# Huiweizhou/GCGCN

Measured on AMD Instinct MI355X. Metric: docs/sec fwd+bwd through CAGGC+MAGGC, higher is better.
Workload: dtype f32; 1 GPU; c2: GraphHops fwd+bwd, B=32/GPU N=64 D=256 L=2 H=8, train mode, E1/E2/X/params require grad, rotating inputs: 3 resident batches (805 MB of E per GPU), step i runs on batch i mod 3; global_batch=32, mode=graph, input_sets=3, parallelism=dp1, grad_allreduce=one coalesced collective after backward

## Files before the change

### gcgcn_amd/_lib.py

```python
from __future__ import annotations

import ctypes
import os
import re
from ctypes import c_char_p, c_double, c_float, c_int, c_int64, c_uint64, c_void_p

_HERE = os.path.dirname(os.path.abspath(__file__))
LIB_PATH = os.environ.get("GCGCN_LIB") or os.path.join(_HERE, "lib", "libgcgcn_hip.so")
HEADER_PATH = os.path.join(os.path.dirname(_HERE), "include", "gcgcn.h")
OPTIM_HEADER_PATH = os.path.join(os.path.dirname(_HERE), "include", "gcgcn_optim.h")
BERT_EMBED_HEADER_PATH = os.path.join(os.path.dirname(_HERE), "include", "gcgcn_bert_embed.h")

ABI_VERSION = 7

SALT_GAT = 0x47415431
SALT_MHA = 0x4D484131
SALT_GCN = 0x47434E31
SALT_GLUE = 0x474C5531
SALT_BERT_ATTN = 0x42415431
SALT_BERT_AO = 0x42414F31
SALT_BERT_OUT = 0x424F5531
SALT_BERT_EMB = 0x42454D31

P, I, F, L = c_void_p, c_int, c_float, c_int64


class MhaHook(ctypes.Structure):
    _fields_ = [("flat_q", c_void_p), ("Q", c_void_p), ("P", c_void_p), ("A", c_void_p), ("dQ", c_void_p), ("rng_snap", c_void_p),
                ("p", ctypes.c_float)]


class EdgeRide(ctypes.Structure):
    _fields_ = [("B", ctypes.c_int32), ("N", ctypes.c_int32), ("D", ctypes.c_int32),
                ("inp", c_void_p), ("n_valid", c_void_p), ("out", c_void_p)]


_SCALARS = {"int": c_int, "int32_t": c_int, "int64_t": c_int64, "uint64_t": c_uint64, "float": c_float, "double": c_double}
_DECL = re.compile(r"([\w\s*]+?)\b(gcgcn_\w+)\s*\(([^()]*)\)")
_DECL_OPTIM = re.compile(r"([\w\s*]+?)\b(gcopt_\w+)\s*\(([^()]*)\)")
_DECL_BERT_EMBED = re.compile(r"([\w\s*]+?)\b(gcbe_\w+)\s*\(([^()]*)\)")
_STRUCT = re.compile(r"typedef\s+struct\s+(\w+)\s*\{([^{}]*)\}\s*\1\s*;")


def _ctype(text: str, symbol: str, named: bool = True, header: str = "include/gcgcn.h"):
    toks = text.replace("*", " * ").split()
    if "*" in toks:
        return c_char_p if toks[:3] == ["const", "char", "*"] and toks.count("*") == 1 else c_void_p
    toks = [t for t in toks if t != "const"]
    if toks == ["void"] and not named:
        return None
    if toks and toks[0] in _SCALARS and len(toks) <= 1 + named:
        return _SCALARS[toks[0]]
    bad = toks[0] if toks and toks[0] not in _SCALARS else " ".join(toks[1:]) or "an empty declaration"
    raise RuntimeError(f"gcgcn_amd: cannot bind {symbol}: no ctypes type for {bad!r} in {text.strip()!r} ({header})")


def _parse_header(text: str, pattern=_DECL, header: str = "include/gcgcn.h"):
    text = re.sub(r"/\*.*?\*/|//[^\n]*", " ", text, flags=re.S)
    text = re.sub(r"^[ \t]*#.*$", " ", text, flags=re.M)
    structs = {}
    for name, body in _STRUCT.findall(text):
        structs[name] = []
        for decl in filter(str.strip, body.split(";")):
            first, *more = decl.split(",")
            ctype = _ctype(first, name, header=header)
            if more and "*" in first:
                raise RuntimeError(f"gcgcn_amd: cannot bind {name}: several names behind a pointer in {decl.strip()!r} ({header})")
            structs[name] += [(n.replace("*", " ").split()[-1], ctype) for n in (first, *more)]
    sigs = {}
    for stmt in filter(str.strip, re.sub(r'extern\s+"C"\s*\{|\}', " ", _STRUCT.sub(" ", text)).split(";")):
        m = pattern.fullmatch(stmt.strip())
        if not m or m.group(2) in sigs:
            raise RuntimeError(f"gcgcn_amd: cannot bind {m.group(2) if m else header}: "
                               f"{'declared twice' if m else 'not a declaration'}: {' '.join(stmt.split())[:100]!r}")
        ret, name, args = m.groups()
        sigs[name] = (_ctype(ret, name, named=False, header=header),
                      [] if args.strip() == "void" else [_ctype(a, name, header=header) for a in args.split(",")])
    return sigs, structs


def _load_header():
    if not os.path.exists(HEADER_PATH):
        raise RuntimeError(f"gcgcn_amd: {HEADER_PATH} not found. The binding is derived from the C header of the source tree; "
                           "there is no recorded copy to fall back to.")
    with open(HEADER_PATH) as f:
        sigs, structs = _parse_header(f.read())
    for cls, name in ((MhaHook, "gcgcn_mha_hook"), (EdgeRide, "gcgcn_edge_ride")):
        declared = [("inp" if n == "in" else n, t) for n, t in structs.get(name, [])]
        if cls._fields_ != declared:
            raise RuntimeError(f"gcgcn_amd: {cls.__name__}._fields_ {cls._fields_} differ from {name} in include/gcgcn.h: {declared}")
    return sigs


def _load_optim_header():
    if not os.path.exists(OPTIM_HEADER_PATH):
        raise RuntimeError(f"gcgcn_amd: {OPTIM_HEADER_PATH} not found. The binding is derived from the C headers of the source tree.")
    with open(OPTIM_HEADER_PATH) as f:
        sigs, structs = _parse_header(f.read(), _DECL_OPTIM, "include/gcgcn_optim.h")
    if structs:
        raise RuntimeError(f"gcgcn_amd: include/gcgcn_optim.h declares structs {list(structs)}; its tables travel as const void*")
    return sigs


def _load_bert_embed_header():
    if not os.path.exists(BERT_EMBED_HEADER_PATH):
        raise RuntimeError(f"gcgcn_amd: {BERT_EMBED_HEADER_PATH} not found. The binding is derived from the C headers of the source tree.")
    with open(BERT_EMBED_HEADER_PATH) as f:
        sigs, structs = _parse_header(f.read(), _DECL_BERT_EMBED, "include/gcgcn_bert_embed.h")
    if structs:
        raise RuntimeError(f"gcgcn_amd: include/gcgcn_bert_embed.h declares structs {list(structs)}; it takes plain arguments only")
    return sigs


SIGNATURES = _load_header()
OPTIM_SIGNATURES = _load_optim_header()
BERT_EMBED_SIGNATURES = _load_bert_embed_header()

_lib = None


def lib() -> ctypes.CDLL:
    global _lib
    if _lib is None:
        if not os.path.exists(LIB_PATH):
            raise RuntimeError(
                f"gcgcn_amd: {LIB_PATH} not found. Build it with `make -C gcgcn_amd/csrc` "
                "(or `python -c 'import __graft_entry__ as g; g.build()'`). There is no CPU fallback.")
        handle = ctypes.CDLL(LIB_PATH)
        for name, (res, args) in list(SIGNATURES.items()) + list(OPTIM_SIGNATURES.items()) + list(BERT_EMBED_SIGNATURES.items()):
            fn = getattr(handle, name)
            fn.restype = res
            fn.argtypes = args
        if handle.gcgcn_version() != ABI_VERSION:
            raise RuntimeError(f"gcgcn_amd: ABI version {handle.gcgcn_version()} != {ABI_VERSION}")
        _lib = handle
    return _lib


def call(name: str, *args):
    h = lib()
    rc = getattr(h, name)(*args)
    if rc != 0:
        raise RuntimeError(f"{name} failed ({rc}): {h.gcgcn_last_error().decode()}")


def layout(kind: str, *dims) -> list:
    n = {"gat": 9, "mha": 3, "gcn": 7, "producer": 17, "head": 7}[kind]
    out = (c_int64 * n)()
    call(f"gcgcn_{kind}_layout", *dims, ctypes.cast(out, c_void_p))
    return list(out)
```

### gcgcn_amd/csrc/api.hip

```cpp
#include "../../include/gcgcn.h"

#include <stdarg.h>
#include <string.h>

#include <new>
#include <vector>

#include <stdlib.h>

#include "attn_plan.hpp"
#include "compact.hpp"
#include "gat_body.hpp"
#include "gemm.hpp"
#include "lstm.hpp"
#include "frontend.hpp"
#include "bert.hpp"
#include "gemm_bf16.hpp"
#include "rowops.hpp"

namespace gc {

static thread_local char g_err[512] = "";

void set_error(const char* fmt, ...) {
  va_list ap;
  va_start(ap, fmt);
  vsnprintf(g_err, sizeof(g_err), fmt, ap);
  va_end(ap);
}

int check_launch(const char* what) {
  hipError_t e = hipGetLastError();
  if (e != hipSuccess) {
    set_error("%s: launch failed: %s", what, hipGetErrorString(e));
    return 2;
  }
  return 0;
}

static struct {
  bool on = false;
  char filter[48] = "";
  std::vector<hipEvent_t> ev;
  int used = 0;
  double work = 0;
} g_prof;

ProfScope::ProfScope(const char* tag, hipStream_t s, double work) : slot(-1), st(s) {
  if (!g_prof.on || strncmp(tag, g_prof.filter, strlen(g_prof.filter)) != 0) return;
  if (2 * (g_prof.used + 1) > (int)g_prof.ev.size()) return;
  slot = g_prof.used++;
  g_prof.work += work;
  (void)hipEventRecord(g_prof.ev[2 * slot], st);
}
ProfScope::~ProfScope() {
  if (slot >= 0) (void)hipEventRecord(g_prof.ev[2 * slot + 1], st);
}
bool prof_events(const char* tag, double work, hipEvent_t* start, hipEvent_t* stop) {
  if (!g_prof.on || strncmp(tag, g_prof.filter, strlen(g_prof.filter)) != 0) return false;
  if (2 * (g_prof.used + 1) > (int)g_prof.ev.size()) return false;
  const int slot = g_prof.used++;
  g_prof.work += work;
  *start = g_prof.ev[2 * slot], *stop = g_prof.ev[2 * slot + 1];
  return true;
}

struct GcnLayout {
  long oWnX, oWe, oWd, oWlin, oblin, total, wd_head;
  int gh;
  long wd_off(int h, int l) const { return oWd + h * wd_head + (long)gh * gh * l * (l - 1) / 2; }
};
static GcnLayout gcn_layout(int D, int L, int H) {
  GcnLayout y;
  y.gh = D / L;
  const long DHD = (long)D * H * D;
  y.wd_head = (long)y.gh * y.gh * L * (L - 1) / 2;
  y.oWnX = 0;
  y.oWe = DHD;
  y.oWd = 2 * DHD;
  y.oWlin = y.oWd + H * y.wd_head;
  y.oblin = y.oWlin + DHD;
  y.total = y.oblin + D;
  return y;
}

static int check_dims(const char* who, int B, int N, int D, int L, int H) {
  GC_REQUIRE(B > 0 && N > 0 && D > 0, "%s: bad shape B=%d N=%d D=%d", who, B, N, D);
  GC_REQUIRE(L > 0 && D % L == 0, "%s: D=%d not divisible by layer_num=%d", who, D, L);
  GC_REQUIRE(H > 0 && D % H == 0, "%s: D=%d not divisible by head_num=%d", who, D, H);
  return 0;
}

static long col_ride_elems(int D) { return (long)COL_RIDE_SLICES * D; }
static long gemm_scratch_elems(int B, int N, int D, int H) {
  const long a = colsum_scratch_elems((long)B * N, D, 1);
  const long rows = (long)B * N > D ? (long)B * N : D;
  const long b = gemm_ws_elems(rows, (long)H * D);
  return a > b ? a : b;
}
static long scratch_elems(int B, int N, int D, int H) { return gemm_scratch_elems(B, N, D, H) + col_ride_elems(D); }

struct Opt {
  const char* name;
  int value;
  bool resolved;
};
static Opt g_opts[] = {{"head_v1", 0, false},      {"head_bil3", 0, false}, {"head_bil3_bwd", 0, false}, {"head_dw3", 0, false},
                       {"head_compact", 0, false}, {"chain_t", 0, false},   {"chain_big", 0, false},     {"split_widen", 0, false},
                       {"chain", 0, false},        {"mha_core", 0, false},  {"group_dump", 0, false},
                       {"bf16_rows", 0, false}};
int option(const char* name, int dflt) {
  for (Opt& o : g_opts) {
    if (strcmp(o.name, name) != 0) continue;
    if (!o.resolved) {
      char env[64] = "GCGCN_";
      size_t n = strlen(env);
      for (const char* c = name; *c && n + 1 < sizeof(env); ++c) env[n++] = (char)((*c >= 'a' && *c <= 'z') ? *c - 32 : *c);
      env[n] = 0;
      const char* e = getenv(env);
      o.value = e ? atoi(e) : dflt;
      o.resolved = true;
    }
    return o.value;
  }
  return dflt;
}
static thread_local int g_head_matmul_next = 0;
int head_matmul_take() {
  const int v = g_head_matmul_next;
  g_head_matmul_next = 0;
  return v;
}
static thread_local int g_lstm_recurrent_next = 0;
int lstm_recurrent_take() {
  const int v = g_lstm_recurrent_next;
  g_lstm_recurrent_next = 0;
  return v;
}
static bool set_opt(const char* name, int value) {
  if (strcmp(name, "head_matmul") == 0) {
    g_head_matmul_next = value;
    return true;
  }
  if (strcmp(name, "lstm_recurrent") == 0) {
    g_lstm_recurrent_next = value;
    return true;
  }
  for (Opt& o : g_opts)
    if (strcmp(o.name, name) == 0) {
      o.value = value, o.resolved = true;
      return true;
    }
  return false;
}

static AttnQuery make_attn_query(int N, int D, int H, const void* Q, const void* dQ, bool hook, bool chain_attends, bool core_done) {
  return AttnQuery{N, D, H, attn_misalign(Q, dQ), hook, chain_attends, core_done, option("mha_core", 1)};
}

static int make_ride(const char* who, const gcgcn_edge_ride* ride, int kind, EdgeRide& r) {
  memset(&r, 0, sizeof(r));
  if (!ride) return 0;
  GC_REQUIRE(ride->B > 0 && ride->N > 0 && ride->D > 0 && ride->in && ride->out, "%s: bad edge ride B=%d N=%d D=%d", who,
             ride->B, ride->N, ride->D);
  GC_REQUIRE((long)ride->B * ride->N <= 0x3fffffffL, "%s: edge ride too large", who);
  r.kind = kind, r.B = ride->B, r.N = ride->N, r.D = ride->D;
  r.in = ride->in, r.n_valid = ride->n_valid, r.out = ride->out;
  return 0;
}

static void use_rows(GemmArgs& g, const int* rowblk, int mode, int zero_dead = 0) {
  if (!rowblk) return;
  g.rb = rowblk + ROWBLK_HDR, g.rb_n = rowblk;
  g.rb_mode = mode, g.rb_zero = zero_dead;
}

static const int* live_rows(const int32_t* rowblk, int N, bool ragged) {
  return (rowblk && ragged && N % 16 == 0 && N >= 32) ? rowblk : nullptr;
}

static ChainQuery make_query(int B, int N, int D, int L, int H, const GcnLayout& y, const float* flat, bool ragged, bool scratch,
                             bool hook, const EdgeRide& ride, const void* A, const void* Pn, const void* Y) {
  ChainQuery q = ChainQuery();
  q.B = B, q.N = N, q.D = D, q.L = L, q.H = H, q.gh = y.gh;
  q.HD = (long)H * D, q.oWd = y.oWd, q.wd_head = y.wd_head, q.oWlin = y.oWlin;
  q.flat = flat, q.ragged = ragged, q.scratch = scratch, q.hook = hook, q.ride = ride;
  q.A = A, q.Pn = Pn, q.Y = Y;
  q.chain = option("chain", 1), q.chain_big = option("chain_big", 0), q.chain_t = option("chain_t", 1);
  return q;
}

static GcnCtx make_ctx(int B, int N, int D, int L, int H, const GcnLayout& y, const float* X, const float* A,
                       const float* flat, const int* n_valid, Drop drop) {
  GcnCtx c;
  memset(&c, 0, sizeof(c));
  c.B = B, c.N = N, c.D = D, c.L = L, c.H = H, c.gh = y.gh;
  c.HD = (long)H * D, c.oWd = y.oWd, c.wd_head = y.wd_head;
  c.X = X, c.A = A, c.flat = flat, c.n_valid = n_valid, c.drop = drop;
  return c;
}

struct EdgeOperand {
  const float* E;
  CmpE ce;
};

static int gat_node_fwd(const float* X, const float* flat, float* uvc, float* s, long M, int D, int Dh, int uvc_valid, void* rng_state,
                        void* rng_snaps, int rng_count, hipStream_t st) {
  if (!uvc_valid) {
    GC_TRY(gat_fold_fwd(flat, uvc, D, Dh, st, rng_state, rng_snaps, rng_count));
    return node_score_fwd(X, uvc, s, M, D, st);
  }
  return node_score_fwd(X, uvc, s, M, D, st, rng_state, rng_snaps, rng_count);
}

static int gat_bwd(const EdgeOperand& eo, int B, int N, int D, int Dh, const float* X, const int* n_valid, const float* flat, Drop drop,
                   const float* uvc, const float* P, const float* dA, const float* dEbar, const float* dX_in, float* dX, float* dE,
                   float* dbias, float* dflat, float* dlogit, float* ds, float* dvpart, float* duvc, float* scratch, DeferQueue* dq,
                   hipStream_t st) {
  const bool compact = eo.E == nullptr;
  const long M = (long)B * N;
  const float* v = uvc + D;
  const EdgePlan plan = edge_plan_bwd({B, N, D, compact, true, dE != nullptr, dEbar != nullptr,
                                       compact ? 0u : edge_misalign(eo.E, v, dE, dEbar, nullptr)});
  const GatTail tail{P, dA, uvc, dX_in, ds, dX, drop, B, plan.slices};
  if (plan.route == EdgePlan::ONE) {
    GC_TRY(gat_dlogit(P, dA, uvc, dX_in, dlogit, ds, dX, B, N, D, plan.slices, drop, st));
  } else if (plan.route == EdgePlan::THREE) {
    GC_TRY(softmax_bwd(P, dA, dlogit, M, N, drop, st));
    GC_TRY(colsum(dlogit, nullptr, ds, N, N, N, B, (long)N * N, 0, N, 0, nullptr, st));
    GC_TRY(node_score_bwd(ds, uvc, dX_in, dX, M, D, st));
  }
  if (compact)
    GC_TRY(cmp_bwd(eo.ce, v, n_valid, dlogit, dEbar, dE, dvpart, scratch + plan.rowbuf_off, dbias, plan, B, N, D, st));
  else
    GC_TRY(edge_bwd(eo.E, v, n_valid, dlogit, dEbar, dE, dvpart, plan, B, N, D, st, dq, &tail));
  long part_off[3];
  int ns = 0;
  GC_TRY(colsum3(X, ds, duvc, M, D, D, dvpart, nullptr, duvc + D, M, D, D, ds, nullptr, duvc + 2 * D, M, 1, 1, scratch,
                 st, false, part_off, &ns));
  return gat_fold_bwd(flat, duvc, dflat, D, Dh, st, scratch, part_off, ns);
}

static OutBwdPlan out_bwd_plan(const OutBwdQuery& q) {
  OutBwdPlan p = OutBwdPlan();
  const bool masked = q.ragged || q.odrop;
  if (q.fuse) {
    p.mask = masked ? OutBwdPlan::MASK_CHAIN : OutBwdPlan::MASK_NONE;
    p.wsum = q.H == 1 ? OutBwdPlan::WSUM_NONE : q.wsum_fwd ? OutBwdPlan::WSUM_FORWARD : OutBwdPlan::WSUM_HERE;
    p.dwlin = OutBwdPlan::DWLIN_BACK;
    const bool in_chain = 2 * q.B <= COL_RIDE_SLICES;
    p.col1 = in_chain ? OutBwdPlan::COL1_CHAIN : OutBwdPlan::COL1_BACK;
    p.chain_slices = in_chain ? 2 * q.B : 0;
    return p;
  }
  p.mask = masked ? OutBwdPlan::MASK_LAUNCH : OutBwdPlan::MASK_NONE;
  constexpr long fold_max = 2L << 20;
  const bool fold = q.scratch && (q.H == 1 || q.wsum_fwd) && (long)q.B * q.N * q.H * q.D <= fold_max && q.dxres_aligned;
  p.fold = !fold ? OutBwdPlan::FOLD_NONE : q.H == 1 ? OutBwdPlan::FOLD_ONE_HEAD : OutBwdPlan::FOLD_HEADS;
  p.fold_drop = fold && (q.H == 1 || q.drop);
  p.head_sum_launch = !fold;
  p.wsum = p.fold == OutBwdPlan::FOLD_HEADS ? OutBwdPlan::WSUM_FORWARD : OutBwdPlan::WSUM_NONE;
  p.dwlin = OutBwdPlan::DWLIN_FRONT;
  p.col1 = q.scratch ? OutBwdPlan::COL1_FRONT : OutBwdPlan::COL1_OWN_LAUNCH;
  return p;
}

static OutBwdCol2 out_bwd_plan_col2(const OutBwdPlan& p, bool front_reduced) {
  switch (p.col1) {
    case OutBwdPlan::COL1_OWN_LAUNCH: return {OutBwdCol2::DONE, 0};
    case OutBwdPlan::COL1_CHAIN: return {OutBwdCol2::BACK_LAUNCH, p.chain_slices};
    case OutBwdPlan::COL1_BACK: return {OutBwdCol2::BACK_REDUCE, 0};
    default: break;
  }
  if (front_reduced) return {OutBwdCol2::FRONT_REDUCE, 0};
  if (p.head_sum_launch) return {OutBwdCol2::HEAD_SUM_KERNEL, 0};
  return {OutBwdCol2::BACK_LAUNCH, COL_RIDE_SLICES};
}

}

using namespace gc;

extern "C" {

int gcgcn_version(void) { return 7; }
const char* gcgcn_last_error(void) { return g_err; }

int gcgcn_set_option(const char* name, int value) {
  GC_REQUIRE(name, "set_option: null name");
  if (set_opt(name, value)) return 0;
  set_error("set_option: unknown option '%s'", name);
  return 1;
}

int64_t gcgcn_row_blocks_ints(int B, int N) { return (B > 0 && N > 0 && N % 16 == 0) ? row_blocks_ints(B, N) : 0; }
// ... 7 lines not shown
  g_prof.ev.assign(2 * (size_t)capacity, nullptr);
  for (auto& e : g_prof.ev) {
    if (hipEventCreate(&e) != hipSuccess) {
      set_error("prof_start: hipEventCreate failed");
      return 2;
    }
  }
  strncpy(g_prof.filter, kernel_prefix, sizeof(g_prof.filter) - 1);
  g_prof.used = 0;
  g_prof.work = 0;
  g_prof.on = true;
  return 0;
}
int gcgcn_prof_enable(int on) {
  g_prof.on = on != 0 && !g_prof.ev.empty();
  return 0;
}
int gcgcn_prof_stop(double* total_ms, int* launches, double* work) {
  GC_REQUIRE(total_ms && launches, "prof_stop: null pointer");
  if (work) *work = g_prof.work;
  g_prof.on = false;
  double tot = 0;
  for (int i = 0; i < g_prof.used; ++i) {
    float ms = 0.f;
    if (hipEventSynchronize(g_prof.ev[2 * i + 1]) != hipSuccess ||
        hipEventElapsedTime(&ms, g_prof.ev[2 * i], g_prof.ev[2 * i + 1]) != hipSuccess) {
      set_error("prof_stop: event query failed");
      return 2;
    }
    tot += ms;
  }
  *total_ms = tot;
  *launches = g_prof.used;
  for (hipEvent_t e : g_prof.ev) (void)hipEventDestroy(e);
  g_prof.ev.clear();
  g_prof.used = 0;
  return 0;
}

int gcgcn_rng_next(void* state, void* snaps, int count, void* stream) {
  GC_REQUIRE(state && snaps && count > 0, "rng_next: bad arguments");
  return rng_next(state, snaps, count, (hipStream_t)stream);
}
int gcgcn_dropout_keep(uint8_t* keep, int64_t n, const void* rng_snap, uint64_t salt, float p, void* stream) {
  GC_REQUIRE(keep && rng_snap, "dropout_keep: null pointer");
  Drop d = make_drop(rng_snap, salt, p);
  d.snap = (const uint64_t*)rng_snap;
  return dropout_keep(keep, n, d, (hipStream_t)stream);
}
int gcgcn_dropout(const float* x, float* y, int64_t n, const void* rng_snap, uint64_t salt, float p, void* stream) {
  GC_REQUIRE(x && y && rng_snap, "dropout: null pointer");
  GC_REQUIRE(p >= 0.f && p < 1.f, "dropout: p=%f out of [0,1)", p);
  Drop d = make_drop(rng_snap, salt, p);
  d.snap = (const uint64_t*)rng_snap;
  return dropout(x, y, n, d, (hipStream_t)stream);
}

int gcgcn_gat_layout(int D, int Dh, int64_t* o) {
  GC_REQUIRE(D > 0 && Dh > 0 && o, "gat_layout: bad arguments");
  const long DD = (long)Dh * D;
  o[0] = 0;
  o[1] = DD;
  o[2] = o[1] + Dh;
  o[3] = o[2] + DD;
  o[4] = o[3] + Dh;
  o[5] = o[4] + DD;
  o[6] = o[5] + Dh;
  o[7] = o[6] + 3 * Dh;
  o[8] = o[7] + 1;
  return 0;
}

int gcgcn_gat_fwd(int B, int N, int D, int Dh, const float* X, const float* E, const int32_t* n_valid, const float* flat,
                  const void* rng_snap, float p, float* uvc, float* s, float* P, float* A, float* Ebar, void* rng_state,
                  void* rng_snaps, int rng_count, const uint8_t* mask, int uvc_valid, void* stream) {
  hipStream_t st = (hipStream_t)stream;
  GC_TRY(check_dims("gat_fwd", B, N, D, 1, 1));
  GC_REQUIRE(Dh > 0, "gat_fwd: hidden_dim=%d", Dh);
  GC_REQUIRE(X && E && flat && uvc && s && P && Ebar, "gat_fwd: null pointer");
  const Drop drop = make_drop(rng_snap, GCGCN_SALT_GAT, p);
  GC_REQUIRE(!drop.snap || A, "gat_fwd: dropout on but A is NULL");
  GC_REQUIRE(!rng_state || (rng_snaps && rng_count > 0), "gat_fwd: rng_state given without snapshots to fill");
  GC_TRY(gat_node_fwd(X, flat, uvc, s, (long)B * N, D, Dh, uvc_valid, rng_state, rng_snaps, rng_count, st));
  return edge_fwd(E, uvc + D, n_valid, Ebar, s, P, A, drop, B, N, D, st, mask);
}

int gcgcn_gat_fwd_compact(int B, int N, int D, int Dh, const float* X, const float* Ec, const int32_t* prow, const float* bias,
                          const int32_t* n_valid, const float* flat, const void* rng_snap, float p, float* uvc, float* s, float* P,
                          float* A, float* Ebar, void* rng_state, void* rng_snaps, int rng_count, int uvc_valid, void* stream) {
  hipStream_t st = (hipStream_t)stream;
  GC_TRY(cmp_check("gat_fwd_compact", B, N, D, Ec, prow, bias));
  GC_REQUIRE(Dh > 0 && X && flat && uvc && s && P && Ebar, "gat_fwd_compact: null pointer");
  const Drop drop = make_drop(rng_snap, GCGCN_SALT_GAT, p);
  GC_REQUIRE(!drop.snap || A, "gat_fwd_compact: dropout on but A is NULL");
  GC_REQUIRE(!rng_state || (rng_snaps && rng_count > 0), "gat_fwd_compact: rng_state given without snapshots to fill");
  GC_TRY(gat_node_fwd(X, flat, uvc, s, (long)B * N, D, Dh, uvc_valid, rng_state, rng_snaps, rng_count, st));
  return cmp_fwd(CmpE{Ec, prow, bias}, uvc + D, n_valid, Ebar, s, P, A, drop, B, N, D, st);
}

int64_t gcgcn_gat_bwd_scratch(int B, int N, int D) { return edge_plan_bwd({B, N, D, false, true, false, false, 0}).scratch; }
int64_t gcgcn_gat_bwd_compact_scratch(int B, int N, int D) { return edge_plan_bwd({B, N, D, true, true, false, false, 0}).scratch; }

int gcgcn_gat_bwd(int B, int N, int D, int Dh, const float* X, const float* E, const int32_t* n_valid, const float* flat,
                  const void* rng_snap, float p, const float* uvc, const float* P, const float* dA, const float* dEbar,
                  const float* dX_in, float* dX, float* dE, float* dflat, float* dlogit, float* ds, float* dvpart,
                  float* duvc, float* scratch, void* defer_queue, void* stream) {
  GC_TRY(check_dims("gat_bwd", B, N, D, 1, 1));
  GC_REQUIRE(Dh > 0, "gat_bwd: hidden_dim=%d", Dh);
  GC_REQUIRE(X && E && flat && uvc && P && dA && dX && dflat && dlogit && ds && dvpart && duvc,
             "gat_bwd: null pointer");
  GC_REQUIRE(scratch, "gat_bwd: scratch is required");
  return gat_bwd(EdgeOperand{E, CmpE()}, B, N, D, Dh, X, n_valid, flat, make_drop(rng_snap, GCGCN_SALT_GAT, p), uvc, P, dA, dEbar, dX_in,
                 dX, dE, nullptr, dflat, dlogit, ds, dvpart, duvc, scratch, (DeferQueue*)defer_queue, (hipStream_t)stream);
}

int gcgcn_gat_bwd_compact(int B, int N, int D, int Dh, const float* X, const float* Ec, const int32_t* prow, const float* bias,
                          const int32_t* n_valid, const float* flat, const void* rng_snap, float p, const float* uvc, const float* P,
                          const float* dA, const float* dEbar, const float* dX_in, float* dX, float* dEc, float* dbias, float* dflat,
                          float* dlogit, float* ds, float* dvpart, float* duvc, float* scratch, void* stream) {
  GC_TRY(cmp_check("gat_bwd_compact", B, N, D, Ec, prow, bias));
  GC_REQUIRE(Dh > 0 && X && flat && uvc && P && dA && dX && dEc && dbias && dflat && dlogit && ds && dvpart && duvc && scratch,
             "gat_bwd_compact: null pointer");
  return gat_bwd(EdgeOperand{nullptr, CmpE{Ec, prow, bias}}, B, N, D, Dh, X, n_valid, flat, make_drop(rng_snap, GCGCN_SALT_GAT, p), uvc, P,
                 dA, dEbar, dX_in, dX, dEc, dbias, dflat, dlogit, ds, dvpart, duvc, scratch, nullptr, (hipStream_t)stream);
}

int gcgcn_edge_mean_fwd(int B, int N, int D, const float* E, const int32_t* n_valid, float* Ebar, void* stream) {
  return edge_fwd(E, nullptr, n_valid, Ebar, nullptr, nullptr, nullptr, make_drop(nullptr, 0, 0.f), B, N, D,
                  (hipStream_t)stream);
}
int gcgcn_edge_mean_bwd(int B, int N, int D, const float* dEbar, const int32_t* n_valid, float* dE, void* stream) {
  GC_REQUIRE(B > 0 && N > 0 && D > 0, "edge_mean_bwd: bad shape");
  return edge_bcast(dEbar, n_valid, dE, B, N, D, (hipStream_t)stream);
}

int gcgcn_edge_mean_fwd_compact(int B, int N, int D, const float* Ec, const int32_t* prow, const float* bias, const int32_t* n_valid,
                                float* Ebar, void* stream) {
  GC_TRY(cmp_check("edge_mean_fwd_compact", B, N, D, Ec, prow, bias));
  GC_REQUIRE(Ebar, "edge_mean_fwd_compact: null pointer");
  return cmp_fwd(CmpE{Ec, prow, bias}, nullptr, n_valid, Ebar, nullptr, nullptr, nullptr, make_drop(nullptr, 0, 0.f), B, N, D,
                 (hipStream_t)stream);
}

int gcgcn_edge_mean_bwd_compact(int B, int N, int D, const int32_t* prow, const int32_t* n_valid, const float* dEbar, float* dEc,
                                float* dbias, float* rowbuf, void* stream) {
  GC_REQUIRE(B > 0 && N > 0 && D > 0, "edge_mean_bwd_compact: bad shape B=%d N=%d D=%d", B, N, D);
  GC_REQUIRE(D <= 64 * CMAXK, "edge_mean_bwd_compact: hidden width %d (compact rows support up to %d)", D, 64 * CMAXK);
  GC_REQUIRE(prow && dEbar && dEc && dbias && rowbuf, "edge_mean_bwd_compact: null pointer");
  return cmp_bwd(CmpE{nullptr, prow, nullptr}, nullptr, n_valid, nullptr, dEbar, dEc, nullptr, rowbuf, dbias,
                 edge_plan_bcast({B, N, D, true, false, false, true, 0}), B, N, D, (hipStream_t)stream);
}

int gcgcn_mha_layout(int D, int64_t* o) {
  GC_REQUIRE(D > 0 && o, "mha_layout: bad arguments");
  o[0] = 0;
  o[1] = (long)D * D;
  o[2] = o[1] + D;
  return 0;
}

int gcgcn_mha_fwd(int B, int N, int D, int H, const float* X, const int32_t* n_valid, const float* flat,
                  const void* rng_snap, float p, float* Q, float* P, float* A, float* scratch, const int32_t* rowblk, void* stream) {
  hipStream_t st = (hipStream_t)stream;
  GC_TRY(check_dims("mha_fwd", B, N, D, 1, H));
  const long wse = scratch ? gemm_scratch_elems(B, N, D, 1) : 0;
  GC_REQUIRE(X && flat && Q && P, "mha_fwd: null pointer");
// ... 940 lines not shown
```

### gcgcn_amd/csrc/chain.hip

```cpp
#include <stdlib.h>

#include <type_traits>

#include "edge_body.hpp"
#include "gcn_plan.hpp"
#include "gemm_body.hpp"
#include "rowops.hpp"

namespace gc {

#ifdef GC_T_TRACE
__device__ long long gc_trace_s[256];
#define TS(i) do { if (blockIdx.x == 0 && threadIdx.x == 0) gc_trace_s[(i) + (c.H == 1 ? 64 : 0)] = wall_clock64(); } while (0)
extern "C" int gcgcn_debug_trace_s(long long* out) { return (int)hipMemcpyFromSymbol(out, HIP_SYMBOL(gc_trace_s), sizeof(long long) * 256); }
#else
#define TS(i)
#endif

__device__ __forceinline__ bool dev_al16(const void* p) { return (((uintptr_t)p) & 15) == 0; }

constexpr int TEAM_LDS = lds_floats<1, 1, true, true>();
constexpr int CHAIN_LDS = 2 * TEAM_LDS;
constexpr int XCHG_LDS = 64 * 64;
typedef float f32x4 __attribute__((ext_vector_type(4)));
constexpr int CW = 8;
constexpr int RB = 8;

template <bool AKC, bool BKC, bool ALIGNED, int MASK, int RT>
__device__ __forceinline__ void run_product(GemmArgs g, float* lds, int z) {
  g.ksplit = g.K;
  g.splits = 1;
  if (!ALIGNED) {
    g.vecA = dev_al16(g.A) && g.lda % 4 == 0 && g.sA1 % 4 == 0 && g.sA2 % 4 == 0;
    g.vecB = dev_al16(g.B) && g.ldb % 4 == 0 && g.sB1 % 4 == 0 && g.sB2 % 4 == 0;
  }
  const int team = threadIdx.x >> 8, t = threadIdx.x & 255;
  float* tl = lds + team * TEAM_LDS;
  const int tn = (g.N + 63) >> 6, tiles = ((g.M + 63) >> 6) * tn;
  for (int p = 0; p < tiles; p += 2) {
    int q = p + team;
    const bool live = q < tiles;
    if (!live) q = tiles - 1;
    gemm_body<1, 1, AKC, BKC, ALIGNED, 16, MASK, RT>(g, tl, q % tn, q / tn, z, t, live);
  }
}

template <bool AKC1, bool BKC1, int MK1, int RTA, bool AKC2, bool BKC2, int MK2, int RTB, bool ALIGNED>
__device__ __forceinline__ void run_two_products(GemmArgs g1, GemmArgs g2, float* lds, int z) {
  auto prep = [](GemmArgs& g) {
    g.ksplit = g.K, g.splits = 1;
    if (!ALIGNED) {
      g.vecA = dev_al16(g.A) && g.lda % 4 == 0 && g.sA1 % 4 == 0 && g.sA2 % 4 == 0;
      g.vecB = dev_al16(g.B) && g.ldb % 4 == 0 && g.sB1 % 4 == 0 && g.sB2 % 4 == 0;
    }
  };
  prep(g1), prep(g2);
  const int team = threadIdx.x >> 8, t = threadIdx.x & 255;
  float* tl = lds + team * TEAM_LDS;
  const int tn1 = (g1.N + 63) >> 6, tiles1 = ((g1.M + 63) >> 6) * tn1, b1 = tiles1 * (1 + (g1.K + 31) / 32);
  const int tn2 = (g2.N + 63) >> 6, tiles2 = ((g2.M + 63) >> 6) * tn2, b2 = tiles2 * (1 + (g2.K + 31) / 32);
  if (team == 0) {
    for (int q = 0; q < tiles1; ++q) gemm_body<1, 1, AKC1, BKC1, ALIGNED, 16, MK1, RTA>(g1, tl, q % tn1, q / tn1, z, t, true);
    for (int i = b1; i < b2; ++i) __syncthreads();
  } else {
    for (int q = 0; q < tiles2; ++q) gemm_body<1, 1, AKC2, BKC2, ALIGNED, 16, MK2, RTB>(g2, tl, q % tn2, q / tn2, z, t, true);
    for (int i = b2; i < b1; ++i) __syncthreads();
  }
}

template <bool ALIGNED>
__global__ __launch_bounds__(64 * CW) void gcn_chain_fwd_kernel(const GcnCtx c) {
  __shared__ __attribute__((aligned(16))) float lds[CHAIN_LDS];
  if (blockIdx.x >= c.B * c.H) {
    const EdgeRide& r = c.ride;
    edge_fwd_row<4, false, CW>(r.in, nullptr, r.n_valid, r.out, nullptr, nullptr, nullptr, Drop(), r.N, r.D,
                               blockIdx.x - c.B * c.H, lds);
    return;
  }
  const int z = blockIdx.x;
  const int lane = threadIdx.x & 63, wave = threadIdx.x >> 6;
  {
    const float* a = c.A + (long)z * c.N * c.N;
    for (int i0 = wave; i0 < c.N; i0 += CW * RB) {
      float s[RB];
#pragma unroll
      for (int u = 0; u < RB; ++u) s[u] = 0.f;
      for (int j = lane; j < c.N; j += 64) {
#pragma unroll
        for (int u = 0; u < RB; ++u) {
          const int i = i0 + CW * u;
          if (i < c.N) s[u] += a[(long)i * c.N + j];
        }
      }
#pragma unroll
      for (int u = 0; u < RB; ++u) {
        const int i = i0 + CW * u;
        const float t = wave_sum(s[u]);
        if (lane == 0 && i < c.N) c.rinv[(long)z * c.N + i] = 1.f / (t + (t == 0.f ? 1.f : 0.f));
      }
    }
  }
  __syncthreads();
  for (int l = 0; l < c.L; ++l) {
    if (l > 0) {
      run_product<true, false, ALIGNED, EPI_ACCUM, 0>(plan_fwd_dense(c, l), lds, z);
      __syncthreads();
    }
    run_product<true, false, ALIGNED, EPI_ADD | EPI_ROWSCALE | EPI_RELU | EPI_C2, 0>(plan_fwd_agg(c, l), lds, z);
    __syncthreads();
  }
}

template <bool ALIGNED>
__global__ __launch_bounds__(64 * CW) void gcn_chain_bwd_kernel(const GcnCtx c, const GemmGroup4 cg) {
  __shared__ __attribute__((aligned(16))) float lds[CHAIN_LDS + XCHG_LDS];
  if (blockIdx.x >= c.B * c.H) {
    int pb;
    if (spread_pick((int)blockIdx.x - c.B * c.H, c.carry, pb)) {
      gemm_group_splitk_block(cg, pb, lds, TEAM_LDS, lds + CHAIN_LDS);
      return;
    }
    const EdgeRide& r = c.ride;
    edge_bcast_row<4, CW>(r.in, r.n_valid, r.out, r.N, r.D, 0, pb);
    return;
  }
  const int z = blockIdx.x;
  const int b = z / c.H, h = z - b * c.H;
  const int lane = threadIdx.x & 63, wave = threadIdx.x >> 6;
  for (int l = c.L - 1; l >= 0; --l) {
    for (int i0 = wave; i0 < c.N; i0 += CW * RB) {
      float acc[RB], rv[RB];
#pragma unroll
      for (int u = 0; u < RB; ++u) {
        const int i = i0 + CW * u;
        acc[u] = 0.f;
        rv[u] = (i < c.N) ? c.rinv[(long)z * c.N + i] : 0.f;
      }
      for (int k = lane; k < c.gh; k += 64) {
        float y[RB], gy[RB];
#pragma unroll
        for (int u = 0; u < RB; ++u) {
          const int i = i0 + CW * u;
          const long off = ((((long)b * c.N + i) * c.H + h) * c.L + l) * c.gh + k;
          y[u] = 0.f, gy[u] = 0.f;
          if (i < c.N) y[u] = c.Y[off], gy[u] = c.dYa[off];
        }
#pragma unroll
        for (int u = 0; u < RB; ++u) {
          const int i = i0 + CW * u;
          const long off = ((((long)b * c.N + i) * c.H + h) * c.L + l) * c.gh + k;
          const float g = y[u] > 0.f ? gy[u] : 0.f;
          if (i < c.N) c.dM[off] = g * rv[u];
          acc[u] = fmaf(g, y[u], acc[u]);
        }
      }
#pragma unroll
      for (int u = 0; u < RB; ++u) {
        const int i = i0 + CW * u;
        const float t = wave_sum(acc[u]);
        if (lane == 0 && i < c.N) {
          const long ri = (long)z * c.N + i;
          const float d = -rv[u] * t;
          c.drow[ri] = (l == c.L - 1) ? d : c.drow[ri] + d;
        }
      }
    }
    __syncthreads();
    run_two_products<false, false, 0, 0, true, true, 0, EPI_ACCUM | EPI_ROWADD, ALIGNED>(plan_bwd_dP(c, l), plan_bwd_dA(c, l), lds, z);
    __syncthreads();
    if (l > 0) {
      run_product<true, true, ALIGNED, EPI_ACCUM, 0>(plan_bwd_dY(c, l), lds, z);
      __syncthreads();
    }
  }
}

constexpr int S_LA = 68;
constexpr int S_LP = 132;
constexpr int S_GH = 128;
constexpr int S_FWD_LDS = 64 * S_LA + 2 * 64 * S_LP + 64 + S_GH * S_LP;
constexpr int S_BWD_XS = 6 * 16 * 64;
constexpr int S_BWD_LDS = 64 * S_LA + 3 * 64 * S_LP + 128 + S_BWD_XS;
static_assert(S_FWD_LDS >= CHAIN_LDS && S_BWD_LDS >= CHAIN_LDS + XCHG_LDS, "passengers use the chain kernels' LDS");
static_assert(S_BWD_LDS * sizeof(float) <= 160 * 1024, "LDS of one compute unit");

__device__ __forceinline__ void lds_barrier() { asm volatile("s_waitcnt lgkmcnt(0)\n\ts_barrier" ::: "memory"); }

template <int K, bool AV, bool BV>
__device__ __forceinline__ void mma_lds(f32x16& acc, const float* __restrict__ pa, const int la,
                                        const float* __restrict__ pb, const int lb) {
#pragma unroll
  for (int k0 = 0; k0 < K; k0 += 8) {
    float a[4], b[4];
    if (AV) {
      const f32x4 v = *reinterpret_cast<const f32x4*>(pa + k0);
      a[0] = v.x, a[1] = v.y, a[2] = v.z, a[3] = v.w;
    } else {
#pragma unroll
      for (int m = 0; m < 4; ++m) a[m] = pa[(k0 + m) * la];
    }
    if (BV) {
      const f32x4 v = *reinterpret_cast<const f32x4*>(pb + k0);
      b[0] = v.x, b[1] = v.y, b[2] = v.z, b[3] = v.w;
    } else {
#pragma unroll
      for (int m = 0; m < 4; ++m) b[m] = pb[(k0 + m) * lb];
    }
#pragma unroll
    for (int m = 0; m < 4; ++m) acc = __builtin_amdgcn_mfma_f32_32x32x2f32(a[m], b[m], acc, 0, 0, 0);
  }
}
__device__ __forceinline__ int acc_row(int r0, int q) { return r0 + (q & 3) + 8 * (q >> 2); }

__global__ __launch_bounds__(64 * CW) void gcn_chain_s_fwd_kernel(const GcnCtx c) {
  __shared__ __attribute__((aligned(16))) float lds[S_FWD_LDS];
  if (blockIdx.x >= c.B * c.H) {
    const EdgeRide& r = c.ride;
    edge_fwd_row<4, false, CW>(r.in, nullptr, r.n_valid, r.out, nullptr, nullptr, nullptr, Drop(), r.N, r.D,
                               blockIdx.x - c.B * c.H, lds);
    return;
  }
  TS(0);
  float* const As = lds;
  float* const Ps = As + 64 * S_LA;
  float* const Ys = Ps + 64 * S_LP;
  float* const Rs = Ys + 64 * S_LP;
  float* const Ws = Rs + 64;
  const int z = blockIdx.x, b = z / c.H, h = z - b * c.H;
  const int t = threadIdx.x, lane = t & 63, wave = t >> 6, r = lane & 31, hf = lane >> 5;
  const int rb = wave & 1, cb = wave >> 1;
  const unsigned HD = (unsigned)c.HD, D = (unsigned)c.D;
  const long zoff = (long)b * 64 * c.HD + (long)h * 2 * S_GH;
  const float* __restrict__ Ag = c.A + (long)z * 64 * 64;
  const float* __restrict__ Pg = c.Pn + zoff;
  const float* __restrict__ Gg = c.G + zoff;
  const float* __restrict__ Xg = c.X + (long)b * 64 * c.D;
  float* __restrict__ Yg = c.Y + zoff;
  float* __restrict__ Hg = c.HO + zoff;
  const int r0 = rb * 32 + hf * 4, col = cb * 32 + r;
  const bool dd = c.drop.snap != nullptr;
  const uint64_t key = dd ? drop_key(c.drop) : 0;

  const bool own_att = c.mha.Q != nullptr;
  f32x4 a[2], p[4];
  float s[8];
  if (!own_att) {
#pragma unroll
    for (int u = 0; u < 2; ++u) {
      const int idx = t + 512 * u;
      a[u] = *reinterpret_cast<const f32x4*>(Ag + (idx >> 4) * 64 + (idx & 15) * 4);
    }
  }
#pragma unroll
  for (int u = 0; u < 4; ++u) {
    const int idx = t + 512 * u;
    p[u] = *reinterpret_cast<const f32x4*>(Pg + (unsigned)(idx >> 5) * HD + (idx & 31) * 4);
  }
  if (!own_att) {
#pragma unroll
    for (int u = 0; u < 8; ++u) s[u] = Ag[(wave * 8 + u) * 64 + lane];
  }
  float gv[2][16], xv[2][16], pv[16];
#pragma unroll
  for (int q = 0; q < 16; ++q) {
    const unsigned row = (unsigned)acc_row(r0, q);
    gv[0][q] = Gg[row * HD + (unsigned)col];
    xv[0][q] = Xg[row * D + (unsigned)col];
  }
  TS(1);
  if (own_att) {
    mha_core_fwd_body<true>(Ys, z, c.mha.Q, c.n_valid, c.mha.P, c.mha.A, 64, c.D, c.H, c.mha.dh, c.mha.kchunk, c.mha.alpha, c.mha.drop, t,
                            t < 256, As, S_LA, CW);
    lds_barrier();
#pragma unroll
    for (int u = 0; u < 8; ++u) s[u] = As[(wave * 8 + u) * S_LA + lane];
  } else {
#pragma unroll
    for (int u = 0; u < 2; ++u) {
      const int idx = t + 512 * u;
      *reinterpret_cast<f32x4*>(As + (idx >> 4) * S_LA + (idx & 15) * 4) = a[u];
    }
  }
  TS(2);
#pragma unroll
  for (int u = 0; u < 4; ++u) {
    const int idx = t + 512 * u;
    *reinterpret_cast<f32x4*>(Ps + (idx >> 5) * S_LP + (idx & 31) * 4) = p[u];
  }
#pragma unroll
  for (int u = 0; u < 8; ++u) {
    const float tt = wave_sum(s[u]);
    if (lane == 0) {
      const float ri = 1.f / (tt + (tt == 0.f ? 1.f : 0.f));
      Rs[wave * 8 + u] = ri;
      c.rinv[(long)z * 64 + wave * 8 + u] = ri;
    }
  }
  {
    const float* __restrict__ W = c.flat + c.wd_off(1) + (long)h * c.wd_head;
    f32x4 wv[8];
#pragma unroll
    for (int u = 0; u < 8; ++u) wv[u] = *reinterpret_cast<const f32x4*>(W + (t + 512 * u) * 4);
// ... 357 lines not shown
    }
    TS(33 + 10 * l);
    mma_lds<64, true, true>(dacc, Ds + ((ab & 1) * 32 + r) * S_LP + kh * 64 + 4 * hf, 0,
                            Ps + ((ab >> 1) * 32 + r) * S_LP + kh * 64 + 4 * hf, 0);
    TS(34 + 10 * l);
    if constexpr (l == 1) {
      lds_barrier();
      TS(35 + 10 * l);
#pragma unroll
      for (int u = 0; u < 8; ++u) {
        const int idx = t + 512 * u;
        *reinterpret_cast<f32x4*>(Ws + (idx >> 5) * S_LP + (idx & 31) * 4) = wd[u];
      }
#pragma unroll
      for (int u = 0; u < 4; ++u) {
        const int idx = t + 512 * u;
        p0[u] = *reinterpret_cast<const f32x4*>(Pg + (unsigned)(idx >> 5) * HD + (idx & 31) * 4);
      }
#pragma unroll
      for (int u = 0; u < 8; ++u)
#pragma unroll
        for (int kk = 0; kk < 2; ++kk) y0[u][kk] = Yg[(unsigned)(wave + 8 * u) * HD + (unsigned)(lane + 64 * kk)];
      if constexpr (!FUSE) {
#pragma unroll
        for (int q = 0; q < 16; ++q)
          gv[q] = Gy[(unsigned)acc_row(r0, q) * HD + (unsigned)col];
      }
      TS(36 + 10 * l);
      lds_barrier();
      TS(37 + 10 * l);
#pragma unroll
      for (int q = 0; q < 16; ++q) acc[q] = 0.f;
      mma_lds<S_GH, true, true>(acc, Qs + (rb * 32 + r) * S_LP + 4 * hf, 0, Ws + col * S_LP + 4 * hf, 0);
      TS(38 + 10 * l);
      lds_barrier();
#pragma unroll
      for (int q = 0; q < 16; ++q) Ds[acc_row(r0, q) * S_LP + col] = acc[q] + gv[q];
#pragma unroll
      for (int u = 0; u < 4; ++u) {
        const int idx = t + 512 * u;
        *reinterpret_cast<f32x4*>(Ps + (idx >> 5) * S_LP + (idx & 31) * 4) = p0[u];
      }
      lds_barrier();
    }
  };
  sublayer(std::integral_constant<int, 1>());
  sublayer(std::integral_constant<int, 0>());
  if (kh == 1) {
#pragma unroll
    for (int q = 0; q < 16; ++q) Qs[(ab * 16 + q) * 64 + lane] = dacc[q];
  }
  lds_barrier();
  if (kh == 0) {
    float* __restrict__ dAg = c.dA + (long)z * 64 * 64;
    const int ar0 = (ab & 1) * 32 + hf * 4, acol = (ab >> 1) * 32 + r;
#pragma unroll
    for (int q = 0; q < 16; ++q) {
      const int row = acc_row(ar0, q);
      dAg[row * 64 + acol] = dacc[q] + Qs[(ab * 16 + q) * 64 + lane] + Ts[row];
    }
  } else if (t >= 256 && t < 320) {
    c.drow[(long)z * 64 + (t - 256)] = Ts[t - 256];
  }
  TS(55);
}

bool chain_g_aligned(const ChainQuery& q, bool bwd) {
  bool ok = q.N % 64 == 0 && q.gh % 64 == 0 && al16(q.A) && al16(q.flat + q.oWd) && al16(q.Pn) && al16(q.Y);
  if (bwd) ok = ok && al16(q.dYa) && al16(q.dM) && al16(q.dP) && al16(q.dA);
  else ok = ok && al16(q.G) && al16(q.HO) && al16(q.X);
  return ok;
}
bool chain_s_serves(const ChainQuery& q, bool bwd) {
  return chain_g_aligned(q, bwd) && q.N == 64 && q.L == 2 && q.gh == S_GH && q.D == 2 * S_GH && q.wd_head % 4 == 0 && q.oWd % 4 == 0;
}
bool chain_s_fuses(const ChainQuery& q) {
  return (q.H == 1 || q.H == 8) && al16(q.flat + q.oWlin) && q.HD % 4 == 0 && al16(q.dout) && al16(q.dXres) && al16(q.dout_m);
}
bool chain_s_attends(const ChainQuery& q) {
  return mha_lds_bytes(q.D / q.H) <= sizeof(float) * 64 * S_LP && (q.D / q.H) % 4 == 0;
}
bool chain_can_carry(const EdgeRide& r) {
  return r.kind != 0 && r.D % 4 == 0 && al16(r.in) && al16(r.out) && (long)CW * r.D <= CHAIN_LDS &&
         (long)r.B * r.N <= 0x3fffffffL;
}

static ChainPlan chain_pick(const ChainQuery& q, bool bwd, bool ride) {
  ChainPlan p;
  p.ride = ride;
  const bool s = chain_s_serves(q, bwd), t = q.chain_t != 0 && chain_t_serves(q, bwd, ride);
  const bool s_preferred = s && q.chain_t < 2 && !(q.chain_t == 1 && q.ragged);
  p.kind = (t && !s_preferred) ? ChainPlan::T : s ? ChainPlan::S : ChainPlan::GENERIC;
  p.aligned = p.kind == ChainPlan::GENERIC && chain_g_aligned(q, bwd);
  p.full = p.kind == ChainPlan::T && q.N == 64 && !q.ragged;
  return p;
}
ChainPlan chain_plan_fwd(const ChainQuery& q) {
  const bool ride = chain_can_carry(q.ride);
  if (!q.chain || !(q.N <= 64 || ride || q.chain_big)) return ChainPlan();
  ChainPlan p = chain_pick(q, false, ride);
  p.attention = q.hook && (p.kind == ChainPlan::T ? chain_t_attends(q) : p.kind == ChainPlan::S && chain_s_attends(q));
  return p;
}
ChainPlan chain_plan_bwd(const ChainQuery& q) {
  if (!q.chain || !(q.N <= 64 || q.chain_big)) return ChainPlan();
  ChainPlan p = chain_pick(q, true, chain_can_carry(q.ride));
  p.fuse = q.scratch && (long)q.B * q.N * q.HD >= (long)q.D * q.D &&
           (p.kind == ChainPlan::T ? chain_t_fuses(q) : p.kind == ChainPlan::S && chain_s_fuses(q));
  return p;
}

static unsigned chain_grid(const GcnCtx& c, int kind) {
  return (unsigned)(c.B * c.H) + (c.ride.kind == kind ? (unsigned)(c.ride.B * c.ride.N) : 0u);
}

int gcn_chain_fwd(const GcnCtx& c, const ChainPlan& p, hipStream_t st) {
  GC_REQUIRE(p.kind != ChainPlan::NONE, "gcn_chain_fwd: the plan names no chain kernel");
  GC_REQUIRE((long)c.B * c.H <= 0x3fffffffL, "gcn_chain_fwd: too many (doc, head) pairs");
  GC_REQUIRE(c.ride.kind == 0 || (c.ride.kind == 1 && chain_can_carry(c.ride)), "gcn_chain_fwd: bad passenger");
  dim3 grid(chain_grid(c, 1)), block(64 * CW);
  double fl = 0;
  for (int l = 0; l < c.L; ++l) fl += 2.0 * c.N * c.gh * (c.N + (double)l * c.gh);
  if (p.kind == ChainPlan::T) return gcn_chain_t_fwd(c, p, grid, fl * c.B * c.H, st);
  if (p.kind == ChainPlan::S)
    GC_LAUNCH_TIMED("gcn_chain_fwd", fl * c.B * c.H, gcn_chain_s_fwd_kernel, grid, block, 0, st, c);
  else if (p.aligned) GC_LAUNCH_TIMED("gcn_chain_fwd", fl * c.B * c.H, gcn_chain_fwd_kernel<true>, grid, block, 0, st, c);
  else GC_LAUNCH_TIMED("gcn_chain_fwd", fl * c.B * c.H, gcn_chain_fwd_kernel<false>, grid, block, 0, st, c);
  return check_launch("gcn_chain_fwd");
}

int gcn_chain_bwd(const GcnCtx& c, const ChainPlan& p, hipStream_t st, DeferQueue* carry) {
  GC_REQUIRE(p.kind != ChainPlan::NONE, "gcn_chain_bwd: the plan names no chain kernel");
  GC_REQUIRE(c.ride.kind == 0 || (c.ride.kind == 2 && chain_can_carry(c.ride)), "gcn_chain_bwd: bad passenger");
  double fl = 0;
  for (int l = 0; l < c.L; ++l) fl += 4.0 * c.N * c.gh * c.N + 2.0 * c.N * c.gh * (double)l * c.gh;
  fl *= (double)c.B * c.H;
  if (p.kind == ChainPlan::T) return gcn_chain_t_bwd(c, p, fl, st, carry);
  GemmGroup4 cg;
  cg.nprob = 0, cg.tile_begin[0] = 0;
  int ng = 0;
  if (carry && carry->n > 0 && (long)c.B * c.H <= 64 && ((long)c.B * c.N) % 64 == 0) {
    const int passes = (((c.N + 63) / 64) * ((c.gh + 63) / 64) + 1) / 2;
    const double t_chain = 8.0 * (4 * c.L - 1) * passes;
    const double t_tile = 0.47 * ((double)c.B * c.N / 32.0);
    const long rounds = t_tile > 0 ? (long)(t_chain / t_tile) : 0;
    bool halves = true;
    for (int i = 0; i < carry->n; ++i) halves = halves && carry->p[i].K % 64 == 0 && !carry->p[i].rb;
    long budget = rounds * (256 - (long)c.B * c.H);
    if (c.ride.kind == 2) budget /= 2;
    if (rounds > 0 && halves && budget > 0) ng = gemm_take_deferred_pairs(carry, cg, &fl, budget);
  }
  dim3 grid(chain_grid(c, 2) + (unsigned)ng), block(64 * CW);
  GcnCtx cc = c;
  cc.carry = chain_carry_spread(c, ng);
  if (p.kind == ChainPlan::S && p.fuse) {
    fl += 2.0 * c.B * c.N * c.D * c.D * (c.H + (c.H > 1 ? 1 : 0));
    GC_LAUNCH_TIMED("gcn_chain_bwd", fl, gcn_chain_s_bwd_kernel<true>, grid, block, 0, st, cc, cg);
  } else if (p.kind == ChainPlan::S)
    GC_LAUNCH_TIMED("gcn_chain_bwd", fl, gcn_chain_s_bwd_kernel<false>, grid, block, 0, st, cc, cg);
  else if (p.aligned) GC_LAUNCH_TIMED("gcn_chain_bwd", fl, gcn_chain_bwd_kernel<true>, grid, block, 0, st, cc, cg);
  else GC_LAUNCH_TIMED("gcn_chain_bwd", fl, gcn_chain_bwd_kernel<false>, grid, block, 0, st, cc, cg);
  return check_launch("gcn_chain_bwd");
}

Spread chain_carry_spread(const GcnCtx& c, int ng) {
  constexpr int spread_pct = 85, cohort = 128, spread_min = 256;
  const long rows = c.ride.kind == 2 ? (long)c.ride.B * c.ride.N : 0;
  const bool on = rows > 0 && ng >= spread_min;
  return make_spread(ng, rows, cohort, on ? spread_pct : 0);
}

}
```

### gcgcn_amd/csrc/chain_t.hpp

```cpp
#pragma once
#include <type_traits>

#include "chain_t_shapes.hpp"
#include "edge_body.hpp"
#include "gcn_plan.hpp"
#include "gemm_body.hpp"
#include "rowops.hpp"

namespace gc {

#ifdef GC_T_TRACE
static __device__ long long gc_trace_t[256];
#define TR(i) do { if (blockIdx.x == 0 && threadIdx.x == 0) gc_trace_t[i] = wall_clock64(); } while (0)
#define TRB(i) do { if (blockIdx.x == 0 && threadIdx.x == 0) gc_trace_t[(i) + (c.H == 1 ? 64 : 0)] = wall_clock64(); } while (0)
#else
#define TR(i)
#define TRB(i)
#endif

typedef float t4 __attribute__((ext_vector_type(4)));

__device__ __forceinline__ void t_barrier() { asm volatile("s_waitcnt lgkmcnt(0)\n\ts_barrier" ::: "memory"); }
__device__ __forceinline__ t4 mfma16(float a, float b, t4 c) { return __builtin_amdgcn_mfma_f32_16x16x4f32(a, b, c, 0, 0, 0); }
__device__ __forceinline__ float row16_sum(float v) {
// ... 135 lines not shown
    }
    t4 acc[4];
#pragma unroll
    for (int ob = 0; ob < 4; ++ob) {
      acc[ob] = t4{0.f, 0.f, 0.f, 0.f};
#pragma unroll
      for (int kb = 0; kb < 4; ++kb) {
        if (ob < NRB && kb < NRB) {
          const t4 a = *reinterpret_cast<const t4*>(Asj + 16 * ob * T_LA + 16 * kb);
#pragma unroll
          for (int v = 0; v < 4; ++v) acc[ob] = mfma16(a[v], Pa[l][kb][v], acc[ob]);
        }
      }
    }
    TR(11 + 8 * l);
#pragma unroll
    for (int rb = 0; rb < 4; ++rb)
#pragma unroll
      for (int v = 0; v < 4; ++v) {
        const float y = fmaxf((acc[rb][v] + gv[rb][v]) * Rsg[16 * rb + v], 0.f);
        if constexpr (NP > 0) Ysg[(16 * rb + v) * P] = y;
        t_st(Yd, tHD, rowHD(rb, v, l), y);
        float d = y;
        if (dd) {
          const unsigned o = (unsigned)(16 * rb + 4 * g + v) * HD + (unsigned)(l * GH + col);
          d = (rng_u32(key, (uint64_t)(zoff + (long)o)) >= c.drop.thresh) ? y * c.drop.scale : 0.f;
        }
        t_st(Hd, tHD, rowHD(rb, v, l), d + xv[rb][v]);
      }
    if constexpr (NP > 0) {
      TR(12 + 8 * l);
      sstore(0, wr[0]);
      t_barrier();
      TR(13 + 8 * l);
      auto compute = [&](const int ch, const int st) __attribute__((always_inline)) {
        t4 a[NRB > 0 ? NRB : 1];
#pragma unroll
        for (int rb = 0; rb < NRB; ++rb) a[rb] = *reinterpret_cast<const t4*>(Ysj + 16 * rb * P + 16 * ch);
#pragma unroll
        for (int p = 0; p < NP; ++p) {
          const float* wb = Ws + ((st * (L - 1) + p) * 16 + 4 * g) * P + col;
          float bv[4];
#pragma unroll
          for (int v = 0; v < 4; ++v) bv[v] = wb[v * P];
#pragma unroll
          for (int v = 0; v < 4; ++v)
#pragma unroll
            for (int rb = 0; rb < NRB; ++rb) Pa[l + 1 + p][rb] = mfma16(a[rb][v], bv[v], Pa[l + 1 + p][rb]);
        }
      };
#pragma nounroll
      for (int ch = 0; ch < NC; ch += 2) {
        if (ch + 2 < NC) gload(ch + 2, wr[0]);
        compute(ch, 0);
        sstore(1, wr[1]);
        t_barrier();
        if (ch + 3 < NC) gload(ch + 3, wr[1]);
        compute(ch + 1, 1);
        if (ch + 2 < NC) sstore(0, wr[0]);
        t_barrier();
      }
      TR(14 + 8 * l);
#pragma unroll
      for (int rb = 0; rb < 4; ++rb)
#pragma unroll
        for (int v = 0; v < 4; ++v) t_st(Pd, tHD, rowHD(rb, v, l + 1), Pa[l + 1][rb][v]);
    }
  };
  static_assert(L >= 1 && L <= 4, "sub-layers are unrolled by hand");
  layer(std::integral_constant<int, 0>());
  if constexpr (L > 1) layer(std::integral_constant<int, 1>());
  if constexpr (L > 2) layer(std::integral_constant<int, 2>());
  if constexpr (L > 3) layer(std::integral_constant<int, 3>());
  TR(50);
}

template <int GH, int L, bool FULL>
__global__ __launch_bounds__(4 * GH) void gcn_chain_t_fwd_kernel(const GcnCtx c) {
  constexpr int W = GH / 16;
  __shared__ __attribute__((aligned(16))) float lds[t_fwd_lds(GH, L)];
  if (blockIdx.x >= c.B * c.H) {
    const EdgeRide& r = c.ride;
    edge_fwd_row<4, false, W>(r.in, nullptr, r.n_valid, r.out, nullptr, nullptr, nullptr, Drop(), r.N, r.D,
                              blockIdx.x - c.B * c.H, lds);
    return;
  }
  const int z = blockIdx.x, b = z / c.H, h = z - b * c.H;
  if constexpr (FULL) {
    chain_t_fwd_body<GH, L, 4>(c, lds, z, b, h);
  } else {
    const int nv = c.n_valid ? min(max(c.n_valid[b], 0), c.N) : c.N;
    const int nrb = (nv + 15) >> 4;
    switch (nrb) {
      case 0: chain_t_fwd_body<GH, L, 0>(c, lds, z, b, h); break;
      case 1: chain_t_fwd_body<GH, L, 1>(c, lds, z, b, h); break;
      case 2: chain_t_fwd_body<GH, L, 2>(c, lds, z, b, h); break;
      case 3: chain_t_fwd_body<GH, L, 3>(c, lds, z, b, h); break;
      default: chain_t_fwd_body<GH, L, 4>(c, lds, z, b, h); break;
    }
  }
}

constexpr int T_TEAM_LDS = lds_floats<1, 1, true, true>();
template <int NTEAM, bool RB>
__device__ __forceinline__ void t_parked_tiles(const GemmGroup4& cg, int pb, float* __restrict__ lds) {
  int i = 0, w = pb;
  while (i + 1 < cg.nprob && w >= (cg.tile_take[i] + NTEAM - 1) / NTEAM) {
    w -= (cg.tile_take[i] + NTEAM - 1) / NTEAM;
    ++i;
  }
  const int team = threadIdx.x >> 8, t = threadIdx.x & 255;
  int q = NTEAM * w + team;
  const bool live = q < cg.tile_take[i];
  if (!live) q = cg.tile_take[i] - 1;
  q = xcd_remap(q + cg.tile_first[i], cg.tile_count[i]);
  const GemmArgs& g = cg.p[i];
  const int tn = g.N >> 6, tm = g.M >> 6;
  const int zs = q / (tn * tm), r = q - zs * (tn * tm);
  const int bx = (tm < tn) ? r / tm : r % tn, by = (tm < tn) ? r % tm : r / tn;
  float* tl = lds + team * T_TEAM_LDS;
  if (g.a_kc) {
    if (g.b_kc) gemm_body<1, 1, true, true, true>(g, tl, bx, by, zs, t, live);
    else gemm_body<1, 1, true, false, true>(g, tl, bx, by, zs, t, live);
  } else {
    if (g.b_kc) gemm_body<1, 1, false, true, true>(g, tl, bx, by, zs, t, live);
    else gemm_body<1, 1, false, false, true, GC_GEMM_EG, 0, EPI_ALL, PlainOperands, RB>(g, tl, bx, by, zs, t, live);
  }
}

template <int GH, int L, int NRB, bool FUSE>
__device__ __forceinline__ void chain_t_bwd_body(const GcnCtx& c, float* __restrict__ lds, const int z, const int b, const int h, const int nv) {
  constexpr int REG = FUSE ? t_bwd_region(GH, L) : 2 * 64 * (GH + 4);
  constexpr int W = GH / 16, NT = 4 * GH, P = GH + 4, NC = GH / 16, SP = 20;
  static_assert(2 * GH * SP <= 64 * P, "weight stages live in the Pn image");
  static_assert(W <= 4 || (W / 4 - 1) * 4096 <= 64 * P, "dA exchange lives in the dM image");
  constexpr int OBW = W >= 4 ? 1 : 4 / W;
  constexpr int KS = GH >= 64 ? 4 : GH / 16;
  TRB(100);
  float* const ATs = lds;
  float* const Ds = ATs + 64 * T_LA;
  float* const Ps = Ds + 64 * P;
  float* const Tp = Ds + REG;
  float* const Ts = Tp + W * 64;
  float* const Rs = Ts + 64;
  const int t = threadIdx.x, lane = t & 63, w = t >> 6, j = lane & 15, g = lane >> 4;
  const int N = c.N;
  const unsigned HD = (unsigned)c.HD;
  const long zoff = (long)b * N * c.HD + (long)h * c.D;
  const float* __restrict__ Ag = c.A + (long)z * N * N;
  const unsigned Dw = (unsigned)c.D;
  const t_desc Yd = t_buffer(c.Y + zoff, N, HD, Dw), Gd = t_buffer(c.dYa + zoff, N, HD, Dw);
  const t_desc Md = t_buffer(c.dM + zoff, N, HD, Dw), Qd = t_buffer(c.dP + zoff, N, HD, Dw);
  const t_desc Pd = t_buffer(c.Pn + zoff, min(N, 16 * NRB), HD, Dw);
  const int col = 16 * w + j;
  const int ob = w & 3, ks = w >> 2;
  const unsigned tHD = ((unsigned)(4 * g) * HD + (unsigned)col) * 4u;
  auto rowHD = [&](const int rb, const int v, const int l) { return ((unsigned)(16 * rb + v) * HD + (unsigned)(l * GH)) * 4u; };
  const t_desc Wdd = t_buffer(c.flat + c.oWd + (long)h * c.wd_head, 1, 0, (unsigned)c.wd_head);
  const unsigned wvoff = ((unsigned)(t >> 2) * GH + 4u * (unsigned)(t & 3)) * 4u;
  float* const Dsg = Ds + 4 * g * P + col;
  float* const Tpg = Tp + w * 64 + 4 * g;
  const float* const Rsg = Rs + 4 * g;
  const float* const ATj = ATs + j * T_LA + 4 * g;
  const float* const Dsj = Ds + j * P + 4 * g;
  const float* const Psj = Ps + j * P + 4 * g;

  {
// ... 460 lines not shown
```

### gcgcn_amd/csrc/edge.hip

```cpp
#include <string.h>

#include "edge_body.hpp"
#include "compact.hpp"
#include "gat_body.hpp"
#include "gemm_body.hpp"
#include "rowops.hpp"

namespace gc {

template <int VEC, bool ATT>
__global__ __launch_bounds__(64 * EW) void edge_fwd_kernel(const float* __restrict__ E, const float* __restrict__ v,
                                                           const int* __restrict__ n_valid, float* __restrict__ Ebar,
                                                           const float* __restrict__ coladd, float* __restrict__ P,
                                                           float* __restrict__ Aout, Drop drop, int N, int D,
                                                           const unsigned char* __restrict__ mask) {
  extern __shared__ __attribute__((aligned(16))) float cs[];
  edge_fwd_row<VEC, ATT, EW>(E, v, n_valid, Ebar, coladd, P, Aout, drop, N, D, blockIdx.x, cs, mask);
}

template <int VEC>
__device__ __forceinline__ void edge_bwd_row(const float* __restrict__ E, const float* __restrict__ v,
                                             const int* __restrict__ n_valid, const float* __restrict__ dlogit,
                                             const float* __restrict__ dEbar, float* __restrict__ dE,
                                             float* __restrict__ dvpart, int N, int D, int nt, const int bi,
                                             float* __restrict__ sm, const GatTail& gt) {
  float* dl = sm;
  float* cs = sm + ((N + 3) & ~3);
  const int b = bi / N, i = bi - b * N;
  const int t = threadIdx.x, lane = t & 63, wave = t >> 6;
  const int nv = n_valid ? min(max(n_valid[b], 0), N) : N;
  float* dEr = dE ? dE + (long)bi * N * D : nullptr;
  float* dvp = dvpart + (long)bi * D;
  if (i >= nv) {
    for (int c = t; c < D; c += 64 * EW) dvp[c] = 0.f;
    if (dEr) {
      const long tot = (long)N * D;
      for (long o = t; o < tot; o += 64 * EW) dEr[o] = 0.f;
    }
    return;
  }
  if (gt.P) {
    if (wave == 0) {
      const long o = (long)bi * N + min(lane, N - 1);
      float p = gt.P[o], g = gt.dA[o];
      if (lane >= N) p = 0.f, g = 0.f;
      if (gt.drop.snap) g = (rng_u32(drop_key(gt.drop), (uint64_t)((long)bi * N + lane)) >= gt.drop.thresh) ? g * gt.drop.scale : 0.f;
      const float dot = wave_sum(g * p);
      if (lane < N) dl[lane] = p * (g - dot);
    }
  } else {
    for (int j = t; j < N; j += 64 * EW) dl[j] = dlogit[(long)bi * N + j];
  }
  __syncthreads();
  const float* __restrict__ Er = E + (long)bi * N * D;
  const float inv = 1.f / (float)nv;
  const int nchunk = (D + 64 * VEC - 1) / (64 * VEC);
  for (int q = 0; q < nchunk; ++q) {
    const int c = (q * 64 + lane) * VEC;
    const bool act = c < D;
    float vr[VEC], g[VEC], acc[VEC];
#pragma unroll
    for (int e = 0; e < VEC; ++e) vr[e] = 0.f, g[e] = 0.f, acc[e] = 0.f;
    if (act) {
      vload<VEC>(vr, v + c);
      if (dEbar) {
        vload<VEC>(g, dEbar + (long)bi * D + c);
#pragma unroll
        for (int e = 0; e < VEC; ++e) g[e] *= inv;
      }
    }
    int j = wave;
    for (; j + (EUNR - 1) * EW < nv; j += EUNR * EW) {
      float x[EUNR][VEC];
#pragma unroll
      for (int u = 0; u < EUNR; ++u) {
#pragma unroll
        for (int e = 0; e < VEC; ++e) x[u][e] = 0.f;
        if (act) vload_nt<VEC>(x[u], Er + (long)(j + u * EW) * D + c);
      }
#pragma unroll
      for (int u = 0; u < EUNR; ++u) {
        const float d = dl[j + u * EW];
        float o[VEC];
#pragma unroll
        for (int e = 0; e < VEC; ++e) {
// ... 74 lines not shown
    gemm_group_block<RB>(gg, r, tile_lds);
    return;
  }
  const int ngat = gt.P ? gt.B * gt.slices : 0;
  if (r < ngat) {
    const int b = r / gt.slices;
    gat_dlogit_doc(gt.P, gt.dA, gt.uvc, gt.dXin, nullptr, gt.ds, gt.dX, N, D, gt.drop, b, r - b * gt.slices, gt.slices, tile_lds);
    return;
  }
  edge_bwd_row<VEC>(E, v, n_valid, dlogit, dEbar, dE, dvpart, N, D, nt, r - ngat, tile_lds, gt);
}

template <int VEC>
__global__ __launch_bounds__(64 * EW) void edge_bcast_kernel(const float* __restrict__ dEbar,
                                                             const int* __restrict__ n_valid, float* __restrict__ dE,
                                                             int N, int D, int nt) {
  edge_bcast_row<VEC, EW>(dEbar, n_valid, dE, N, D, nt, blockIdx.x);
}

static inline bool al16(const void* p) { return (((uintptr_t)p) & 15) == 0; }
unsigned edge_misalign(const void* E, const void* v, const void* dE, const void* dEbar, const void* Ebar) {
  return (al16(E) ? 0 : EDGE_MIS_E) | (al16(v) ? 0 : EDGE_MIS_V) | (al16(dE) ? 0 : EDGE_MIS_DE) | (al16(dEbar) ? 0 : EDGE_MIS_DEBAR) |
         (al16(Ebar) ? 0 : EDGE_MIS_EBAR);
}
constexpr size_t EDGE_LDS_MAX = 160 * 1024;
constexpr size_t CMP_LDS_MAX = 64 * 1024;
constexpr size_t TILE_LDS = sizeof(float) * lds_floats<1, 1, true, true>();
static_assert(sizeof(float) * GAT_DOC_LDS <= TILE_LDS, "GAT passenger needs more LDS than a tile");

static EdgePlan plan_rows(const EdgeQuery& q, unsigned operands) {
  EdgePlan p;
  p.compact = q.compact, p.att = q.att;
  p.vec = (!q.compact && q.D % 4 == 0 && !(q.mis & operands)) ? 4 : 1;
  p.grid = (long)q.B * q.N;
  return p;
}

EdgePlan edge_plan_fwd(const EdgeQuery& q) {
  EdgePlan p = plan_rows(q, EDGE_MIS_E | EDGE_MIS_EBAR | (q.att ? EDGE_MIS_V : 0));
  p.lds = ((size_t)(q.compact ? CW4 : EW) * q.D + (q.att ? (size_t)q.N : 0)) * sizeof(float);
  p.lds_limit = q.compact ? CMP_LDS_MAX : EDGE_LDS_MAX;
  return p;
}

EdgePlan edge_plan_bwd(const EdgeQuery& q) {
  EdgePlan p = plan_rows(q, EDGE_MIS_E | EDGE_MIS_V | (q.has_dE ? EDGE_MIS_DE : 0) | (q.has_dEbar ? EDGE_MIS_DEBAR : 0));
  if (q.att) {
    p.route = q.N > GT ? EdgePlan::THREE : (q.compact ? EdgePlan::ONE : EdgePlan::RIDE);
    if (p.route != EdgePlan::THREE) p.slices = gat_dlogit_slices(q.D);
    if (p.route == EdgePlan::RIDE) p.ngat = q.B * p.slices;
    const long a = colsum_scratch_elems((long)q.B * q.N, q.D, 1), b = 3L * 64 * (2 * q.D + 1);
    p.scratch = a > b ? a : b;
    if (q.compact) p.rowbuf_off = p.scratch, p.scratch += 2L * q.B * q.N;
  }
  if (q.compact) {
    p.lds = ((size_t)CW4 * q.D + 2 * CW4) * sizeof(float);
    return p;
  }
  const size_t lds_row = ((size_t)((q.N + 3) & ~3) + (size_t)EW * q.D) * sizeof(float);
  p.lds = (p.ngat && lds_row < sizeof(float) * GAT_DOC_LDS) ? sizeof(float) * GAT_DOC_LDS : lds_row;
  p.lds_limit = EDGE_LDS_MAX;
  p.carry_ok = p.vec == 4 && lds_row <= TILE_LDS;
  p.grid += p.ngat;
  return p;
}

EdgePlan edge_plan_bcast(const EdgeQuery& q) {
  if (!q.compact) return plan_rows(q, EDGE_MIS_DE | EDGE_MIS_DEBAR);
  EdgeQuery m = q;
  m.att = false;
  return edge_plan_bwd(m);
}

void edge_plan_carry(EdgePlan& p, int ntile, bool any_rb, int col_C) {
  if (ntile <= 0) return;
  const long rows = p.grid;
  p.ntile = ntile, p.RB = any_rb;
  p.ncolwg = col_C > 0 ? cdiv(col_C, 256) : 0;
  p.col_base = col_C > 0 ? (int)(rows + ntile) : 0;
  p.grid = rows + ntile + p.ncolwg;
  constexpr int spread_pct = 90, cohort = 256, spread_min = 1024;
  p.spread = make_spread(ntile, rows, cohort, ntile >= spread_min ? spread_pct : 0);
  p.lds = 0;
}

constexpr int NT_STORE = 0;

int edge_fwd(const float* E, const float* v, const int* n_valid, float* Ebar, const float* coladd, float* P, float* A,
             Drop drop, int B, int N, int D, hipStream_t st, const unsigned char* mask) {
  GC_REQUIRE(E && Ebar, "edge_fwd: null pointer");
  GC_REQUIRE(B > 0 && N > 0 && D > 0, "edge_fwd: bad shape B=%d N=%d D=%d", B, N, D);
  const bool att = P != nullptr;
  GC_REQUIRE(!att || (v && coladd), "edge_fwd: attention requested without v / node scores");
  const EdgePlan p = edge_plan_fwd({B, N, D, false, att, false, false, edge_misalign(E, v, nullptr, nullptr, Ebar)});
  GC_REQUIRE(p.lds_ok(), "edge_fwd: N=%d D=%d needs %zu B of LDS", N, D, p.lds);
  dim3 grid((unsigned)p.grid), block(64 * EW);
  const char* tag = att ? "edge_fwd_att" : "edge_fwd_mean";
  const double bytes = 4.0 * B * N * N * D;
#define GC_EDGE_FWD(V, AT) \
  GC_LAUNCH_TIMED(tag, bytes, (edge_fwd_kernel<V, AT>), grid, block, p.lds, st, E, v, n_valid, Ebar, coladd, P, A, drop, N, D, mask)
  if (p.vec == 4) {
    if (att) GC_EDGE_FWD(4, true);
    else GC_EDGE_FWD(4, false);
  } else {
    if (att) GC_EDGE_FWD(1, true);
    else GC_EDGE_FWD(1, false);
  }
#undef GC_EDGE_FWD
  return check_launch("edge_fwd");
}

int edge_bwd(const float* E, const float* v, const int* n_valid, const float* dlogit, const float* dEbar, float* dE,
             float* dvpart, const EdgePlan& plan, int B, int N, int D, hipStream_t st, DeferQueue* carry, const GatTail* tail) {
  GatTail gt;
  memset(&gt, 0, sizeof gt);
  if (tail && plan.route == EdgePlan::RIDE) gt = *tail;
  GC_REQUIRE(E && v && (dlogit || gt.P) && dvpart, "edge_bwd: null pointer");
  GC_REQUIRE(!gt.P || (N <= GT && gt.B == B && gt.slices == plan.slices && gt.dA && gt.uvc && gt.ds && gt.dX), "edge_bwd: bad GAT passenger");
  GC_REQUIRE(!plan.compact && plan.ngat == (gt.P ? B * gt.slices : 0) &&
                 (plan.vec == 4) == (D % 4 == 0 && !edge_misalign(E, v, dE, dEbar, nullptr)),
             "edge_bwd: the plan was made for other operands");
  static_assert(sizeof(GatTail) + sizeof(GemmGroup) + 96 <= 4096, "edge_bwd_carry_kernel: kernel arguments exceed 4 KB");
  GC_REQUIRE(plan.lds_ok(), "edge_bwd: N=%d D=%d needs %zu B of LDS", N, D, plan.lds);
  EdgePlan p = plan;
  dim3 block(64 * EW);
  const double bytes = (dE ? 8.0 : 4.0) * B * N * N * D;
  GemmGroup gg;
  double gflops = 0;
  const int ntile = (p.carry_ok && carry && carry->n > 0) ? gemm_take_deferred(carry, gg, &gflops) : 0;
  if (ntile > 0) {
    const bool col = gemm_take_deferred_col2(carry, gg.col);
    bool any_rb = false;
    for (int i = 0; i < gg.nprob; ++i) any_rb = any_rb || gg.p[i].rb != nullptr;
    edge_plan_carry(p, ntile, any_rb, col ? gg.col.C : 0);
    dim3 grid((unsigned)p.grid);
#define GC_EDGE_CARRY(RBV)                                                                                                  \
  GC_LAUNCH_TIMED("edge_bwd", bytes, (edge_bwd_carry_kernel<4, RBV>), grid, block, 0, st, E, v, n_valid, dlogit, dEbar, dE, \
                  dvpart, N, D, NT_STORE, p.spread, gt, gg, p.col_base)
    if (p.RB) GC_EDGE_CARRY(true);
    else GC_EDGE_CARRY(false);
#undef GC_EDGE_CARRY
    return check_launch("edge_bwd_carry");
  }
  dim3 grid((unsigned)p.grid);
#define GC_EDGE_BWD(V)                                                                                                             \
  GC_LAUNCH_TIMED("edge_bwd", bytes, (edge_bwd_kernel<V>), grid, block, p.lds, st, E, v, n_valid, dlogit, dEbar, dE, dvpart, N, D, \
                  NT_STORE, gt)
  if (p.vec == 4) GC_EDGE_BWD(4);
  else GC_EDGE_BWD(1);
#undef GC_EDGE_BWD
  return check_launch("edge_bwd");
}

int edge_bcast(const float* dEbar, const int* n_valid, float* dE, int B, int N, int D, hipStream_t st) {
  GC_REQUIRE(dEbar && dE, "edge_bcast: null pointer");
  const EdgePlan p = edge_plan_bcast({B, N, D, false, false, true, true, edge_misalign(nullptr, nullptr, dE, dEbar, nullptr)});
  dim3 grid((unsigned)p.grid), block(64 * EW);
  ProfScope ps("edge_bcast", st, 4.0 * B * N * N * D);
  if (p.vec == 4) hipLaunchKernelGGL((edge_bcast_kernel<4>), grid, block, 0, st, dEbar, n_valid, dE, N, D, NT_STORE);
  else hipLaunchKernelGGL((edge_bcast_kernel<1>), grid, block, 0, st, dEbar, n_valid, dE, N, D, NT_STORE);
  return check_launch("edge_bcast");
}

}
```

### gcgcn_amd/csrc/edge_body.hpp

```cpp
#pragma once
#include "common.hpp"

namespace gc {

template <int VEC>
__device__ __forceinline__ void vload(float (&r)[VEC], const float* p) {
  if constexpr (VEC == 4) {
    const float4 v = *reinterpret_cast<const float4*>(p);
    r[0] = v.x, r[1] = v.y, r[2] = v.z, r[3] = v.w;
  } else {
    r[0] = p[0];
  }
}
template <int VEC>
__device__ __forceinline__ void vstore(float* p, const float (&r)[VEC]) {
  if constexpr (VEC == 4) {
    *reinterpret_cast<float4*>(p) = make_float4(r[0], r[1], r[2], r[3]);
  } else {
    p[0] = r[0];
  }
}

template <int VEC>
__device__ __forceinline__ void vload_nt(float (&r)[VEC], const float* p) {
// ... 52 lines not shown
                                             float* __restrict__ cs, const unsigned char* __restrict__ mask = nullptr) {
  const int b = bi / N, i = bi - b * N;
  const int t = threadIdx.x, lane = t & 63, wave = t >> 6;
  const int nv = n_valid ? min(max(n_valid[b], 0), N) : N;
  float* eb = Ebar + (long)bi * D;
  float* lg = cs + (long)EWT * D;
  if (i >= nv) {
    for (int c = t; c < D; c += 64 * EWT) eb[c] = 0.f;
    if (ATT)
      for (int j = t; j < N; j += 64 * EWT) {
        P[(long)bi * N + j] = 0.f;
        if (Aout) Aout[(long)bi * N + j] = 0.f;
      }
    return;
  }
  const float* __restrict__ Er = E + (long)bi * N * D;
  const int nchunk = (D + 64 * VEC - 1) / (64 * VEC);
  for (int q = 0; q < nchunk; ++q) {
    const int c = (q * 64 + lane) * VEC;
    const bool act = c < D;
    float vr[VEC], acc[VEC];
#pragma unroll
    for (int e = 0; e < VEC; ++e) vr[e] = 0.f, acc[e] = 0.f;
    if (ATT && act) vload<VEC>(vr, v + c);
    int j = wave;
    for (; j + (EUNR - 1) * EWT < nv; j += EUNR * EWT) {
      float x[EUNR][VEC];
#pragma unroll
      for (int u = 0; u < EUNR; ++u) {
#pragma unroll
        for (int e = 0; e < VEC; ++e) x[u][e] = 0.f;
        if (act) vload_nt<VEC>(x[u], Er + (long)(j + u * EWT) * D + c);
      }
#pragma unroll
      for (int u = 0; u < EUNR; ++u) {
        float dot = 0.f;
#pragma unroll
        for (int e = 0; e < VEC; ++e) {
          acc[e] += x[u][e];
          dot = fmaf(x[u][e], vr[e], dot);
        }
        if (ATT) {
          dot = wave_sum(dot);
          if (lane == 0) {
            if (q == 0) lg[j + u * EWT] = dot;
            else lg[j + u * EWT] += dot;
          }
        }
      }
    }
    for (; j < nv; j += EWT) {
      float x[VEC];
#pragma unroll
      for (int e = 0; e < VEC; ++e) x[e] = 0.f;
      if (act) vload<VEC>(x, Er + (long)j * D + c);
      float dot = 0.f;
#pragma unroll
      for (int e = 0; e < VEC; ++e) {
        acc[e] += x[e];
        dot = fmaf(x[e], vr[e], dot);
      }
      if (ATT) {
        dot = wave_sum(dot);
        if (lane == 0) {
          if (q == 0) lg[j] = dot;
          else lg[j] += dot;
        }
      }
    }
    if (act) vstore<VEC>(cs + wave * D + c, acc);
  }
  __syncthreads();
  const float inv = 1.f / (float)nv;
  for (int c = t; c < D; c += 64 * EWT) {
    float s = 0.f;
#pragma unroll
    for (int w = 0; w < EWT; ++w) s += cs[w * D + c];
    eb[c] = s * inv;
  }
  if (ATT && wave == 0) edge_softmax_tail(lg, coladd + (long)b * N, mask, P, Aout, drop, N, nv, (long)bi * N, lane);
}


template <int VEC, int EWT>
__device__ __forceinline__ void edge_bcast_row(const float* __restrict__ dEbar, const int* __restrict__ n_valid,
                                               float* __restrict__ dE, int N, int D, int nt, int bi) {
  const int b = bi / N, i = bi - b * N;
  const int t = threadIdx.x, lane = t & 63, wave = t >> 6;
  const int nv = n_valid ? min(max(n_valid[b], 0), N) : N;
  float* dEr = dE + (long)bi * N * D;
  const bool rowpad = i >= nv;
  const float inv = rowpad ? 0.f : 1.f / (float)nv;
  const int nchunk = (D + 64 * VEC - 1) / (64 * VEC);
  for (int q = 0; q < nchunk; ++q) {
    const int c = (q * 64 + lane) * VEC;
    if (c >= D) continue;
    float g[VEC], z[VEC];
    vload<VEC>(g, dEbar + (long)bi * D + c);
#pragma unroll
    for (int e = 0; e < VEC; ++e) g[e] *= inv, z[e] = 0.f;
    for (int j = wave; j < N; j += EWT) {
      const bool live = !rowpad && j < nv;
      if (nt) vstore_nt<VEC>(dEr + (long)j * D + c, live ? g : z);
      else vstore<VEC>(dEr + (long)j * D + c, live ? g : z);
    }
  }
}

}
```

### gcgcn_amd/csrc/edge_plan.hpp

```cpp
#pragma once
#include "common.hpp"

namespace gc {

enum EdgeMisalign { EDGE_MIS_E = 1, EDGE_MIS_V = 2, EDGE_MIS_DE = 4, EDGE_MIS_DEBAR = 8, EDGE_MIS_EBAR = 16 };
unsigned edge_misalign(const void* E, const void* v, const void* dE, const void* dEbar, const void* Ebar);

struct EdgeQuery {
  int B, N, D;
  bool compact;
  bool att;
  bool has_dE, has_dEbar;
  unsigned mis;
};

struct EdgePlan {
  enum Route { RIDE = 0, ONE = 1, THREE = 2 };
  bool compact = false, att = false;
  int vec = 1;
  int route = -1;
  int slices = -1;
  int ngat = 0;
  size_t lds = 0;
  size_t lds_limit = 0;
  bool lds_ok() const { return lds_limit == 0 || lds <= lds_limit; }
  bool carry_ok = false;
  int ntile = 0, ncolwg = 0, col_base = 0;
  bool RB = false;
  long grid = 0;
  Spread spread = {0, 0, 0};
  long scratch = -1;
  long rowbuf_off = -1;
};

EdgePlan edge_plan_fwd(const EdgeQuery& q);
EdgePlan edge_plan_bwd(const EdgeQuery& q);
EdgePlan edge_plan_bcast(const EdgeQuery& q);
void edge_plan_carry(EdgePlan& p, int ntile, bool any_rb, int col_C);

}
```

### gcgcn_amd/csrc/gcn_plan.hpp

```cpp
#pragma once
#include "gemm.hpp"
#include "mha_body.hpp"

namespace gc {

struct EdgeRide {
  int kind;
  int B, N, D;
  const float* in;
  const int* n_valid;
  float* out;
};

struct GcnCtx {
  int B, N, D, L, H, gh;
  EdgeRide ride;
  struct MhaFwd {
    const float* Q;
    float* P;
    float* A;
    float alpha;
    Drop drop;
    int dh, kchunk;
  } mha;
  Spread carry;
  long HD, oWd, wd_head;
  const float* X;
  const float* A;
  const float* flat;
  const int* n_valid;
  Drop drop;
  const float* G;
  float* Pn;
  float* Y;
  float* HO;
  float* rinv;
  float* dYa;
  float* dM;
  float* dP;
  float* dA;
  float* drow;
  const float* dout;
  float* dout_m;
  Drop odrop;
  const float* Wsum;
  float* dXres;
  float* colpart;
  long oWlin;
  __host__ __device__ long wd_off(int l) const { return oWd + (long)gh * gh * l * (l - 1) / 2; }
};

__host__ __device__ inline GemmArgs plan_fwd_dense(const GcnCtx& c, int l) {
  const long sb = (long)c.N * c.HD, sh = (long)c.L * c.gh;
  GemmArgs g = gemm_nn(c.Y, c.HD, c.flat + c.wd_off(l), c.gh, c.Pn + (long)l * c.gh, c.HD, c.N, c.gh, l * c.gh);
  g.batch_z1(c.B, sb, 0, sb).batch_z2(c.H, sh, c.wd_head, sh);
  g.splits = 1;
  g.accumulate = 1;
  g.tag = "gemm_dense";
  return g;
}

__host__ __device__ inline GemmArgs plan_fwd_agg(const GcnCtx& c, int l) {
  const long off = (long)l * c.gh, sb = (long)c.N * c.HD, sh = (long)c.L * c.gh;
  GemmArgs g = gemm_nn(c.A, c.N, c.Pn + off, c.HD, c.Y + off, c.HD, c.N, c.gh, c.N);
  g.batch_z1(c.B, (long)c.H * c.N * c.N, sb, sb).batch_z2(c.H, (long)c.N * c.N, sh, sh);
  g.splits = 1;
  g.add = c.G + off, g.ldadd = c.HD, g.sAdd1 = sb, g.sAdd2 = sh;
  g.rowscale = c.rinv, g.sRs1 = (long)c.H * c.N, g.sRs2 = c.N;
  g.relu = 1;
  g.C2 = c.HO + off, g.ldc2 = c.HD, g.sC21 = sb, g.sC22 = sh;
  g.add2 = c.X + off, g.ldadd2 = c.D, g.sAdd21 = (long)c.N * c.D, g.sAdd22 = 0;
  g.drop = c.drop, g.drop_base = off;
  g.tag = "gemm_agg";
  return g;
}

__host__ __device__ inline GemmArgs plan_bwd_dP(const GcnCtx& c, int l) {
  const long off = (long)l * c.gh, sb = (long)c.N * c.HD, sh = (long)c.L * c.gh;
  GemmArgs g = gemm_tn(c.A, c.N, c.dM + off, c.HD, c.dP + off, c.HD, c.N, c.gh, c.N);
  g.batch_z1(c.B, (long)c.H * c.N * c.N, sb, sb).batch_z2(c.H, (long)c.N * c.N, sh, sh);
  g.splits = 1;
  g.tag = "gemm_dP";
  return g;
}

__host__ __device__ inline GemmArgs plan_bwd_dA(const GcnCtx& c, int l) {
  const long off = (long)l * c.gh, sb = (long)c.N * c.HD, sh = (long)c.L * c.gh;
  GemmArgs g = gemm_nt(c.dM + off, c.HD, c.Pn + off, c.HD, c.dA, c.N, c.N, c.N, c.gh);
  g.batch_z1(c.B, sb, sb, (long)c.H * c.N * c.N).batch_z2(c.H, sh, sh, (long)c.N * c.N);
  g.splits = 1;
  g.accumulate = (l != c.L - 1);
// ... 87 lines not shown
```

### gcgcn_amd/csrc/rowops.hip

```cpp
#include "gat_body.hpp"
#include "gemm.hpp"
#include "rowops.hpp"

namespace gc {

constexpr int RW = 4;

__global__ __launch_bounds__(64 * RW) void softmax_fwd_kernel(const float* __restrict__ S, const float* __restrict__ coladd,
                                                              const int* __restrict__ n_valid, float* __restrict__ P,
                                                              float* __restrict__ A, long rows, int N, int heads,
                                                              Drop drop) {
  const long r = (long)blockIdx.x * RW + (threadIdx.x >> 6);
  if (r >= rows) return;
  const int lane = threadIdx.x & 63;
  const long doc = r / ((long)heads * N);
  const int i = (int)(r % N);
  const int nv = n_valid ? min(max(n_valid[doc], 0), N) : N;
  const float* s = S + r * N;
  float* p = P + r * N;
  float* a = A ? A + r * N : nullptr;
  if (i >= nv) {
    for (int j = lane; j < N; j += 64) {
      p[j] = 0.f;
      if (a) a[j] = 0.f;
    }
    return;
  }
  const float* ca = coladd ? coladd + doc * N : nullptr;
  float m = -INFINITY;
  for (int j = lane; j < nv; j += 64) m = fmaxf(m, s[j] + (ca ? ca[j] : 0.f));
  m = wave_max(m);
  float sum = 0.f;
  for (int j = lane; j < nv; j += 64) sum += expf(s[j] + (ca ? ca[j] : 0.f) - m);
  sum = wave_sum(sum);
  const float inv = 1.f / sum;
  const bool dd = a && drop.snap;
  const uint64_t key = dd ? drop_key(drop) : 0;
  for (int j = lane; j < N; j += 64) {
    float v = 0.f;
    if (j < nv) v = expf(s[j] + (ca ? ca[j] : 0.f) - m) * inv;
    p[j] = v;
    if (a) {
      if (dd) v = (rng_u32(key, (uint64_t)(r * N + j)) >= drop.thresh) ? v * drop.scale : 0.f;
      a[j] = v;
    }
  }
}

__global__ __launch_bounds__(64 * RW) void softmax_bwd_kernel(const float* __restrict__ P, const float* __restrict__ dA,
                                                              float* __restrict__ dS, long rows, int N, Drop drop) {
  const long r = (long)blockIdx.x * RW + (threadIdx.x >> 6);
  if (r >= rows) return;
  const int lane = threadIdx.x & 63;
  const float* p = P + r * N;
  const float* da = dA + r * N;
  float* ds = dS + r * N;
  const bool dd = drop.snap != nullptr;
  const uint64_t key = dd ? drop_key(drop) : 0;
  float dot = 0.f;
  for (int j = lane; j < N; j += 64) {
    float g = da[j];
    if (dd) g = (rng_u32(key, (uint64_t)(r * N + j)) >= drop.thresh) ? g * drop.scale : 0.f;
    dot = fmaf(g, p[j], dot);
  }
  dot = wave_sum(dot);
  for (int j = lane; j < N; j += 64) {
    float g = da[j];
    if (dd) g = (rng_u32(key, (uint64_t)(r * N + j)) >= drop.thresh) ? g * drop.scale : 0.f;
    ds[j] = p[j] * (g - dot);
  }
}

__global__ __launch_bounds__(64 * RW) void rowsum_inv_kernel(const float* __restrict__ A, float* __restrict__ rinv,
                                                             long rows, int N) {
  const long r = (long)blockIdx.x * RW + (threadIdx.x >> 6);
  if (r >= rows) return;
  const int lane = threadIdx.x & 63;
  float s = 0.f;
  for (int j = lane; j < N; j += 64) s += A[r * N + j];
  s = wave_sum(s);
  if (lane == 0) rinv[r] = 1.f / (s + (s == 0.f ? 1.f : 0.f));
}
// ... 125 lines not shown
  if (c < C) {
    long r = r0 + wave;
    for (; r + 28 < r1; r += 32) {
      float v[8], wv[8];
#pragma unroll
      for (int u = 0; u < 8; ++u) v[u] = x[(r + 4 * u) * ld + c], wv[u] = ww ? ww[r + 4 * u] : 1.f;
#pragma unroll
      for (int u = 0; u < 8; ++u) acc = fmaf(wv[u], v[u], acc);
    }
    for (; r < r1; r += 4) acc = fmaf(ww ? ww[r] : 1.f, x[r * ld + c], acc);
  }
  red[wave][lane] = acc;
  __syncthreads();
  if (wave == 0 && c < C) {
    const float s = red[0][lane] + red[1][lane] + red[2][lane] + red[3][lane];
    float* o = out + z * sOz + (long)sp * C + c;
    *o = accumulate ? *o + s : s;
  }
}

struct ColJobs {
  static constexpr int MAXJ = 4;
  const float* X[MAXJ];
  const float* w[MAXJ];
  float* out[MAXJ];
  long R[MAXJ], ld[MAXJ];
  int C[MAXJ];
  long part_off[MAXJ];
  int n;
};
__global__ __launch_bounds__(256) void colsum_multi_kernel(const ColJobs j, float* __restrict__ scratch, int ns, int stage) {
  __shared__ float red[4][64];
  const int job = blockIdx.z;
  const int lane = threadIdx.x & 63, wave = threadIdx.x >> 6;
  const int C = j.C[job];
  const int c = blockIdx.x * 64 + lane;
  if (blockIdx.x * 64 >= C) return;
  float acc = 0.f;
  if (stage == 0) {
    const long R = j.R[job], rps = (R + ns - 1) / ns;
    const long r0 = (long)blockIdx.y * rps;
    const long r1 = r0 + rps < R ? r0 + rps : R;
    const float* x = j.X[job];
    const float* w = j.w[job];
    const long ld = j.ld[job];
    if (c < C) {
      long r = r0 + wave;
      for (; r + 28 < r1; r += 32) {
        float v[8], wv[8];
#pragma unroll
        for (int u = 0; u < 8; ++u) v[u] = x[(r + 4 * u) * ld + c], wv[u] = w ? w[r + 4 * u] : 1.f;
#pragma unroll
        for (int u = 0; u < 8; ++u) acc = fmaf(wv[u], v[u], acc);
      }
      for (; r < r1; r += 4) acc = fmaf(w ? w[r] : 1.f, x[r * ld + c], acc);
    }
  } else {
    const float* x = scratch + j.part_off[job];
    if (c < C) {
      int r = wave;
      for (; r + 28 < ns; r += 32) {
        float v[8];
#pragma unroll
        for (int u = 0; u < 8; ++u) v[u] = x[(long)(r + 4 * u) * C + c];
#pragma unroll
        for (int u = 0; u < 8; ++u) acc += v[u];
      }
      for (; r < ns; r += 4) acc += x[(long)r * C + c];
    }
  }
  red[wave][lane] = acc;
  __syncthreads();
  if (wave == 0 && c < C) {
    const float s = red[0][lane] + red[1][lane] + red[2][lane] + red[3][lane];
    if (stage == 0) scratch[j.part_off[job] + (long)blockIdx.y * C + c] = s;
    else j.out[job][c] = s;
  }
}

constexpr int FW = 16;
constexpr int FC = 16;
__global__ __launch_bounds__(64 * FW) void gat_fold_fwd_kernel(const float* __restrict__ flat, float* __restrict__ uvc, int D,
                                                               int Dh, uint64_t* rng_state, uint64_t* rng_snaps,
                                                               int rng_count) {
  __shared__ float red[2][64][FC + 1];
  __shared__ float redc[FW];
  if (rng_state && blockIdx.x == 0 && threadIdx.x < 64) {
    const uint64_t seed = rng_state[0], ctr = rng_state[1];
    for (int i = threadIdx.x; i < rng_count; i += 64) rng_snaps[2 * i] = seed, rng_snaps[2 * i + 1] = ctr + (uint64_t)i;
    if (threadIdx.x == 0) rng_state[1] = ctr + (uint64_t)rng_count;
  }
  const long DD = (long)Dh * D;
  const float* Wh = flat;
  const float* bh = Wh + DD;
  const float* Wt = bh + Dh;
  const float* bt = Wt + DD;
  const float* Wr = bt + Dh;
  const float* br = Wr + DD;
  const float* wt = br + Dh;
  const int lane = threadIdx.x & 63, wave = threadIdx.x >> 6;
  const int cl = threadIdx.x & (FC - 1), rl = threadIdx.x >> 4;
  const int k = blockIdx.x * FC + cl;
  float au = 0.f, av = 0.f;
  if (k < D) {
#pragma unroll 4
    for (int d = rl; d < Dh; d += 64) {
      au = fmaf(Wh[(long)d * D + k], wt[d], au);
      au = fmaf(Wt[(long)d * D + k], wt[Dh + d], au);
      av = fmaf(Wr[(long)d * D + k], wt[2 * Dh + d], av);
    }
  }
  red[0][rl][cl] = au;
  red[1][rl][cl] = av;
  __syncthreads();
  if (threadIdx.x < 2 * FC) {
    const int which = threadIdx.x / FC, c = threadIdx.x - which * FC, kk = blockIdx.x * FC + c;
    if (kk < D) {
      float sacc = 0.f;
#pragma unroll 8
      for (int r = 0; r < 64; ++r) sacc += red[which][r][c];
      uvc[which * D + kk] = sacc;
    }
  }
  if (blockIdx.x == 0) {
    float c = 0.f;
    for (int d = threadIdx.x; d < Dh; d += 64 * FW) c += wt[d] * bh[d] + wt[Dh + d] * bt[d] + wt[2 * Dh + d] * br[d];
    c = wave_sum(c);
    if (lane == 0) redc[wave] = c;
    __syncthreads();
    if (threadIdx.x == 0) {
      float tot = wt[3 * Dh];
      for (int w = 0; w < FW; ++w) tot += redc[w];
      uvc[2 * D] = tot;
    }
  }
}

__global__ __launch_bounds__(64 * FW) void gat_fold_bwd_kernel(const float* __restrict__ flat, const float* __restrict__ duvc,
                                                               float* __restrict__ dflat, int D, int Dh,
                                                               const float* __restrict__ part, long off_dv, long off_dc,
                                                               int ns) {
  extern __shared__ float sduvc[];
  if (ns > 0) {
    for (int k = threadIdx.x; k < 2 * D + 1; k += 64 * FW) {
      const float* src = k < D ? part + k : (k < 2 * D ? part + off_dv + (k - D) : part + off_dc);
      const int C = k < 2 * D ? D : 1;
      float a = 0.f;
      int q = 0;
      for (; q + 16 <= ns; q += 16) {
        float v[16];
#pragma unroll
        for (int u = 0; u < 16; ++u) v[u] = src[(long)(q + u) * C];
#pragma unroll
        for (int u = 0; u < 16; ++u) a += v[u];
      }
      for (; q < ns; ++q) a += src[(long)q * C];
      sduvc[k] = a;
    }
    __syncthreads();
    duvc = sduvc;
  }
  const int d = blockIdx.x * FW + (threadIdx.x >> 6);
  if (d >= Dh) return;
  const int lane = threadIdx.x & 63;
  const long DD = (long)Dh * D;
  const long oWh = 0, obh = DD, oWt = obh + Dh, obt = oWt + DD, oWr = obt + Dh, obr = oWr + DD, owt = obr + Dh;
  const float* du = duvc;
  const float* dv = duvc + D;
  const float dc = duvc[2 * D];
  const float wh = flat[owt + d], wtt = flat[owt + Dh + d], wr = flat[owt + 2 * Dh + d];
  float ah = 0.f, at = 0.f, ar = 0.f;
  for (int k = lane; k < D; k += 64) {
    const float u = du[k], v = dv[k];
    dflat[oWh + (long)d * D + k] = wh * u;
    dflat[oWt + (long)d * D + k] = wtt * u;
    dflat[oWr + (long)d * D + k] = wr * v;
    ah = fmaf(flat[oWh + (long)d * D + k], u, ah);
    at = fmaf(flat[oWt + (long)d * D + k], u, at);
    ar = fmaf(flat[oWr + (long)d * D + k], v, ar);
  }
  ah = wave_sum(ah), at = wave_sum(at), ar = wave_sum(ar);
  if (lane == 0) {
    dflat[obh + d] = wh * dc;
    dflat[obt + d] = wtt * dc;
    dflat[obr + d] = wr * dc;
    dflat[owt + d] = ah + flat[obh + d] * dc;
    dflat[owt + Dh + d] = at + flat[obt + d] * dc;
    dflat[owt + 2 * Dh + d] = ar + flat[obr + d] * dc;
    if (d == 0) dflat[owt + 3 * Dh] = dc;
  }
}

__global__ __launch_bounds__(256) void gat_dlogit_kernel(const float* __restrict__ P, const float* __restrict__ dA,
                                                         const float* __restrict__ uvc, const float* __restrict__ dXin,
                                                         float* __restrict__ dlogit, float* __restrict__ ds,
                                                         float* __restrict__ dX, int N, int D, Drop drop) {
  __shared__ float sm[GAT_DOC_LDS];
  gat_dlogit_doc(P, dA, uvc, dXin, dlogit, ds, dX, N, D, drop, blockIdx.x, blockIdx.y, gridDim.y, sm);
}

__global__ __launch_bounds__(64 * RW) void node_score_fwd_kernel(const float* __restrict__ X, const float* __restrict__ uvc,
                                                                 float* __restrict__ s, long M, int D, uint64_t* rng_state,
                                                                 uint64_t* rng_snaps, int rng_count) {
  if (rng_state && blockIdx.x == 0 && threadIdx.x < 64) {
    const uint64_t seed = rng_state[0], ctr = rng_state[1];
    for (int i = threadIdx.x; i < rng_count; i += 64) rng_snaps[2 * i] = seed, rng_snaps[2 * i + 1] = ctr + (uint64_t)i;
    if (threadIdx.x == 0) rng_state[1] = ctr + (uint64_t)rng_count;
  }
  const long m = (long)blockIdx.x * RW + (threadIdx.x >> 6);
  if (m >= M) return;
  const int lane = threadIdx.x & 63;
  float a = 0.f;
  for (int k = lane; k < D; k += 64) a = fmaf(X[m * D + k], uvc[k], a);
  a = wave_sum(a);
  if (lane == 0) s[m] = a + uvc[2 * D];
}

__global__ __launch_bounds__(256) void node_score_bwd_kernel(const float* __restrict__ ds, const float* __restrict__ uvc,
                                                             const float* __restrict__ dXin, float* __restrict__ dX, long M,
                                                             int D) {
  const long e = (long)blockIdx.x * 256 + threadIdx.x;
  if (e >= M * D) return;
  const long m = e / D;
  const float v = ds[m] * uvc[e - m * D];
  dX[e] = dXin ? v + dXin[e] : v;
}

__global__ __launch_bounds__(256) void mask_rows_kernel(const float* __restrict__ x, float* __restrict__ y, long M, int D,
                                                        int N, const int* __restrict__ n_valid, Drop drop, int main_blocks,
                                                        const float* __restrict__ wlin, float* __restrict__ wsum, int H, int vec) {
  if ((int)blockIdx.x >= main_blocks) {
    const int e = (blockIdx.x - main_blocks) * 256 + threadIdx.x;
    if (e < D * D) {
      const int k = e / D, c = e - k * D;
      float s = 0.f;
      for (int h0 = 0; h0 < H; h0 += 8) {
        float v[8];
#pragma unroll
        for (int u = 0; u < 8; ++u) v[u] = wlin[((long)k * H + min(h0 + u, H - 1)) * D + c];
#pragma unroll
        for (int u = 0; u < 8; ++u) s += (h0 + u < H) ? v[u] : 0.f;
      }
      wsum[e] = s;
    }
    return;
  }
  if (vec) {
    const long e = ((long)blockIdx.x * 256 + threadIdx.x) * 4;
    if (e >= M * D) return;
    const long m = e / D;
    const long b = m / N;
    float4 v = *reinterpret_cast<const float4*>(x + e);
    if (n_valid && (int)(m - b * N) >= n_valid[b]) v = make_float4(0.f, 0.f, 0.f, 0.f);
    if (drop.snap) {
      const uint64_t key = drop_key(drop);
      v.x = (rng_u32(key, (uint64_t)e) >= drop.thresh) ? v.x * drop.scale : 0.f;
      v.y = (rng_u32(key, (uint64_t)(e + 1)) >= drop.thresh) ? v.y * drop.scale : 0.f;
      v.z = (rng_u32(key, (uint64_t)(e + 2)) >= drop.thresh) ? v.z * drop.scale : 0.f;
      v.w = (rng_u32(key, (uint64_t)(e + 3)) >= drop.thresh) ? v.w * drop.scale : 0.f;
    }
    *reinterpret_cast<float4*>(y + e) = v;
    return;
  }
  const long e = (long)blockIdx.x * 256 + threadIdx.x;
  if (e >= M * D) return;
  const long m = e / D;
  const long b = m / N;
  float v = (!n_valid || (int)(m - b * N) < n_valid[b]) ? x[e] : 0.f;
  if (drop.snap) v = (rng_u32(drop_key(drop), (uint64_t)e) >= drop.thresh) ? v * drop.scale : 0.f;
  y[e] = v;
}

__global__ __launch_bounds__(256) void row_blocks_kernel(const int* __restrict__ n_valid, int B, int N, int* __restrict__ out) {
  __shared__ int part[256];
  __shared__ int total;
  const int t = threadIdx.x, chunk = (B + 255) / 256, per = N / 16;
  int s = 0;
  for (int b = t * chunk; b < min(B, (t + 1) * chunk); ++b) s += (min(max(n_valid[b], 0), N) + 15) >> 4;
  part[t] = s;
  __syncthreads();
  if (t == 0) {
    int run = 0;
    for (int k = 0; k < 256; ++k) {
      const int v = part[k];
      part[k] = run;
      run += v;
// ... 59 lines not shown
  GC_REQUIRE(drop.snap, "dropout: no rng snapshot");
  if (n == 0) return 0;
  ProfScope ps("dropout", st);
  hipLaunchKernelGGL(dropout_kernel, dim3(cdiv(n, 256)), dim3(256), 0, st, x, y, n, drop);
  return check_launch("dropout");
}
int dropout_keep(unsigned char* keep, long n, Drop drop, hipStream_t st) {
  GC_REQUIRE(drop.snap, "dropout_keep: no rng snapshot");
  if (n == 0) return 0;
  hipLaunchKernelGGL(dropout_keep_kernel, dim3(cdiv(n, 256)), dim3(256), 0, st, keep, n, drop);
  return check_launch("dropout_keep");
}
int rng_next(void* state, void* snaps, int count, hipStream_t st) {
  hipLaunchKernelGGL(rng_next_kernel, dim3(1), dim3(64), 0, st, (uint64_t*)state, (uint64_t*)snaps, count);
  return check_launch("rng_next");
}

constexpr int COLSUM_MIN_ROWS = 32;
constexpr int COLSUM_MAX_SPLITS = 128;
long colsum_scratch_elems(long R, int C, int batch) {
  if (R < 2 * COLSUM_MIN_ROWS) return 0;
  long ns = R / COLSUM_MIN_ROWS;
  if (ns > COLSUM_MAX_SPLITS) ns = COLSUM_MAX_SPLITS;
  return ns * C * batch;
}
int colsum(const float* X, const float* w, float* out, long R, int C, long ld, int batch, long sXz, long sWz, long sOz,
           int accumulate, float* scratch, hipStream_t st) {
  if (C == 0 || batch == 0) return 0;
  long ns = 1;
  if (R >= 2 * COLSUM_MIN_ROWS && scratch) {
    ns = R / COLSUM_MIN_ROWS;
    if (ns > COLSUM_MAX_SPLITS) ns = COLSUM_MAX_SPLITS;
    const long want = 512 / ((long)cdiv(C, 64) * batch) + 1;
    if (ns > want) ns = want;
    if (ns < 2) ns = 1;
  }
  ProfScope ps("colsum", st);
  if (ns == 1) {
    hipLaunchKernelGGL(colsum_kernel, dim3(cdiv(C, 64), 1, batch), dim3(256), 0, st, X, w, out, R, C, ld, sXz, sWz, sOz,
                       R > 0 ? R : 1, accumulate);
    return check_launch("colsum");
  }
  const long rps = (R + ns - 1) / ns;
  hipLaunchKernelGGL(colsum_kernel, dim3(cdiv(C, 64), (unsigned)ns, batch), dim3(256), 0, st, X, w, scratch, R, C, ld, sXz,
                     sWz, ns * C, rps, 0);
  if (int e = check_launch("colsum/1")) return e;
  hipLaunchKernelGGL(colsum_kernel, dim3(cdiv(C, 64), 1, batch), dim3(256), 0, st, scratch, (const float*)nullptr, out, ns, C,
                     (long)C, ns * C, 0L, sOz, ns, accumulate);
  return check_launch("colsum/2");
}

int colsum3(const float* X0, const float* w0, float* o0, long R0, int C0, long ld0, const float* X1, const float* w1,
            float* o1, long R1, int C1, long ld1, const float* X2, const float* w2, float* o2, long R2, int C2, long ld2,
            float* scratch, hipStream_t st, bool stage2, long* part_off, int* ns_out) {
  ColJobs j;
  j.n = 3;
  const float* Xs[3] = {X0, X1, X2};
  const float* ws[3] = {w0, w1, w2};
  float* os[3] = {o0, o1, o2};
  const long Rs[3] = {R0, R1, R2}, lds[3] = {ld0, ld1, ld2};
  const int Cs[3] = {C0, C1, C2};
  const int ns = stage2 ? 64 : 32;
  long off = 0;
  int maxC = 1;
  for (int i = 0; i < 3; ++i) {
    j.X[i] = Xs[i], j.w[i] = ws[i], j.out[i] = os[i], j.R[i] = Rs[i], j.ld[i] = lds[i], j.C[i] = Cs[i];
    j.part_off[i] = off;
    if (part_off) part_off[i] = off;
    off += (long)ns * Cs[i];
    if (Cs[i] > maxC) maxC = Cs[i];
  }
  if (ns_out) *ns_out = ns;
  {
    ProfScope ps("colsum", st);
    hipLaunchKernelGGL(colsum_multi_kernel, dim3(cdiv(maxC, 64), ns, 3), dim3(256), 0, st, j, scratch, ns, 0);
  }
  if (int e = check_launch("colsum3/1")) return e;
  if (!stage2) return 0;
  ProfScope ps("colsum", st);
  hipLaunchKernelGGL(colsum_multi_kernel, dim3(cdiv(maxC, 64), 1, 3), dim3(256), 0, st, j, scratch, ns, 1);
  return check_launch("colsum3/2");
}

int gat_fold_fwd(const float* flat, float* uvc, int D, int Dh, hipStream_t st, void* rng_state, void* rng_snaps,
                 int rng_count) {
  ProfScope ps("gat_fold_fwd", st);
  hipLaunchKernelGGL(gat_fold_fwd_kernel, dim3(cdiv(D, FC)), dim3(64 * FW), 0, st, flat, uvc, D, Dh, (uint64_t*)rng_state,
                     (uint64_t*)rng_snaps, rng_count);
  return check_launch("gat_fold_fwd");
}
int gat_fold_bwd(const float* flat, const float* duvc, float* dflat, int D, int Dh, hipStream_t st, const float* part,
                 const long* part_off, int ns) {
  ProfScope ps("gat_fold_bwd", st);
  const size_t lds = ns > 0 ? sizeof(float) * (2 * (size_t)D + 1) : 0;
  hipLaunchKernelGGL(gat_fold_bwd_kernel, dim3(cdiv(Dh, FW)), dim3(64 * FW), lds, st, flat, duvc, dflat, D, Dh, part,
                     ns > 0 ? part_off[1] : 0L, ns > 0 ? part_off[2] : 0L, ns);
  return check_launch("gat_fold_bwd");
}
int gat_dlogit_slices(int D) { return D >= 256 ? 8 : (D >= 64 ? 4 : 1); }
int gat_dlogit(const float* P, const float* dA, const float* uvc, const float* dXin, float* dlogit, float* ds, float* dX,
               int B, int N, int D, int slices, Drop drop, hipStream_t st) {
  GC_REQUIRE(N <= GT && slices > 0, "gat_dlogit: N=%d slices=%d", N, slices);
  ProfScope ps("gat_dlogit", st);
  hipLaunchKernelGGL(gat_dlogit_kernel, dim3(B, slices), dim3(256), 0, st, P, dA, uvc, dXin, dlogit, ds, dX, N, D, drop);
  return check_launch("gat_dlogit");
}
int node_score_fwd(const float* X, const float* uvc, float* s, long M, int D, hipStream_t st, void* rng_state, void* rng_snaps,
                   int rng_count) {
  ProfScope ps("node_score_fwd", st);
  hipLaunchKernelGGL(node_score_fwd_kernel, dim3(cdiv(M, RW)), dim3(64 * RW), 0, st, X, uvc, s, M, D, (uint64_t*)rng_state,
                     (uint64_t*)rng_snaps, rng_count);
  return check_launch("node_score_fwd");
}
int node_score_bwd(const float* ds, const float* uvc, const float* dXin, float* dX, long M, int D, hipStream_t st) {
  ProfScope ps("node_score_bwd", st);
  hipLaunchKernelGGL(node_score_bwd_kernel, dim3(cdiv(M * D, 256)), dim3(256), 0, st, ds, uvc, dXin, dX, M, D);
  return check_launch("node_score_bwd");
}
int mask_rows(const float* x, float* y, long M, int D, int N, const int* n_valid, Drop drop, hipStream_t st, const float* wlin,
              float* wsum, int H) {
  ProfScope ps("mask_rows", st);
  const int vec = x && D % 4 == 0 && ((((uintptr_t)x) | ((uintptr_t)y)) & 15) == 0;
  const int main_blocks = x ? cdiv(vec ? M * D / 4 : M * D, 256) : 0, extra = wsum ? cdiv((long)D * D, 256) : 0;
  if (main_blocks + extra == 0) return 0;
  hipLaunchKernelGGL(mask_rows_kernel, dim3(main_blocks + extra), dim3(256), 0, st, x, y, M, D, N, n_valid, drop, main_blocks,
                     wlin, wsum, H, vec);
  return check_launch("mask_rows");
}

}
```

### gcgcn_amd/csrc/rowops.hpp

```cpp
#pragma once
#include "common.hpp"

namespace gc {

int softmax_fwd(const float* S, const float* coladd, const int* n_valid, float* P, float* A, long rows, int N, int heads,
                Drop drop, hipStream_t st);
int softmax_bwd(const float* P, const float* dA, float* dS, long rows, int N, Drop drop, hipStream_t st);
int rowsum_inv(const float* A, float* rinv, long rows, int N, hipStream_t st);
int relu_norm_bwd(const float* dY, const float* Y, const float* rinv, float* dM, float* drow, long rows_m, int N, int H,
                  int L, int gh, int l, int first, hipStream_t st, int relu = 1);
struct ColRide;
struct DeferQueue;
int head_sum_drop_bwd(const float* dHO, float* dY, float* dXres, long M, int H, int D, Drop drop, hipStream_t st,
                      const ColRide* finish = nullptr);
int dropout(const float* x, float* y, long n, Drop drop, hipStream_t st);
int dropout_keep(unsigned char* keep, long n, Drop drop, hipStream_t st);
int rng_next(void* state, void* snaps, int count, hipStream_t st);
long colsum_scratch_elems(long R, int C, int batch);
int colsum(const float* X, const float* w, float* out, long R, int C, long ld, int batch, long sXz, long sWz, long sOz,
           int accumulate, float* scratch, hipStream_t st);
int colsum3(const float* X0, const float* w0, float* o0, long R0, int C0, long ld0, const float* X1, const float* w1,
            float* o1, long R1, int C1, long ld1, const float* X2, const float* w2, float* o2, long R2, int C2, long ld2,
            float* scratch, hipStream_t st, bool stage2 = true, long* part_off = nullptr, int* ns_out = nullptr);
int gat_fold_fwd(const float* flat, float* uvc, int D, int Dh, hipStream_t st, void* rng_state = nullptr,
                 void* rng_snaps = nullptr, int rng_count = 0);
int gat_fold_bwd(const float* flat, const float* duvc, float* dflat, int D, int Dh, hipStream_t st,
                 const float* part = nullptr, const long* part_off = nullptr, int ns = 0);
int gat_dlogit_slices(int D);
struct GatTail;
int gat_dlogit(const float* P, const float* dA, const float* uvc, const float* dXin, float* dlogit, float* ds, float* dX,
               int B, int N, int D, int slices, Drop drop, hipStream_t st);
int node_score_fwd(const float* X, const float* uvc, float* s, long M, int D, hipStream_t st, void* rng_state = nullptr,
                   void* rng_snaps = nullptr, int rng_count = 0);
int node_score_bwd(const float* ds, const float* uvc, const float* dXin, float* dX, long M, int D, hipStream_t st);
int mask_rows(const float* x, float* y, long M, int D, int N, const int* n_valid, Drop drop, hipStream_t st,
              const float* wlin = nullptr, float* wsum = nullptr, int H = 0);

int edge_fwd(const float* E, const float* v, const int* n_valid, float* Ebar, const float* coladd, float* P, float* A,
             Drop drop, int B, int N, int D, hipStream_t st, const unsigned char* mask = nullptr);
struct EdgePlan;
int edge_bwd(const float* E, const float* v, const int* n_valid, const float* dlogit, const float* dEbar, float* dE,
             float* dvpart, const EdgePlan& plan, int B, int N, int D, hipStream_t st, DeferQueue* carry = nullptr,
             const GatTail* tail = nullptr);
int edge_bcast(const float* dEbar, const int* n_valid, float* dE, int B, int N, int D, hipStream_t st);

int row_blocks(const int* n_valid, int B, int N, int* out, hipStream_t st);
constexpr int ROWBLK_HDR = 4;
constexpr int ROWBLK_LIST_MAX = 512;
static inline long row_blocks_ints(int B, int N) { return ROWBLK_HDR + (long)B * N / 16; }

int pair_bce_fwd(const float* logits, const float* labels, const int* n_valid, float* loss, float* part, int B, int N, int R,
                 hipStream_t st);
int pair_bce_bwd(const float* logits, const float* labels, const int* n_valid, const float* dloss, float* dlogits, int B, int N,
                 int R, hipStream_t st);
int pair_stats(const float* logits, const float* labels, const int* n_valid, int64_t* counters, int B, int N, int R,
               hipStream_t st);

int64_t eval_ws_bytes(int64_t n_records, int64_t n_keep);
int eval_scan(const float* logits, const float* labels, const uint8_t* in_train, const int* n_valid, const int64_t* doc_base,
              uint64_t* rec, int64_t capacity, int64_t* counters, int B, int N, int R, hipStream_t st);
int eval_rank(const uint64_t* rec, int64_t n, void* ws, int64_t ws_bytes, int64_t* sorted_off, hipStream_t st);
int eval_curve(const uint64_t* keys, int64_t m, const int64_t* counters, double input_theta, float* pr_x, float* pr_y,
               float* ign_pr_y, double* res, void* ws, int64_t ws_bytes, int64_t n_records, hipStream_t st);

}
```

### gcgcn_amd/functional.py

```python
from __future__ import annotations

import ctypes
import os
import threading
import weakref
from dataclasses import dataclass
from typing import Optional

import torch
from torch.autograd.function import once_differentiable

from . import _lib
from ._lib import SALT_GLUE, call

Tensor = torch.Tensor


def _p(t: Optional[Tensor]):
    return None if t is None else t.data_ptr()


_raw_stream = getattr(torch._C, "_cuda_getCurrentRawStream", None)


# ... 73 lines not shown
        with _rng_lock:
            st = _rng_state.setdefault(idx, st)
    return st


def _new_snaps(dev: torch.device, count: int) -> Tensor:
    snaps = torch.empty(count, 2, dtype=torch.int64, device=dev)
    call("gcgcn_rng_next", _p(_state(dev)), _p(snaps), count, _stream())
    return snaps


class rng_scope:

    def __init__(self, dev: torch.device, count: int, enabled: bool = True):
        self.dev, self.count, self.enabled = dev, count, enabled

    def __enter__(self):
        self.prev = _get_scope()
        if self.enabled:
            _tls.scope = [torch.empty(self.count, 2, dtype=torch.int64, device=self.dev), 0, True]
        return self

    def __exit__(self, *exc):
        _tls.scope = self.prev
        return False


def _take_pending_rng(dev: torch.device):
    sc = _get_scope()
    if sc is not None and sc[2] and sc[0].device == dev:
        sc[2] = False
        return _state(dev), sc[0], sc[0].shape[0]
    return None


def rng_snapshot(dev: torch.device, lazy: bool = False) -> Tensor:
    sc = _get_scope()
    if sc is not None and sc[1] < sc[0].shape[0] and sc[0].device == dev:
        if sc[2] and not lazy:
            sc[2] = False
            call("gcgcn_rng_next", _p(_state(dev)), _p(sc[0]), sc[0].shape[0], _stream())
        snap = sc[0][sc[1]]
        sc[1] += 1
        return snap
    return _new_snaps(dev, 1)[0]


def dropout_keep_mask(snap: Tensor, salt: int, p: float, numel: int) -> Tensor:
    keep = torch.empty(numel, dtype=torch.uint8, device=snap.device)
    call("gcgcn_dropout_keep", _p(keep), numel, _p(snap), salt, float(p), _stream())
    return keep.bool()


def _gat_fwd_buffers(x: Tensor, snap, pending, uvc, uvc_valid):
    B, N, D = x.shape
    dev = x.device
    rng = pending if pending is not None else (None, None, 0)
    if uvc is None:
        uvc, uvc_valid = torch.empty(2 * D + 1, device=dev), False
    s = torch.empty(B, N, device=dev)
    P = torch.empty(B, N, N, device=dev)
    A = torch.empty(B, N, N, device=dev) if snap is not None else None
    ebar = torch.empty(B, N, D, device=dev)
    return uvc, uvc_valid, s, P, A, ebar, rng


def _gat_bwd_buffers(x: Tensor, dA, dEbar, dXin, scratch_elems: str):
    B, N, D = x.shape
    dev = x.device
    dA = torch.zeros(B, N, N, device=dev) if dA is None else dA.contiguous()
    dEbar = None if dEbar is None else dEbar.contiguous()
    dXin = None if dXin is None else dXin.contiguous()
    dlogit = torch.empty(B, N, N, device=dev)
    ds = torch.empty(B, N, device=dev)
    dvpart = torch.empty(B * N, D, device=dev)
    duvc = torch.empty(2 * D + 1, device=dev)
    scratch = torch.empty(max(getattr(_lib.lib(), scratch_elems)(B, N, D), 1), device=dev)
    return dA, dEbar, dXin, dlogit, ds, dvpart, duvc, scratch


class GatFn(torch.autograd.Function):

    @staticmethod
    def forward(ctx, x, e, flat, n_valid, p, snap, pending, Dh, mask, uvc, uvc_valid):
        B, N, D = x.shape
        uvc, uvc_valid, s, P, A, ebar, (st, sn, cnt) = _gat_fwd_buffers(x, snap, pending, uvc, uvc_valid)
        call("gcgcn_gat_fwd", B, N, D, Dh, _p(x), _p(e), _p(n_valid), _p(flat), _p(snap), float(p), _p(uvc), _p(s),
             _p(P), _p(A), _p(ebar), _p(st), _p(sn), cnt, _p(mask), 1 if uvc_valid else 0, _stream())
        ctx.save_for_backward(x, e, flat, uvc, P)
        ctx.n_valid, ctx.p, ctx.snap, ctx.Dh, ctx.mask = n_valid, float(p), snap, Dh, mask
        return (P if A is None else A), ebar, x.view_as(x)

    @staticmethod
    def backward(ctx, dA, dEbar, dXin):
        x, e, flat, uvc, P = ctx.saved_tensors
        B, N, D = x.shape
        dev = x.device
        dA, dEbar, dXin, dlogit, ds, dvpart, duvc, scratch = _gat_bwd_buffers(x, dA, dEbar, dXin, "gcgcn_gat_bwd_scratch")
        if ctx.mask is not None:
            gone = ctx.mask.bool()
            if ctx.n_valid is not None:
                gone = gone | (torch.arange(N, device=dev)[None, None, :] >= ctx.n_valid[:, None, None])
            dA = dA.masked_fill(gone.all(-1, keepdim=True), 0.0)
        dX = torch.empty_like(x)
        dE = torch.empty_like(e) if ctx.needs_input_grad[1] else None
        dflat = torch.empty_like(flat)
        bp = _current_pass()
        call("gcgcn_gat_bwd", B, N, D, ctx.Dh, _p(x), _p(e), _p(ctx.n_valid), _p(flat), _p(ctx.snap), ctx.p, _p(uvc), _p(P),
             _p(dA), _p(dEbar), _p(dXin), _p(dX), _p(dE), _p(dflat), _p(dlogit), _p(ds), _p(dvpart), _p(duvc),
             _p(scratch), None if bp is None else bp.queue, _stream())
        return dX, dE, dflat, None, None, None, None, None, None, None, None


class EdgeMeanFn(torch.autograd.Function):

    @staticmethod
    def forward(ctx, e, n_valid):
        B, N, _, D = e.shape
        ebar = torch.empty(B, N, D, device=e.device)
        call("gcgcn_edge_mean_fwd", B, N, D, _p(e), _p(n_valid), _p(ebar), _stream())
        ctx.n_valid, ctx.shape = n_valid, (B, N, D)
        return ebar

    @staticmethod
    def backward(ctx, dEbar):
        B, N, D = ctx.shape
        dEbar = dEbar.contiguous()
        dE = torch.empty(B, N, N, D, device=dEbar.device)
        call("gcgcn_edge_mean_bwd", B, N, D, _p(dEbar), _p(ctx.n_valid), _p(dE), _stream())
        return dE, None


class MhaFn(torch.autograd.Function):

    @staticmethod
    def forward(ctx, x, flat, n_valid, H, p, snap, rowblk=None):
        B, N, D = x.shape
        dev = x.device
        Q = torch.empty(B, N, D, device=dev)
        P = torch.empty(B, H, N, N, device=dev)
        A = torch.empty(B, H, N, N, device=dev) if snap is not None else None
        scratch = torch.empty(max(_lib.lib().gcgcn_mha_scratch(B, N, D), 1), device=dev)
        call("gcgcn_mha_fwd", B, N, D, H, _p(x), _p(n_valid), _p(flat), _p(snap), float(p), _p(Q), _p(P), _p(A),
             _p(scratch), _p(rowblk), _stream())
        ctx.save_for_backward(x, flat, Q, P)
        ctx.H, ctx.p, ctx.snap, ctx.rowblk = H, float(p), snap, rowblk
        return (P if A is None else A), x.view_as(x)

    @staticmethod
    def backward(ctx, dA, dXin):
        x, flat, Q, P = ctx.saved_tensors
        B, N, D = x.shape
        H, dev = ctx.H, x.device
        dA = torch.zeros(B, H, N, N, device=dev) if dA is None else dA.contiguous()
        dXin = None if dXin is None else dXin.contiguous()
        dX = torch.empty_like(x)
        dflat = torch.empty_like(flat)
        dS = torch.empty(B, H, N, N, device=dev)
        dQ = torch.empty(B, N, D, device=dev)
        scratch = torch.empty(max(_lib.lib().gcgcn_mha_scratch(B, N, D), 1), device=dev)
        call("gcgcn_mha_bwd", B, N, D, H, _p(x), _p(flat), _p(ctx.snap), ctx.p, _p(Q), _p(P), _p(dA), _p(dXin), _p(dX),
             _p(dflat), _p(dS), _p(dQ), _p(scratch), None, 0, _p(ctx.rowblk), _stream())
        return dX, dflat, None, None, None, None, None


defer_weight_grads = os.environ.get("GCGCN_DEFER", "1") != "0"
defer_fused_mha_weight_grads = os.environ.get("GCGCN_DEFER_MHA", "1") != "0"
_warned_ddp = [False]


def _under_ddp() -> bool:
    ddp = getattr(torch.nn.parallel, "DistributedDataParallel", None)
    if ddp is not None and not hasattr(ddp, "_active_ddp_module"):
        import torch.distributed as dist
        on = dist.is_available() and dist.is_initialized() and dist.get_world_size() > 1
    else:
        on = ddp is not None and getattr(ddp, "_active_ddp_module", None) is not None
    if on and defer_weight_grads and not _warned_ddp[0]:
        _warned_ddp[0] = True
        import warnings
        warnings.warn("gcgcn_amd: running under torch DistributedDataParallel -- deferred weight gradients are switched off "
                      "for these blocks (their AccumulateGrad hooks need the gradient during backward); "
                      "gcgcn_amd.dist.FlatGradBucket reduces the flat gradients without that cost")
    return on
_passes = {}
_passes_lock = threading.Lock()


class _BackwardPass:
    def __init__(self, task_id: int):
        self.task_id = task_id
        self.queue = _lib.lib().gcgcn_defer_create()
        if not self.queue:
            raise MemoryError("gcgcn_defer_create failed")
        self.keep = []
        self.installs = []

    def park(self, leaf, dflat, operands):
        self.keep.append(operands)
        self.installs.append((leaf, dflat))

    def __call__(self):
        with _passes_lock:
            _passes.pop(self.task_id, None)
        try:
            if _lib.lib().gcgcn_defer_count(self.queue) > 0:
                call("gcgcn_defer_flush", self.queue, _stream())
            with torch.no_grad():
                for leaf, dflat in self.installs:
                    if leaf.grad is None:
                        leaf.grad = dflat
                    else:
                        leaf.grad.add_(dflat)
        finally:
            self.keep.clear()
            self.installs.clear()

    def __del__(self):
        q, self.queue = self.queue, None
        if q:
            try:
                _lib.lib().gcgcn_defer_destroy(q)
            except Exception:
                pass


def _current_pass() -> Optional[_BackwardPass]:
    tid = torch._C._current_graph_task_id()
    if tid < 0:
        return None
    ref = _passes.get(tid)
    return None if ref is None else ref()


def _pass_for_parking(ctx, idx: int, leaf=None) -> Optional[_BackwardPass]:
    if not (defer_weight_grads and ctx.needs_input_grad[idx]):
        return None
    leaf = ctx.flat_leaf if leaf is None else leaf
    if leaf is None or leaf._post_accumulate_grad_hooks or leaf._backward_hooks:
        return None
    tid = torch._C._current_graph_task_id()
    if tid < 0:
        return None
    try:
        acc = ctx.next_functions[idx][0]
        if acc is None or getattr(acc, "variable", None) is not leaf or torch._C._will_engine_execute_node(acc) is not True:
            return None
    except RuntimeError:
        return None
    with _passes_lock:
        ref = _passes.get(tid)
        bp = None if ref is None else ref()
        if bp is None:
            bp = _BackwardPass(tid)
            _passes[tid] = weakref.ref(bp)
            torch.autograd.Variable._execution_engine.queue_callback(bp)
            for k in [k for k, r in _passes.items() if r() is None]:
                del _passes[k]
    return bp


def _ride(inp, n_valid, out, B, N, D):
    r = _lib.EdgeRide(B, N, D, inp.data_ptr(), None if n_valid is None else n_valid.data_ptr(), out.data_ptr())
    return r, ctypes.cast(ctypes.pointer(r), ctypes.c_void_p)


head_sum_in_forward = True


def _gcn_forward(ctx, x, ebar, adj, flat, n_valid, L, H, p, snap, e_next, out_p, out_snap, rowblk, hook=None, saved=()):
    B, N, D = x.shape
    dev = x.device
    HD = H * D
    out = torch.empty(B, N, D, device=dev)
    Pn, Y, HO = (torch.empty(B, N, HD, device=dev) for _ in range(3))
    if hook is None:
        rinv = torch.empty(B, H, N, device=dev)
        G = torch.empty(B, N, HD, device=dev)
    else:
        G = torch.empty(B, N, HD, device=dev)
        rinv = torch.empty(B, H, N, device=dev)
    wsum = torch.empty(D, D, device=dev) if (H > 1 and head_sum_in_forward and any(ctx.needs_input_grad[:4])) else None
    scratch = torch.empty(max(_lib.lib().gcgcn_gcn_scratch(B, N, D, H), 1), device=dev)
    ebar_next, ride, ride_p = None, None, None
    if e_next is not None:
        ebar_next = torch.empty(e_next.shape[0], e_next.shape[1], e_next.shape[3], device=dev)
        ride, ride_p = _ride(e_next, n_valid, ebar_next, *ebar_next.shape)
    call("gcgcn_gcn_fwd", B, N, D, L, H, _p(x), _p(ebar), None if hook is not None else _p(adj), _p(n_valid), _p(flat), _p(snap),
         float(p), _p(out_snap), float(out_p), _p(out), _p(Pn), _p(Y), _p(HO), _p(rinv), _p(G), _p(wsum), _p(scratch), ride_p,
         None if hook is None else ctypes.cast(ctypes.pointer(hook), ctypes.c_void_p), _p(rowblk), _stream())
    del ride
    ctx.save_for_backward(x, ebar, adj, flat, Pn, Y, HO, rinv, *saved)
    ctx.wsum, ctx.rowblk, ctx.n_valid, ctx.L, ctx.H = wsum, rowblk, n_valid, L, H
    ctx.p, ctx.snap, ctx.out_p, ctx.out_snap = float(p), snap, float(out_p), out_snap
    ctx.flat_leaf = flat if (flat.is_leaf and not _under_ddp()) else None
    ctx.next_shape = None if e_next is None else tuple(e_next.shape)
    return out, ebar_next


def _gcn_backward(ctx, dout, debar_next, e_next_input, mha_hook=None):
    x, ebar, adj, flat, Pn, Y, HO, rinv = ctx.saved_tensors[:8]
    B, N, D = x.shape
    L, H, dev = ctx.L, ctx.H, x.device
    HD = H * D
    dout = dout.contiguous()
    dX, dEbar = torch.empty_like(x), torch.empty_like(ebar)
    dA = torch.empty_like(adj)
    dflat = torch.empty_like(flat)
    W1, W2, W3 = (torch.empty(B, N, HD, device=dev) for _ in range(3))
    drow = torch.empty(B, H, N, device=dev)
    dXres = torch.empty(B, N, D, device=dev)
    dout_m = torch.empty(B, N, D, device=dev) if (ctx.n_valid is not None or ctx.out_snap is not None) else None
    scratch = torch.empty(max(_lib.lib().gcgcn_gcn_scratch(B, N, D, H), 1), device=dev)
    dQ = None if mha_hook is None else torch.empty(B, N, D, device=dev)
    hook = None if mha_hook is None else mha_hook(dQ)
    dE_next, ride, ride_p = None, None, None
    if ctx.next_shape is not None and ctx.needs_input_grad[e_next_input] and debar_next is not None:
        debar_next = debar_next.contiguous()
        dE_next = torch.empty(ctx.next_shape, device=dev)
        ride, ride_p = _ride(debar_next, ctx.n_valid, dE_next, *debar_next.shape)
    bp = _pass_for_parking(ctx, 3)
    call("gcgcn_gcn_bwd", B, N, D, L, H, _p(x), _p(ebar), _p(adj), _p(ctx.n_valid), _p(flat), _p(ctx.snap),
         ctx.p, _p(ctx.out_snap), ctx.out_p, _p(Pn), _p(Y), _p(HO), _p(rinv), _p(ctx.wsum), _p(dout), _p(dX), _p(dEbar), _p(dA),
         _p(dflat), _p(W1), _p(W2), _p(W3), _p(drow), _p(dXres), _p(dout_m), _p(scratch), ride_p,
         None if hook is None else ctypes.cast(ctypes.pointer(hook), ctypes.c_void_p),
         None if bp is None else bp.queue, _p(ctx.rowblk), _stream())
    del ride, hook
    if bp is not None:
        bp.park(ctx.flat_leaf, dflat, (x, ebar, Y, HO, dout, dout_m, W2, W3, ctx.rowblk))
        dflat = None
    return dX, dEbar, dA, dflat, dE_next, dQ


class GcnFn(torch.autograd.Function):

    @staticmethod
    def forward(ctx, x, ebar, adj, flat, n_valid, L, H, p, snap, e_next, out_p, out_snap, rowblk=None):
        return _gcn_forward(ctx, x, ebar, adj, flat, n_valid, L, H, p, snap, e_next, out_p, out_snap, rowblk)

    @staticmethod
    def backward(ctx, dout, debar_next):
        dX, dEbar, dA, dflat, dE_next, _ = _gcn_backward(ctx, dout, debar_next, 9)
        return dX, dEbar, dA, dflat, None, None, None, None, None, dE_next, None, None, None


class MaggcFn(torch.autograd.Function):

    @staticmethod
    def forward(ctx, x, ebar, flat_mha, flat, n_valid, L, H, p_mha, snap_mha, p, snap, e_next, out_p, out_snap, rowblk=None):
        B, N, D = x.shape
        dev = x.device
        Q = torch.empty(B, N, D, device=dev)
        P = torch.empty(B, H, N, N, device=dev)
        A = torch.empty(B, H, N, N, device=dev) if snap_mha is not None else None
        hook = _lib.MhaHook(flat_mha.data_ptr(), Q.data_ptr(), P.data_ptr(), _p(A), None, _p(snap_mha), float(p_mha))
        ctx.p_mha, ctx.snap_mha = float(p_mha), snap_mha
        ctx.flat_mha_leaf = flat_mha if (flat_mha.is_leaf and not _under_ddp()) else None
        return _gcn_forward(ctx, x, ebar, P if A is None else A, flat, n_valid, L, H, p, snap, e_next, out_p, out_snap, rowblk,
                            hook=hook, saved=(flat_mha, Q, P))

    @staticmethod
    def backward(ctx, dout, debar_next):
        x, flat_mha, Q, P = ctx.saved_tensors[0], *ctx.saved_tensors[8:]
        B, N, D = x.shape
        H, dev = ctx.H, x.device
        dXc, dEbar, dA, dflat, dE_next, dQ = _gcn_backward(
            ctx, dout, debar_next, 11, lambda dQ: _lib.MhaHook(None, Q.data_ptr(), P.data_ptr(), None, dQ.data_ptr(), _p(ctx.snap_mha), ctx.p_mha))
        dX = torch.empty_like(x)
        dflat_mha = torch.empty_like(flat_mha)
        dS = torch.empty(1, device=dev)
# ... 331 lines not shown
    feats = [_chk(f, f"node_feats[{i}]", 3) for i, f in enumerate(feats)]
    B, N, Hd = feats[0].shape
    if any(tuple(f.shape) != (B, N, Hd) for f in feats):
        raise ValueError("node_feats: every entry must have the same [B,N,H] shape")
    for nm, t, shp in (("node_type", node_type, (B, N)), ("node_relative_pos", node_relative_pos, (B, N, N))):
        if not t.is_cuda or t.dtype != torch.int64 or tuple(t.shape) != shp:
            raise ValueError(f"{nm}: expected a GPU int64 tensor of shape {shp}, got {t.dtype} {tuple(t.shape)} on {t.device}")
    if ner_emb.dim() != 2 or ner_emb.shape[0] != NER_ROWS:
        raise ValueError(f"ner_emb.weight: the head indexes {NER_ROWS} rows (nn.Embedding(7, .), glove:241), got {tuple(ner_emb.shape)}")
    if dis_table.dim() != 2 or dis_table.shape[0] < 2 * int(dis_plus) + 1:
        raise ValueError(f"dis_embed.weight: needs at least 2 * dis_plus + 1 = {2 * int(dis_plus) + 1} rows, got {tuple(dis_table.shape)}")
    if dis_table.shape[0] > HEAD_MAX_DIS_ROWS:
        raise ValueError(f"dis_embed.weight: the head handles at most {HEAD_MAX_DIS_ROWS} rows of the distance table (its backward "
                         f"pass keeps one sum per id in LDS), got {tuple(dis_table.shape)}")
    _check_id_range([("node_type", node_type, 0, NER_ROWS - 1),
                     ("node_relative_pos", node_relative_pos, -int(dis_plus), int(dis_plus))])
    return HEAD_MATMUL[matmul].apply(_chk(flat, "flat"), _chk(ner_emb, "ner_emb.weight", 2), _chk(dis_table, "dis_embed.weight", 2),
                                     node_type.contiguous(), node_relative_pos.contiguous(), _nv(n_valid, B, N, flat.device),
                                     int(relation_num), int(dis_plus), *feats)


def producer_live_counts(sen: Tensor, n_valid=None):
    B, N, _, S, T = sen.shape
    counts = torch.empty(2, dtype=torch.int32, device=sen.device)
    call("gcgcn_producer_count", B, N, S, T, _p(sen), _p(n_valid), _p(counts), _stream())
    r, q = counts.tolist()
    return r, q


check_position_ids = False


class ProducerCapacityError(RuntimeError):
    """max_live_slots / max_live_pairs were smaller than what the batch holds."""


def edge_features(tok, sen, pos_h, pos_t, node, dis_table, flat, n_valid=None, max_live_slots=None, max_live_pairs=None,
                  check_capacity=False, return_counts=False, compact=False, deterministic=False):
    tok, node, dis_table = _chk(tok, "context_output", 3), _chk(node, "node_feat", 3), _chk(dis_table, "dis_embed.weight", 2)
    B, T, Hd = tok.shape
    if sen.dim() != 5 or sen.shape[0] != B or sen.shape[4] != T or sen.shape[1] != sen.shape[2]:
        raise ValueError(f"sen_matrix: expected [B={B}, N, N, S, T={T}], got {tuple(sen.shape)}")
    N, S = sen.shape[1], sen.shape[3]
    if node.shape != (B, N, Hd):
        raise ValueError(f"node_feat: expected {(B, N, Hd)}, got {tuple(node.shape)}")
    if not sen.is_cuda:
        raise RuntimeError("sen_matrix: gcgcn_amd runs on MI355X only (no CPU fallback)")
    if sen.dtype == torch.bool:
        sen = sen.view(torch.uint8)
    elif sen.dtype != torch.uint8:
        sen = (sen != 0).to(torch.uint8)
    sen = sen.contiguous()
    for nm, p in (("pos_matrix_h", pos_h), ("pos_matrix_t", pos_t)):
        if tuple(p.shape) != tuple(sen.shape) or p.dtype not in (torch.int64, torch.int32, torch.uint8) or not p.is_cuda:
            raise ValueError(f"{nm}: expected a GPU int64 / int32 / uint8 tensor of shape {tuple(sen.shape)}")
    if pos_t.dtype != pos_h.dtype:
        raise ValueError("pos_matrix_h and pos_matrix_t must have the same dtype")
    if check_position_ids:
        _check_id_range([("pos_matrix_h", pos_h, 0, dis_table.shape[0] - 1), ("pos_matrix_t", pos_t, 0, dis_table.shape[0] - 1)])
    nv = _nv(n_valid, B, N, tok.device)
    given = max_live_slots is not None and max_live_pairs is not None
    if not given:
        r, q = producer_live_counts(sen, nv)
        max_live_slots = r if max_live_slots is None else max_live_slots
        max_live_pairs = q if max_live_pairs is None else max_live_pairs
    out = ProducerFn.apply(tok, node, dis_table, _chk(flat, "flat"), sen, pos_h.contiguous(), pos_t.contiguous(), nv,
                           int(max_live_slots), int(max_live_pairs), bool(compact), bool(deterministic))
    if compact:
        E, counts = (out[0], out[2]), out[1]
    else:
        E, counts = out
    if check_capacity and not torch.cuda.is_current_stream_capturing():
        if int(counts[2].item()) != 0:
            raise ProducerCapacityError(f"edge_features: max_live_slots={max_live_slots} / max_live_pairs={max_live_pairs} are "
                                        "smaller than the batch's live sentence slots / entity pairs (producer_live_counts "
                                        "reports both); nothing was computed")
    return (E, counts) if return_counts else E


def _snap_for(training: bool, p: float, dev) -> Optional[Tensor]:
    return rng_snapshot(dev) if (training and p > 0.0) else None


def gat_attention(x, e, flat, n_valid=None, p=0.1, training=False, hidden_dim=None, mask=None, uvc=None, uvc_valid=False):
    x, e = _chk(x, "node_feat", 3), _chk(e, "edge_feat", 4)
    B, N, D = x.shape
    if e.shape != (B, N, N, D):
        raise ValueError(f"edge_feat: expected {(B, N, N, D)}, got {tuple(e.shape)}")
    nv = _nv(n_valid, B, N, x.device)
    snap = rng_snapshot(x.device, lazy=True) if (training and p > 0.0) else None
    if mask is not None:
        if not mask.is_cuda or tuple(mask.shape) != (B, N, N):
            raise ValueError(f"mask: expected a GPU tensor of shape {(B, N, N)}, got {tuple(mask.shape)} on {mask.device}")
        mask = (mask != 0).to(torch.uint8).contiguous()
    return GatFn.apply(x, e, _chk(flat, "flat"), nv, p, snap, _take_pending_rng(x.device),
                       D if hidden_dim is None else int(hidden_dim), mask, uvc, bool(uvc_valid))


def gat_attention_compact(x, ce: CompactEdges, flat, n_valid=None, p=0.1, training=False, hidden_dim=None, uvc=None, uvc_valid=False):
    x = _chk(x, "node_feat", 3)
    B, N, D = x.shape
    if tuple(ce.prow.shape) != (B, N, N) or ce.Ec.shape[1] != D:
        raise ValueError(f"compact edge_feat: pairs {tuple(ce.prow.shape)} / width {ce.Ec.shape[1]} do not match node_feat {tuple(x.shape)}")
    nv = _nv(n_valid, B, N, x.device)
    snap = rng_snapshot(x.device, lazy=True) if (training and p > 0.0) else None
    return GatCompactFn.apply(x, _chk(ce.Ec, "Ec", 2), _chk(ce.bias, "bias", 1), _chk(flat, "flat"), ce.prow, nv, p, snap,
                              _take_pending_rng(x.device), D if hidden_dim is None else int(hidden_dim), uvc, bool(uvc_valid))


def edge_mean_compact(ce: CompactEdges, n_valid=None):
    B, N, _ = ce.prow.shape
    return EdgeMeanCompactFn.apply(_chk(ce.Ec, "Ec", 2), _chk(ce.bias, "bias", 1), ce.prow, _nv(n_valid, B, N, ce.Ec.device))


def edge_mean(e, n_valid=None):
    if isinstance(e, CompactEdges):
        return edge_mean_compact(e, n_valid)
    e = _chk(e, "edge_feat", 4)
    B, N = e.shape[0], e.shape[1]
    return EdgeMeanFn.apply(e, _nv(n_valid, B, N, e.device))


def multi_head_adjacency(x, flat, H, n_valid=None, p=0.1, training=False, rowblk=None):
    x = _chk(x, "node_feat", 3)
    B, N, D = x.shape
    return MhaFn.apply(x, _chk(flat, "flat"), _nv(n_valid, B, N, x.device), H, p, _snap_for(training, p, x.device), rowblk)


def gcn_stack(x, ebar, adj, flat, L, H, n_valid=None, p=0.2, training=False, e_next=None, out_dropout=0.0, rowblk=None):
    x, ebar, adj = _chk(x, "node_feat", 3), _chk(ebar, "edge_mean", 3), _chk(adj, "adjacency", 4)
    B, N, D = x.shape
    if ebar.shape != (B, N, D) or adj.shape != (B, H, N, N):
        raise ValueError(f"gcn_stack: shapes x{tuple(x.shape)} ebar{tuple(ebar.shape)} adj{tuple(adj.shape)} H={H}")
    nv = _nv(n_valid, B, N, x.device)
    if e_next is not None:
        e_next = _chk(e_next, "next edge_feat", 4)
        if e_next.shape[:3] != (B, N, N):
            raise ValueError(f"gcn_stack: next edge tensor {tuple(e_next.shape)} does not match B={B} N={N}")
    snap = _snap_for(training, p, x.device)
    out_snap = _snap_for(training, out_dropout, x.device)
    if rowblk is None:
        rowblk = row_blocks(nv, B, N)
    out, ebar_next = GcnFn.apply(x, ebar, adj, _chk(flat, "flat"), nv, L, H, p, snap, e_next,
                                 out_dropout if out_snap is not None else 0.0, out_snap, rowblk)
    return out if e_next is None else (out, ebar_next)


def maggc_fusable(x: Tensor, H: int) -> bool:
    return x.is_cuda and x.dim() == 3 and bool(_lib.lib().gcgcn_maggc_fusable(x.shape[1], x.shape[2], int(H)))


def maggc_hop(x, ebar, flat_mha, flat, L, H, n_valid=None, p_mha=0.1, p=0.2, training=False, e_next=None, out_dropout=0.0, rowblk=None):
    x, ebar = _chk(x, "node_feat", 3), _chk(ebar, "edge_mean", 3)
    B, N, D = x.shape
    if ebar.shape != (B, N, D):
        raise ValueError(f"maggc_hop: shapes x{tuple(x.shape)} ebar{tuple(ebar.shape)}")
    nv = _nv(n_valid, B, N, x.device)
    if e_next is not None:
        e_next = _chk(e_next, "next edge_feat", 4)
    snap_mha = _snap_for(training, p_mha, x.device)
    snap = _snap_for(training, p, x.device)
    out_snap = _snap_for(training, out_dropout, x.device)
    if rowblk is None:
        rowblk = row_blocks(nv, B, N)
    out, ebar_next = MaggcFn.apply(x, ebar, _chk(flat_mha, "flat"), _chk(flat, "flat"), nv, L, H, p_mha, snap_mha, p, snap, e_next,
                                   out_dropout if out_snap is not None else 0.0, out_snap, rowblk)
    return out if e_next is None else (out, ebar_next)


def graph_conv(x, ebar, adj, we, wn, bias=None):
    x, ebar, adj = _chk(x, "inputs", 3), _chk(ebar, "edge_mean", 3), _chk(adj, "adjacency_matrix", 3)
    return GraphConvFn.apply(x, ebar, adj, _chk(we, "weights_edge", 2), _chk(wn, "weights_node", 2),
                             None if bias is None else _chk(bias, "bias", 1))


def dropout(x, p=0.2, training=False, salt=SALT_GLUE):
    x = _chk(x, "x")
    if not training or p <= 0.0:
        return x
# ... 636 lines not shown
```

### gcgcn_amd/modules.py

```python
from __future__ import annotations

from typing import Dict, List, Optional, Sequence, Union

import torch
from torch import nn

from . import functional as F_
from . import params as P_

Tensor = torch.Tensor


class _FlatBlock(nn.Module):

    def _ref_tensors(self) -> Dict[str, Tensor]:
        raise NotImplementedError

    def _load_ref(self, sd: Dict[str, Tensor]):
        raise NotImplementedError

    def _ref_shapes(self) -> Dict[str, tuple]:
        raise NotImplementedError

    def named_tensors(self) -> Dict[str, Tensor]:
# ... 2 lines not shown

    def named_grads(self) -> Dict[str, Optional[Tensor]]:
        raise NotImplementedError

    def _save_to_state_dict(self, destination, prefix, keep_vars):
        for k, v in self.named_tensors().items():
            destination[prefix + k] = v.detach().clone()

    def _load_from_state_dict(self, state_dict, prefix, local_metadata, strict, missing_keys, unexpected_keys,
                              error_msgs):
        shapes = self._ref_shapes()
        got = {}
        for k, shp in shapes.items():
            key = prefix + k
            if key not in state_dict:
                missing_keys.append(key)
                continue
            v = state_dict[key]
            if tuple(v.shape) != tuple(shp):
                error_msgs.append(f"size mismatch for {key}: copying a param with shape {tuple(v.shape)} from "
                                  f"checkpoint, the shape in current model is {tuple(shp)}.")
                continue
            got[k] = v
        if strict:
            for key in state_dict.keys():
                if key.startswith(prefix) and key[len(prefix):] not in shapes:
                    unexpected_keys.append(key)
        if got:
            with torch.no_grad():
                dev = self.flat.device
                full = {k: v.to(device=dev, dtype=torch.float32) for k, v in got.items()}
                if len(got) < len(shapes):
                    cur = self._ref_tensors()
                    full = {k: full.get(k, cur[k]) for k in shapes}
                self._load_ref(full)


def _batched(x: Tensor, nd: int):
    if x.dim() == nd:
        return x.unsqueeze(0), False
    if x.dim() == nd + 1:
        return x, True
    raise ValueError(f"expected {nd} or {nd + 1} dims, got shape {tuple(x.shape)}")


class GATAttention(_FlatBlock):

    def __init__(self, att_input_dim: int, hidden_dim: int, dropout: float = 0.1, apply_mask: bool = False):
        super().__init__()
        self.dim = att_input_dim
        self.hidden_dim = hidden_dim
        self.apply_mask = bool(apply_mask)
        self.cache_fold = "infer"
        self._uvc = None
        self.p = float(dropout) if dropout is not None else 0.0
        self.flat = nn.Parameter(torch.empty(P_.gat_layout(self.dim, hidden_dim)[-1]))
        with torch.no_grad():
            P_.pack_gat(P_.init_gat(self.dim, hidden_dim), self.dim, self.flat, hidden_dim)

    def _ref_shapes(self):
        return P_.gat_shapes(self.dim, self.hidden_dim)

    def _ref_tensors(self):
        return P_.unpack_gat(self.flat.detach(), self.dim, self.hidden_dim)

    def _load_ref(self, sd):
        P_.pack_gat(sd, self.dim, self.flat, self.hidden_dim)

    def named_grads(self):
        return P_.unpack_gat(self.flat.grad, self.dim, self.hidden_dim) if self.flat.grad is not None else {}

    def invalidate_fold(self):
        self._uvc = None

    def _apply(self, fn, *args, **kwargs):
        self._uvc = None
        return super()._apply(fn, *args, **kwargs)

    def _load_from_state_dict(self, *args, **kwargs):
        self._uvc = None
        return super()._load_from_state_dict(*args, **kwargs)

    def forward(self, node_feat: Tensor, edge_feat: Tensor, mask: Optional[Tensor] = None,
                n_valid: Optional[Tensor] = None, return_input_alias: bool = False) -> Tensor:
        x, batched = _batched(node_feat, 2)
        compact = isinstance(edge_feat, F_.CompactEdges)
        if compact and self.apply_mask:
            raise ValueError("GATAttention(apply_mask=True) needs the dense edge tensor (CompactEdges.dense())")
        e = edge_feat if compact else _batched(edge_feat, 3)[0]
        mk = None
        if self.apply_mask and mask is not None:
            mk, _ = _batched(mask, 2)
        uvc, valid = None, False
        use_cache = (not (self.training and torch.is_grad_enabled())) if self.cache_fold == "infer" else bool(self.cache_fold)
        if use_cache and x.is_cuda and not torch.cuda.is_current_stream_capturing():
            key = (self.flat._version, self.flat.data_ptr(), x.device)
            if self._uvc is not None and self._uvc[0] == key:
                uvc, valid = self._uvc[1], True
            else:
                uvc = torch.empty(2 * self.dim + 1, device=x.device)
                self._uvc = (key, uvc)
        if compact:
            a, ebar, xa = F_.gat_attention_compact(x, e, self.flat, n_valid, self.p, self.training, hidden_dim=self.hidden_dim,
                                                   uvc=uvc, uvc_valid=valid)
        else:
            a, ebar, xa = F_.gat_attention(x, e, self.flat, n_valid, self.p, self.training, hidden_dim=self.hidden_dim,
                                           mask=mk, uvc=uvc, uvc_valid=valid)
        F_.park_edge_mean(edge_feat, n_valid, ebar)
        a = a if batched else a.squeeze(0)
        return (a, xa if batched else xa.squeeze(0)) if return_input_alias else a


class MultiHeadAttention(_FlatBlock):

    def __init__(self, head_num: int, att_size: int, dropout: float = 0.1):
        super().__init__()
        assert att_size % head_num == 0
        self.hidden_size = att_size // head_num
        self.head_num = head_num
        self.dim = att_size
        self.p = float(dropout) if dropout is not None else 0.0
        n = P_.mha_layout(att_size)[-1]
        self.flat = nn.Parameter(torch.empty(n))
        self.flat_k = nn.Parameter(torch.empty(n))
        with torch.no_grad():
            P_.pack_mha(P_.init_mha(att_size, head_num, "q"), att_size, head_num, self.flat, "q")
            P_.pack_mha(P_.init_mha(att_size, head_num, "k"), att_size, head_num, self.flat_k, "k")

    def _ref_shapes(self):
        dh, D = self.hidden_size, self.dim
        s = {}
        for w in ("q", "k"):
            for h in range(self.head_num):
                s[f"linears_{w}.{h}.weight"] = (dh, D)
                s[f"linears_{w}.{h}.bias"] = (dh,)
        return s

    def _ref_tensors(self):
        d = P_.unpack_mha(self.flat.detach(), self.dim, self.head_num, "q")
        d.update(P_.unpack_mha(self.flat_k.detach(), self.dim, self.head_num, "k"))
        return d

    def _load_ref(self, sd):
        P_.pack_mha(sd, self.dim, self.head_num, self.flat, "q")
        P_.pack_mha(sd, self.dim, self.head_num, self.flat_k, "k")

    def named_grads(self):
        if self.flat.grad is None:
            return {}
        return P_.unpack_mha(self.flat.grad, self.dim, self.head_num, "q")

    def forward(self, node_feat: Tensor, mask: Optional[Tensor] = None, n_valid: Optional[Tensor] = None,
                return_input_alias: bool = False, rowblk: Optional[Tensor] = None) -> List[Tensor]:
        x, batched = _batched(node_feat, 2)
        a, xa = F_.multi_head_adjacency(x, self.flat, self.head_num, n_valid, self.p, self.training, rowblk=rowblk)
        heads = list(a.unbind(1)) if batched else list(a.squeeze(0).unbind(0))
        return (heads, xa if batched else xa.squeeze(0)) if return_input_alias else heads


class _GcnBase(_FlatBlock):
    def _setup(self, layer_num: int, head_num: int, input_dim: int, output_dim: int, bias: bool):
        if input_dim != output_dim:
            raise ValueError("residual connection needs input_dim == output_dim (glove:76)")
        if output_dim % layer_num != 0:
            raise ValueError("output_dim must be divisible by layer_num (glove:58,76)")
        self.input_dim = input_dim
        self.layer_num = layer_num
        self.head_num = head_num
        self.dim = output_dim
        self.p = 0.2
        self.flat = nn.Parameter(torch.empty(P_.gcn_layout(self.dim, layer_num, head_num)[5]))
        with torch.no_grad():
            P_.pack_gcn(P_.init_gcn(self.dim, layer_num, head_num), self.dim, layer_num, head_num, self.flat)

    def _ref_shapes(self):
        return P_.gcn_shapes(self.dim, self.layer_num, self.head_num)

    def _ref_tensors(self):
        return P_.unpack_gcn(self.flat.detach(), self.dim, self.layer_num, self.head_num)

    def _load_ref(self, sd):
        P_.pack_gcn(sd, self.dim, self.layer_num, self.head_num, self.flat)

    def named_grads(self):
        if self.flat.grad is None:
            return {}
        return P_.unpack_gcn(self.flat.grad, self.dim, self.layer_num, self.head_num)

    def _edge_mean(self, edge_feat: Tensor, n_valid) -> Tensor:
        ebar = F_.take_edge_mean(edge_feat, n_valid)
# ... 163 lines not shown

class ClassifierHead(_FlatBlock):

    def __init__(self, hidden_size: int = 128, graph_hop: int = 2, entity_type_size: int = 20, dis_size: int = 20,
                 relation_num: int = 97, dis_plus: int = 10, matmul: str = "fp32"):
        super().__init__()
        if matmul not in F_.HEAD_MATMUL:
            raise ValueError(f"ClassifierHead: matmul must be 'fp32' or 'bf16', got {matmul!r}")
        self.matmul = matmul
        self.hidden, self.nf, self.pt, self.pr, self.R, self.dis_plus = hidden_size, graph_hop + 1, entity_type_size, dis_size, \
            relation_num, dis_plus
        self.flat = nn.Parameter(torch.zeros(P_.head_layout(*self._dims())[-1]))
        with torch.no_grad():
            P_.pack_head(P_.init_head(*self._dims()), *self._dims(), self.flat)

    def _dims(self):
        return self.hidden, self.nf, self.pt, self.pr, self.R

    def _ref_shapes(self):
        s = P_.head_shapes(*self._dims())
        return {k: s[k] for k in P_.HEAD_STATE_ORDER}

    def _ref_tensors(self):
        return P_.unpack_head(self.flat.detach(), *self._dims())

    def _load_ref(self, sd):
        P_.pack_head(sd, *self._dims(), self.flat)

    def named_grads(self):
        return P_.unpack_head(self.flat.grad, *self._dims()) if self.flat.grad is not None else {}

    def forward(self, node_feats: Sequence[Tensor], node_type: Tensor, node_relative_pos: Tensor, ner_emb_weight: Tensor,
                dis_embed_weight: Tensor, n_valid: Optional[Tensor] = None) -> Tensor:
        if len(node_feats) != self.nf:
            raise ValueError(f"node_feats: expected {self.nf} tensors (graph_hop + 1), got {len(node_feats)}")
        batched = node_feats[0].dim() == 3
        if not batched:
            node_feats = [f.unsqueeze(0) for f in node_feats]
            node_type, node_relative_pos = node_type.unsqueeze(0), node_relative_pos.unsqueeze(0)
        out = F_.classifier_head(node_feats, node_type, node_relative_pos, ner_emb_weight, dis_embed_weight, self.flat, self.R,
                                 n_valid, self.dis_plus, matmul=self.matmul)
        return out if batched else out.squeeze(0)


class GraphHops(nn.Module):

    def __init__(self, hidden_size: int = 128, layer_num: int = 2, head_num: int = 8, graph_hop: int = 2,
                 alpha: float = 1.0, dropout: float = 0.2, apply_mask: bool = False):
        super().__init__()
        self.graph_hop, self.alpha, self.p = graph_hop, float(alpha), float(dropout)
        self.get_weighted_adj_matrix = GATAttention(hidden_size, hidden_size, apply_mask=apply_mask)
        self.get_adj_matrix = nn.ModuleList([MultiHeadAttention(head_num, hidden_size) for _ in range(graph_hop - 1)])
        self.graphcnn = nn.ModuleList()
        for i in range(graph_hop):
            if i == 0:
                self.graphcnn.append(GraphConvolution(layer_num, hidden_size, hidden_size))
            else:
                self.graphcnn.append(MultiGraphConvolution(layer_num, head_num, hidden_size, hidden_size))

    def forward(self, node_feat: Tensor, edge_feats: Sequence[Tensor], adj_matrix: Optional[Tensor] = None,
                n_valid: Optional[Tensor] = None) -> List[Tensor]:
        feats = [node_feat]
        x = node_feat
        with F_.rng_scope(node_feat.device, 3 * self.graph_hop, enabled=self.training and node_feat.is_cuda):
            return self._hops(x, feats, edge_feats, adj_matrix, n_valid)

    def _hops(self, x, feats, edge_feats, adj_matrix, n_valid):
        def ride(i):
            on = self.ride_edge_mean and x.is_cuda and i + 1 < self.graph_hop
            return edge_feats[i + 1] if on else None

        fused_out = self.alpha == 1.0 and x.is_cuda
        odrop = self.p if (fused_out and self.training) else 0.0
        rb = None
        if n_valid is not None and x.is_cuda and x.dim() == 3:
            rb = F_.row_blocks(n_valid, x.shape[0], x.shape[1])

        for i in range(self.graph_hop):
            e = edge_feats[i]
            if i < 1:
                mask = None
                if self.get_weighted_adj_matrix.apply_mask and adj_matrix is not None:
                    mask = torch.eq(adj_matrix, 0)
                a, xa = self.get_weighted_adj_matrix(x, e, mask, n_valid=n_valid, return_input_alias=True)
                new = self.graphcnn[i](xa, e, a, n_valid=n_valid, ride_edge=ride(i), out_dropout=odrop, rowblk=rb)
            else:
                if self.fuse_maggc:
                    new = self.graphcnn[i].forward_with_attention(self.get_adj_matrix[i - 1], x, e, n_valid=n_valid,
                                                                  ride_edge=ride(i), out_dropout=odrop, rowblk=rb)
                else:
                    al, xa = self.get_adj_matrix[i - 1](x, e, n_valid=n_valid, return_input_alias=True, rowblk=rb)
                    new = self.graphcnn[i](xa, e, al, n_valid=n_valid, ride_edge=ride(i), out_dropout=odrop, rowblk=rb)
            if fused_out:
                x = new
            else:
                x = self.alpha * new + (1 - self.alpha) * x
                x = F_.dropout(x, self.p, self.training)
            feats.append(x)
        return feats

    ride_edge_mean = True
    fuse_maggc = True


class GraphModelTail(nn.Module):

    def __init__(self, hidden_size: int = 128, layer_num: int = 2, head_num: int = 8, graph_hop: int = 2, alpha: float = 1.0,
                 dis_size: int = 20, entity_type_size: int = 20, relation_num: int = 97, dis_plus: int = 10, dropout: float = 0.2,
                 head_matmul: str = "fp32"):
        super().__init__()
        self.graph_hop, self.alpha, self.p = graph_hop, float(alpha), float(dropout)
        self.producers = nn.ModuleList([EdgeFeatureProducer(hidden_size, dis_size) for _ in range(graph_hop)])
        self.get_weighted_adj_matrix = GATAttention(hidden_size, hidden_size)
        self.get_adj_matrix = nn.ModuleList([MultiHeadAttention(head_num, hidden_size) for _ in range(graph_hop - 1)])
        self.graphcnn = nn.ModuleList([GraphConvolution(layer_num, hidden_size, hidden_size) if i == 0 else
                                       MultiGraphConvolution(layer_num, head_num, hidden_size, hidden_size) for i in range(graph_hop)])
        self.head = ClassifierHead(hidden_size, graph_hop, entity_type_size, dis_size, relation_num, dis_plus, matmul=head_matmul)
        self._install_key_hooks()

    _PROD_MODS = tuple(sorted(set(k.split(".", 1)[0] for k in P_.producer_shapes(1, 1))))
    _HEAD_MODS = tuple(sorted(set(k.split(".", 1)[0] for k in P_.HEAD_STATE_ORDER)))

    @staticmethod
    def _to_model_key(k: str) -> str:
        p = k.split(".")
        if p[0] == "producers":
            return ".".join([p[2], p[1]] + p[3:])
        if p[0] == "head":
            return ".".join(p[1:])
        return k

    @classmethod
    def _to_module_key(cls, k: str) -> str:
        p = k.split(".")
        if p[0] in cls._PROD_MODS and len(p) > 2 and p[1].isdigit():
            return ".".join(["producers", p[1], p[0]] + p[2:])
        if p[0] in cls._HEAD_MODS:
            return "head." + k
        return k

    @staticmethod
    def _rename_keys(sd, prefix: str, fn):
        items = list(sd.items())
        sd.clear()
        for k, v in items:
            sd[prefix + fn(k[len(prefix):]) if k.startswith(prefix) else k] = v

    @staticmethod
    def _state_dict_hook(module, state_dict, prefix, local_metadata):
        module._rename_keys(state_dict, prefix, module._to_model_key)

    def _load_pre_hook(self, state_dict, prefix, local_metadata, strict, missing_keys, unexpected_keys, error_msgs):
        self._rename_keys(state_dict, prefix, self._to_module_key)

    def _install_key_hooks(self):
        self._register_state_dict_hook(self._state_dict_hook)
        self._register_load_state_dict_pre_hook(self._load_pre_hook)

    skip_dead_hop = False
    compact_edges = False
    deterministic = False

    def forward(self, context_output: Tensor, node_feat: Tensor, adj_matrix: Optional[Tensor], sen_matrix: Tensor,
                pos_matrix_h: Tensor, pos_matrix_t: Tensor, node_type: Tensor, node_relative_pos: Tensor,
                dis_embed_weight: Tensor, ner_emb_weight: Tensor, n_valid: Optional[Tensor] = None,
                max_live_slots: Optional[int] = None, max_live_pairs: Optional[int] = None) -> Tensor:
        x = node_feat
        feats = [x]
# ... 29 lines not shown
```

### include/gcgcn.h

```cpp
#ifndef GCGCN_H
#define GCGCN_H
#include <stdint.h>

#ifdef __cplusplus
extern "C" {
#endif

int gcgcn_version(void);
const char* gcgcn_last_error(void);

int gcgcn_set_option(const char* name, int value);

int64_t gcgcn_row_blocks_ints(int B, int N);
int gcgcn_row_blocks(int B, int N, const int32_t* n_valid, int32_t* out, void* stream);

int gcgcn_prof_start(const char* kernel_prefix, int capacity);
int gcgcn_prof_enable(int on);
int gcgcn_prof_stop(double* total_ms, int* launches, double* work);

int gcgcn_rng_next(void* state, void* snaps, int count, void* stream);
int gcgcn_dropout_keep(uint8_t* keep, int64_t n, const void* rng_snap, uint64_t salt, float p, void* stream);
int gcgcn_dropout(const float* x, float* y, int64_t n, const void* rng_snap, uint64_t salt, float p, void* stream);

#define GCGCN_SALT_GAT 0x47415431ull
#define GCGCN_SALT_MHA 0x4d484131ull
#define GCGCN_SALT_GCN 0x47434e31ull
#define GCGCN_SALT_GLUE 0x474c5531ull

int gcgcn_gat_layout(int D, int Dh, int64_t* out9);

int gcgcn_gat_fwd(int B, int N, int D, int Dh, const float* X, const float* E, const int32_t* n_valid, const float* flat,
                  const void* rng_snap, float p, float* uvc, float* s, float* P, float* A, float* Ebar, void* rng_state,
                  void* rng_snaps, int rng_count, const uint8_t* mask, int uvc_valid, void* stream);

int64_t gcgcn_gat_bwd_scratch(int B, int N, int D);
int gcgcn_gat_bwd(int B, int N, int D, int Dh, const float* X, const float* E, const int32_t* n_valid, const float* flat,
                  const void* rng_snap, float p, const float* uvc, const float* P, const float* dA, const float* dEbar,
                  const float* dX_in, float* dX, float* dE, float* dflat, float* dlogit, float* ds, float* dvpart,
                  float* duvc, float* scratch, void* defer_queue, void* stream);

int gcgcn_edge_mean_fwd(int B, int N, int D, const float* E, const int32_t* n_valid, float* Ebar, void* stream);
int gcgcn_edge_mean_bwd(int B, int N, int D, const float* dEbar, const int32_t* n_valid, float* dE, void* stream);

int gcgcn_mha_layout(int D, int64_t* out3);
int64_t gcgcn_mha_scratch(int B, int N, int D);
int gcgcn_mha_fwd(int B, int N, int D, int H, const float* X, const int32_t* n_valid, const float* flat,
                  const void* rng_snap, float p, float* Q, float* P, float* A, float* scratch, const int32_t* rowblk, void* stream);
int gcgcn_mha_bwd(int B, int N, int D, int H, const float* X, const float* flat, const void* rng_snap, float p,
                  const float* Q, const float* P, const float* dA, const float* dX_in, float* dX, float* dflat,
                  float* dS, float* dQ, float* scratch, void* defer_queue, int core_done, const int32_t* rowblk, void* stream);

int gcgcn_gcn_layout(int D, int L, int H, int64_t* out7);
int64_t gcgcn_gcn_scratch(int B, int N, int D, int H);
typedef struct gcgcn_edge_ride {
  int32_t B, N, D;
  const float* in;
  const int32_t* n_valid;
  float* out;
} gcgcn_edge_ride;
typedef struct gcgcn_mha_hook {
  const float* flat_q;
  float* Q;
  float* P;
  float* A;
  float* dQ;
  const void* rng_snap;
  float p;
} gcgcn_mha_hook;
int gcgcn_maggc_fusable(int N, int D, int H);
int gcgcn_gcn_fwd(int B, int N, int D, int L, int H, const float* X, const float* Ebar, const float* A,
                  const int32_t* n_valid, const float* flat, const void* rng_snap, float p, const void* out_rng_snap,
                  float out_p, float* out, float* Pn, float* Y, float* HO, float* rinv, float* G, float* wsum, float* scratch,
                  const gcgcn_edge_ride* ride, const gcgcn_mha_hook* mha, const int32_t* rowblk, void* stream);
int gcgcn_gcn_bwd(int B, int N, int D, int L, int H, const float* X, const float* Ebar, const float* A,
                  const int32_t* n_valid, const float* flat, const void* rng_snap, float p, const void* out_rng_snap,
                  float out_p, const float* Pn, const float* Y, const float* HO, const float* rinv, const float* wsum,
                  const float* dout, float* dX, float* dEbar,
                  float* dA, float* dflat, float* W1, float* W2, float* W3, float* drow, float* dXres, float* dout_m,
                  float* scratch, const gcgcn_edge_ride* ride, const gcgcn_mha_hook* mha, void* defer_queue, const int32_t* rowblk,
                  void* stream);
void* gcgcn_defer_create(void);
void gcgcn_defer_destroy(void* queue);
int gcgcn_defer_count(const void* queue);
int gcgcn_defer_flush(void* queue, void* stream);

int gcgcn_graphconv_fwd(int B, int N, int Din, int De, int Dout, const float* X, const float* Ebar, const float* A,
                        const float* We, const float* Wn, const float* bias, float* out, float* T, float* rinv,
                        float* scratch, void* stream);
int gcgcn_graphconv_bwd(int B, int N, int Din, int De, int Dout, const float* X, const float* Ebar, const float* A,
                        const float* We, const float* Wn, const float* out, const float* T, const float* rinv,
                        const float* dout, float* dX, float* dEbar, float* dA, float* dWe, float* dWn, float* dbias,
                        float* dS, float* dT, float* drow, float* scratch, void* stream);

int gcgcn_pair_bce_fwd(int B, int N, int R, const float* logits, const float* labels, const int32_t* n_valid, float* loss,
                       float* part, void* stream);
int gcgcn_pair_bce_bwd(int B, int N, int R, const float* logits, const float* labels, const int32_t* n_valid,
                       const float* dloss, float* dlogits, void* stream);
int gcgcn_pair_stats(int B, int N, int R, const float* logits, const float* labels, const int32_t* n_valid, int64_t* counters,
                     void* stream);

int64_t gcgcn_eval_ws_bytes(int64_t n_records, int64_t n_keep);
int gcgcn_eval_scan(int B, int N, int R, const float* logits, const float* labels, const uint8_t* in_train, const int32_t* n_valid,
                    const int64_t* doc_base, uint64_t* records, int64_t capacity, int64_t* counters, void* stream);
int gcgcn_eval_rank(const uint64_t* records, int64_t n, void* ws, int64_t ws_bytes, int64_t* sorted_off, void* stream);
int gcgcn_eval_curve(const uint64_t* ranked, int64_t m, int64_t n_records, const int64_t* counters, double input_theta,
                     float* pr_x, float* pr_y, float* ign_pr_y, double* result, void* ws, int64_t ws_bytes, void* stream);

int gcgcn_producer_layout(int Hd, int P, int64_t* out17);
int gcgcn_producer_count(int B, int N, int S, int T, const uint8_t* sen, const int32_t* n_valid, int32_t* counts2, void* stream);
int gcgcn_producer_sizes(int B, int N, int S, int T, int Hd, int P, int ND, int64_t cap_rows, int64_t cap_pairs, int64_t* out7);
int gcgcn_producer_fwd(int B, int N, int S, int T, int Hd, int P, int ND, const float* ctx, const uint8_t* sen, const void* pos_h,
                       const void* pos_t, int pos_bytes, const float* node, const float* dis_table, const int32_t* n_valid,
                       const float* flat, int64_t cap_rows, int64_t cap_pairs, int32_t* ibuf, float* fbuf, float* scratch,
                       int64_t scratch_elems, float* E, void* stream);
int gcgcn_producer_bwd(int B, int N, int S, int T, int Hd, int P, int ND, const float* ctx, const uint8_t* sen, const void* pos_h,
                       const void* pos_t, int pos_bytes, const float* node, const float* dis_table, const int32_t* n_valid,
                       const float* flat, int64_t cap_rows, int64_t cap_pairs, int32_t* ibuf, float* fbuf, float* bbuf,
                       const float* dE, const float* dEc, float* dctx, float* dnode, float* ddis_table, float* dflat, void* stream);
int gcgcn_producer_det_elems(int B, int N, int Hd, int64_t cap_pairs, int64_t* out);
int gcgcn_producer_bwd_det(int B, int N, int S, int T, int Hd, int P, int ND, const float* ctx, const uint8_t* sen, const void* pos_h,
                           const void* pos_t, int pos_bytes, const float* node, const float* dis_table, const int32_t* n_valid,
                           const float* flat, int64_t cap_rows, int64_t cap_pairs, int32_t* ibuf, float* fbuf, float* bbuf,
                           const float* dE, const float* dEc, float* dctx, float* dnode, float* ddis_table, float* dflat,
                           float* detbuf, int64_t det_elems, void* stream);

int gcgcn_edge_mean_fwd_compact(int B, int N, int D, const float* Ec, const int32_t* prow, const float* bias, const int32_t* n_valid,
                                float* Ebar, void* stream);
int gcgcn_edge_mean_bwd_compact(int B, int N, int D, const int32_t* prow, const int32_t* n_valid, const float* dEbar, float* dEc,
                                float* dbias, float* rowbuf, void* stream);
int gcgcn_gat_fwd_compact(int B, int N, int D, int Dh, const float* X, const float* Ec, const int32_t* prow, const float* bias,
                          const int32_t* n_valid, const float* flat, const void* rng_snap, float p, float* uvc, float* s, float* P,
                          float* A, float* Ebar, void* rng_state, void* rng_snaps, int rng_count, int uvc_valid, void* stream);
int64_t gcgcn_gat_bwd_compact_scratch(int B, int N, int D);
int gcgcn_gat_bwd_compact(int B, int N, int D, int Dh, const float* X, const float* Ec, const int32_t* prow, const float* bias,
                          const int32_t* n_valid, const float* flat, const void* rng_snap, float p, const float* uvc, const float* P,
                          const float* dA, const float* dEbar, const float* dX_in, float* dX, float* dEc, float* dbias, float* dflat,
                          float* dlogit, float* ds, float* dvpart, float* duvc, float* scratch, void* stream);

// ... 148 lines not shown
```

Baseline: 65640 docs/s.

## Compute early rows of next layer's edge mean inside GAT fold and score launches

Extra blocks are appended to the GAT fold and node-score kernels so they compute the first rows of the next hop's edge mean, which normally rides on the GCN chain kernel. The chain kernel then starts its riding rows at an offset r0. A cost model chooses how many rows go into each early launch. The aim is to fill idle CUs in the small fold/score launches and shorten the chain launch's tail. In exchange it adds LDS use and wider blocks to those kernels, plus thread-local state that hands the partial result between modules.

```diff
diff --git a/gcgcn_amd/_lib.py b/gcgcn_amd/_lib.py
--- a/gcgcn_amd/_lib.py
+++ b/gcgcn_amd/_lib.py
@@ -10,6 +10,7 @@
 HEADER_PATH = os.path.join(os.path.dirname(_HERE), "include", "gcgcn.h")
 OPTIM_HEADER_PATH = os.path.join(os.path.dirname(_HERE), "include", "gcgcn_optim.h")
 BERT_EMBED_HEADER_PATH = os.path.join(os.path.dirname(_HERE), "include", "gcgcn_bert_embed.h")
+RIDE_HEADER_PATH = os.path.join(os.path.dirname(_HERE), "include", "gcgcn_ride.h")
 
 ABI_VERSION = 7
 
@@ -31,7 +32,7 @@
 
 
 class EdgeRide(ctypes.Structure):
-    _fields_ = [("B", ctypes.c_int32), ("N", ctypes.c_int32), ("D", ctypes.c_int32),
+    _fields_ = [("B", ctypes.c_int32), ("N", ctypes.c_int32), ("D", ctypes.c_int32), ("r0", ctypes.c_int32),
                 ("inp", c_void_p), ("n_valid", c_void_p), ("out", c_void_p)]
 
 
@@ -39,6 +40,7 @@
 _DECL = re.compile(r"([\w\s*]+?)\b(gcgcn_\w+)\s*\(([^()]*)\)")
 _DECL_OPTIM = re.compile(r"([\w\s*]+?)\b(gcopt_\w+)\s*\(([^()]*)\)")
 _DECL_BERT_EMBED = re.compile(r"([\w\s*]+?)\b(gcbe_\w+)\s*\(([^()]*)\)")
+_DECL_RIDE = re.compile(r"([\w\s*]+?)\b(gcride_\w+)\s*\(([^()]*)\)")
 _STRUCT = re.compile(r"typedef\s+struct\s+(\w+)\s*\{([^{}]*)\}\s*\1\s*;")
 
 
@@ -112,9 +114,20 @@
     return sigs
 
 
+def _load_ride_header():
+    if not os.path.exists(RIDE_HEADER_PATH):
+        raise RuntimeError(f"gcgcn_amd: {RIDE_HEADER_PATH} not found. The binding is derived from the C headers of the source tree.")
+    with open(RIDE_HEADER_PATH) as f:
+        sigs, structs = _parse_header(f.read(), _DECL_RIDE, "include/gcgcn_ride.h")
+    if structs:
+        raise RuntimeError(f"gcgcn_amd: include/gcgcn_ride.h declares structs {list(structs)}; it takes plain arguments only")
+    return sigs
+
+
 SIGNATURES = _load_header()
 OPTIM_SIGNATURES = _load_optim_header()
 BERT_EMBED_SIGNATURES = _load_bert_embed_header()
+RIDE_SIGNATURES = _load_ride_header()
 
 _lib = None
 
@@ -127,7 +140,8 @@
                 f"gcgcn_amd: {LIB_PATH} not found. Build it with `make -C gcgcn_amd/csrc` "
                 "(or `python -c 'import __graft_entry__ as g; g.build()'`). There is no CPU fallback.")
         handle = ctypes.CDLL(LIB_PATH)
-        for name, (res, args) in list(SIGNATURES.items()) + list(OPTIM_SIGNATURES.items()) + list(BERT_EMBED_SIGNATURES.items()):
+        for name, (res, args) in list(SIGNATURES.items()) + list(OPTIM_SIGNATURES.items()) + list(BERT_EMBED_SIGNATURES.items()) + \
+                list(RIDE_SIGNATURES.items()):
             fn = getattr(handle, name)
             fn.restype = res
             fn.argtypes = args
diff --git a/gcgcn_amd/csrc/api.hip b/gcgcn_amd/csrc/api.hip
--- a/gcgcn_amd/csrc/api.hip
+++ b/gcgcn_amd/csrc/api.hip
@@ -1,4 +1,5 @@
 #include "../../include/gcgcn.h"
+#include "../../include/gcgcn_ride.h"
 
 #include <stdarg.h>
 #include <string.h>
@@ -10,6 +11,7 @@
 
 #include "attn_plan.hpp"
 #include "compact.hpp"
+#include "edge_body.hpp"
 #include "gat_body.hpp"
 #include "gemm.hpp"
 #include "lstm.hpp"
@@ -108,7 +110,8 @@
 static Opt g_opts[] = {{"head_v1", 0, false},      {"head_bil3", 0, false}, {"head_bil3_bwd", 0, false}, {"head_dw3", 0, false},
                        {"head_compact", 0, false}, {"chain_t", 0, false},   {"chain_big", 0, false},     {"split_widen", 0, false},
                        {"chain", 0, false},        {"mha_core", 0, false},  {"group_dump", 0, false},
-                       {"bf16_rows", 0, false}};
+                       {"bf16_rows", 0, false},
+                       {"ride_early", 0, false}};
 int option(const char* name, int dflt) {
   for (Opt& o : g_opts) {
     if (strcmp(o.name, name) != 0) continue;
@@ -165,6 +168,8 @@
              ride->B, ride->N, ride->D);
   GC_REQUIRE((long)ride->B * ride->N <= 0x3fffffffL, "%s: edge ride too large", who);
   r.kind = kind, r.B = ride->B, r.N = ride->N, r.D = ride->D;
+  r.r0 = kind == 1 ? ride->r0 : 0;
+  GC_REQUIRE(r.r0 >= 0 && r.r0 <= ride->B * ride->N, "%s: edge ride starts at row %d of %d", who, r.r0, ride->B * ride->N);
   r.in = ride->in, r.n_valid = ride->n_valid, r.out = ride->out;
   return 0;
 }
@@ -206,12 +211,20 @@
 };
 
 static int gat_node_fwd(const float* X, const float* flat, float* uvc, float* s, long M, int D, int Dh, int uvc_valid, void* rng_state,
-                        void* rng_snaps, int rng_count, hipStream_t st) {
+                        void* rng_snaps, int rng_count, hipStream_t st, const EarlyRows* early = nullptr, int r_fold = 0,
+                        int r_score = 0) {
+  EarlyRows ef, es;
+  memset(&ef, 0, sizeof ef), memset(&es, 0, sizeof es);
+  if (early) {
+    ef = es = *early;
+    ef.first = 0, ef.count = uvc_valid ? 0 : r_fold;
+    es.first = ef.count, es.count = r_fold + r_score - ef.count;
+  }
   if (!uvc_valid) {
-    GC_TRY(gat_fold_fwd(flat, uvc, D, Dh, st, rng_state, rng_snaps, rng_count));
-    return node_score_fwd(X, uvc, s, M, D, st);
-  }
-  return node_score_fwd(X, uvc, s, M, D, st, rng_state, rng_snaps, rng_count);
+    GC_TRY(gat_fold_fwd(flat, uvc, D, Dh, st, rng_state, rng_snaps, rng_count, &ef));
+    return node_score_fwd(X, uvc, s, M, D, st, nullptr, nullptr, 0, &es);
+  }
+  return node_score_fwd(X, uvc, s, M, D, st, rng_state, rng_snaps, rng_count, &es);
 }
 
 static int gat_bwd(const EdgeOperand& eo, int B, int N, int D, int Dh, const float* X, const int* n_valid, const float* flat, Drop drop,
@@ -385,6 +398,35 @@
   GC_REQUIRE(!drop.snap || A, "gat_fwd: dropout on but A is NULL");
   GC_REQUIRE(!rng_state || (rng_snaps && rng_count > 0), "gat_fwd: rng_state given without snapshots to fill");
   GC_TRY(gat_node_fwd(X, flat, uvc, s, (long)B * N, D, Dh, uvc_valid, rng_state, rng_snaps, rng_count, st));
+  return edge_fwd(E, uvc + D, n_valid, Ebar, s, P, A, drop, B, N, D, st, mask);
+}
+
+int gcride_debug_plan(int B, int N, int D, int pairs, int gh, int L, int present, int misalign, int32_t* out2) {
+  GC_REQUIRE(out2, "ride_debug_plan: null pointer");
+  const RideEarlyPlan p = ride_early_plan({B, N, D, pairs, gh, L, present != 0,
+                                           ((misalign & 1) ? (unsigned)EDGE_MIS_E : 0u) | ((misalign & 2) ? (unsigned)EDGE_MIS_EBAR : 0u)});
+  out2[0] = p.r_fold, out2[1] = p.r_score;
+  return 0;
+}
+
+int gcride_gat_fwd(int B, int N, int D, int Dh, const float* X, const float* E, const int32_t* n_valid, const float* flat,
+                   const void* rng_snap, float p, float* uvc, float* s, float* P, float* A, float* Ebar, void* rng_state,
+                   void* rng_snaps, int rng_count, const uint8_t* mask, int uvc_valid, const float* E_next, int D_next,
+                   float* ebar_next, int r_fold, int r_score, void* stream) {
+  hipStream_t st = (hipStream_t)stream;
+  GC_TRY(check_dims("ride_gat_fwd", B, N, D, 1, 1));
+  GC_REQUIRE(Dh > 0, "ride_gat_fwd: hidden_dim=%d", Dh);
+  GC_REQUIRE(X && E && flat && uvc && s && P && Ebar, "ride_gat_fwd: null pointer");
+  GC_REQUIRE(E_next && ebar_next && D_next > 0, "ride_gat_fwd: no passenger");
+  GC_REQUIRE(r_fold >= 0 && r_score >= 0 && (long)r_fold + r_score <= (long)B * N, "ride_gat_fwd: rows %d + %d of %ld", r_fold, r_score,
+             (long)B * N);
+  GC_REQUIRE(D_next % 4 == 0 && !edge_misalign(E_next, nullptr, nullptr, nullptr, ebar_next), "ride_gat_fwd: the passenger needs 16-byte rows");
+  GC_REQUIRE(ride_early_lds(D_next) <= RIDE_EARLY_LDS_MAX, "ride_gat_fwd: D_next=%d needs %zu B of LDS", D_next, ride_early_lds(D_next));
+  const Drop drop = make_drop(rng_snap, GCGCN_SALT_GAT, p);
+  GC_REQUIRE(!drop.snap || A, "ride_gat_fwd: dropout on but A is NULL");
+  GC_REQUIRE(!rng_state || (rng_snaps && rng_count > 0), "ride_gat_fwd: rng_state given without snapshots to fill");
+  const EarlyRows er{E_next, n_valid, ebar_next, N, D_next, 0, r_fold + r_score};
+  GC_TRY(gat_node_fwd(X, flat, uvc, s, (long)B * N, D, Dh, uvc_valid, rng_state, rng_snaps, rng_count, st, &er, r_fold, r_score));
   return edge_fwd(E, uvc + D, n_valid, Ebar, s, P, A, drop, B, N, D, st, mask);
 }
 
diff --git a/gcgcn_amd/csrc/chain.hip b/gcgcn_amd/csrc/chain.hip
--- a/gcgcn_amd/csrc/chain.hip
+++ b/gcgcn_amd/csrc/chain.hip
@@ -24,6 +24,7 @@
 constexpr int XCHG_LDS = 64 * 64;
 typedef float f32x4 __attribute__((ext_vector_type(4)));
 constexpr int CW = 8;
+static_assert(CW == RIDE_W, "a riding row is summed by the same number of waves in the chain and in the early launches");
 constexpr int RB = 8;
 
 template <bool AKC, bool BKC, bool ALIGNED, int MASK, int RT>
@@ -74,7 +75,7 @@
   if (blockIdx.x >= c.B * c.H) {
     const EdgeRide& r = c.ride;
     edge_fwd_row<4, false, CW>(r.in, nullptr, r.n_valid, r.out, nullptr, nullptr, nullptr, Drop(), r.N, r.D,
-                               blockIdx.x - c.B * c.H, lds);
+                               blockIdx.x - c.B * c.H + r.r0, lds);
     return;
   }
   const int z = blockIdx.x;
@@ -217,7 +218,7 @@
   if (blockIdx.x >= c.B * c.H) {
     const EdgeRide& r = c.ride;
     edge_fwd_row<4, false, CW>(r.in, nullptr, r.n_valid, r.out, nullptr, nullptr, nullptr, Drop(), r.N, r.D,
-                               blockIdx.x - c.B * c.H, lds);
+                               blockIdx.x - c.B * c.H + r.r0, lds);
     return;
   }
   TS(0);
@@ -741,7 +742,7 @@
 }
 bool chain_can_carry(const EdgeRide& r) {
   return r.kind != 0 && r.D % 4 == 0 && al16(r.in) && al16(r.out) && (long)CW * r.D <= CHAIN_LDS &&
-         (long)r.B * r.N <= 0x3fffffffL;
+         (long)r.B * r.N <= 0x3fffffffL && r.r0 >= 0 && r.r0 <= r.B * r.N && (r.kind == 1 || r.r0 == 0);
 }
 
 static ChainPlan chain_pick(const ChainQuery& q, bool bwd, bool ride) {
@@ -770,7 +771,7 @@
 }
 
 static unsigned chain_grid(const GcnCtx& c, int kind) {
-  return (unsigned)(c.B * c.H) + (c.ride.kind == kind ? (unsigned)(c.ride.B * c.ride.N) : 0u);
+  return (unsigned)(c.B * c.H) + (c.ride.kind == kind ? (unsigned)(c.ride.B * c.ride.N - c.ride.r0) : 0u);
 }
 
 int gcn_chain_fwd(const GcnCtx& c, const ChainPlan& p, hipStream_t st) {
diff --git a/gcgcn_amd/csrc/chain_t.hpp b/gcgcn_amd/csrc/chain_t.hpp
--- a/gcgcn_amd/csrc/chain_t.hpp
+++ b/gcgcn_amd/csrc/chain_t.hpp
@@ -241,7 +241,7 @@
   if (blockIdx.x >= c.B * c.H) {
     const EdgeRide& r = c.ride;
     edge_fwd_row<4, false, W>(r.in, nullptr, r.n_valid, r.out, nullptr, nullptr, nullptr, Drop(), r.N, r.D,
-                              blockIdx.x - c.B * c.H, lds);
+                              blockIdx.x - c.B * c.H + r.r0, lds);
     return;
   }
   const int z = blockIdx.x, b = z / c.H, h = z - b * c.H;
diff --git a/gcgcn_amd/csrc/edge.hip b/gcgcn_amd/csrc/edge.hip
--- a/gcgcn_amd/csrc/edge.hip
+++ b/gcgcn_amd/csrc/edge.hip
@@ -1,6 +1,8 @@
 #include <string.h>
 
 #include "edge_body.hpp"
+#include "edge_plan.hpp"
+#include "chain_t_shapes.hpp"
 #include "compact.hpp"
 #include "gat_body.hpp"
 #include "gemm_body.hpp"
@@ -241,6 +243,32 @@
   constexpr int spread_pct = 90, cohort = 256, spread_min = 1024;
   p.spread = make_spread(ntile, rows, cohort, ntile >= spread_min ? spread_pct : 0);
   p.lds = 0;
+}
+
+size_t ride_early_lds(int D) { return sizeof(float) * RIDE_W * (size_t)D; }
+RideEarlyPlan ride_early_plan(const RideEarlyQuery& q) {
+  constexpr double hbm_bytes_per_us = 5.4e6;
+  constexpr double chain_bytes_per_us = 4.29e6;
+  constexpr double t_fold_us = 5.4, t_score_us = 4.9;
+  constexpr double t_pair_layer_us = 9.5;
+  constexpr int cus = 256;
+  RideEarlyPlan p;
+  if (!q.present || option("ride_early", 1) == 0) return p;
+  if (q.B <= 0 || q.N <= 0 || q.D <= 0 || q.pairs <= 0 || q.N > 64) return p;
+  if (q.D % 4 != 0 || (q.mis & (EDGE_MIS_E | EDGE_MIS_EBAR)) || (long)q.B * q.N > 0x3fffffffL) return p;
+  if (ride_early_lds(q.D) > RIDE_EARLY_LDS_MAX || (long)RIDE_W * q.D > 2L * lds_floats<1, 1, true, true>()) return p;
+  if (q.gh != 16 * RIDE_W && t_instantiated(q.gh, q.L)) return p;
+  const long rows = (long)q.B * q.N;
+  const double t_row_us = 4.0 * q.N * (double)q.D / chain_bytes_per_us;
+  const double t_early_us = 4.0 * q.N * (double)q.D / hbm_bytes_per_us;
+  const double t_pairs_us = t_pair_layer_us * (q.L > 0 ? q.L : 1) * ((q.pairs + cus - 1) / cus);
+  if ((double)rows * t_row_us <= t_pairs_us) return p;
+  const long spare = (long)(((double)rows * t_row_us - t_pairs_us) / t_row_us);
+  long rf = (long)(t_fold_us / t_early_us), rs = (long)(t_score_us / t_early_us);
+  if (rf + rs > spare) rf = spare * rf / (rf + rs), rs = spare - rf;
+  if (rf + rs > rows) rf = rows * rf / (rf + rs), rs = rows - rf;
+  p.r_fold = (int)(rf > 0 ? rf : 0), p.r_score = (int)(rs > 0 ? rs : 0);
+  return p;
 }
 
 constexpr int NT_STORE = 0;
diff --git a/gcgcn_amd/csrc/edge_body.hpp b/gcgcn_amd/csrc/edge_body.hpp
--- a/gcgcn_amd/csrc/edge_body.hpp
+++ b/gcgcn_amd/csrc/edge_body.hpp
@@ -158,6 +158,19 @@
 }
 
 
+constexpr int RIDE_W = 8;
+struct EarlyRows {
+  const float* in;
+  const int* n_valid;
+  float* out;
+  int N, D;
+  int first, count;
+};
+__device__ __forceinline__ void early_row_block(const EarlyRows& er, int k, float* __restrict__ cs) {
+  if ((threadIdx.x >> 6) >= RIDE_W) return;
+  edge_fwd_row<4, false, RIDE_W>(er.in, nullptr, er.n_valid, er.out, nullptr, nullptr, nullptr, Drop(), er.N, er.D, er.first + k, cs);
+}
+
 template <int VEC, int EWT>
 __device__ __forceinline__ void edge_bcast_row(const float* __restrict__ dEbar, const int* __restrict__ n_valid,
                                                float* __restrict__ dE, int N, int D, int nt, int bi) {
diff --git a/gcgcn_amd/csrc/edge_plan.hpp b/gcgcn_amd/csrc/edge_plan.hpp
--- a/gcgcn_amd/csrc/edge_plan.hpp
+++ b/gcgcn_amd/csrc/edge_plan.hpp
@@ -38,4 +38,18 @@
 EdgePlan edge_plan_bcast(const EdgeQuery& q);
 void edge_plan_carry(EdgePlan& p, int ntile, bool any_rb, int col_C);
 
+struct RideEarlyQuery {
+  int B, N, D;
+  int pairs;
+  int gh, L;
+  bool present;
+  unsigned mis;
+};
+struct RideEarlyPlan {
+  int r_fold = 0, r_score = 0;
+};
+RideEarlyPlan ride_early_plan(const RideEarlyQuery& q);
+size_t ride_early_lds(int D);
+constexpr size_t RIDE_EARLY_LDS_MAX = 48 * 1024;
+
 }
diff --git a/gcgcn_amd/csrc/gcn_plan.hpp b/gcgcn_amd/csrc/gcn_plan.hpp
--- a/gcgcn_amd/csrc/gcn_plan.hpp
+++ b/gcgcn_amd/csrc/gcn_plan.hpp
@@ -7,6 +7,7 @@
 struct EdgeRide {
   int kind;
   int B, N, D;
+  int r0;
   const float* in;
   const int* n_valid;
   float* out;
diff --git a/gcgcn_amd/csrc/rowops.hip b/gcgcn_amd/csrc/rowops.hip
--- a/gcgcn_amd/csrc/rowops.hip
+++ b/gcgcn_amd/csrc/rowops.hip
@@ -1,3 +1,6 @@
+#include <string.h>
+
+#include "edge_body.hpp"
 #include "gat_body.hpp"
 #include "gemm.hpp"
 #include "rowops.hpp"
@@ -289,9 +292,14 @@
 constexpr int FC = 16;
 __global__ __launch_bounds__(64 * FW) void gat_fold_fwd_kernel(const float* __restrict__ flat, float* __restrict__ uvc, int D,
                                                                int Dh, uint64_t* rng_state, uint64_t* rng_snaps,
-                                                               int rng_count) {
+                                                               int rng_count, const EarlyRows er, const int own) {
   __shared__ float red[2][64][FC + 1];
   __shared__ float redc[FW];
+  extern __shared__ __attribute__((aligned(16))) float early_cs[];
+  if ((int)blockIdx.x >= own) {
+    early_row_block(er, (int)blockIdx.x - own, early_cs);
+    return;
+  }
   if (rng_state && blockIdx.x == 0 && threadIdx.x < 64) {
     const uint64_t seed = rng_state[0], ctr = rng_state[1];
     for (int i = threadIdx.x; i < rng_count; i += 64) rng_snaps[2 * i] = seed, rng_snaps[2 * i + 1] = ctr + (uint64_t)i;
@@ -406,9 +414,16 @@
   gat_dlogit_doc(P, dA, uvc, dXin, dlogit, ds, dX, N, D, drop, blockIdx.x, blockIdx.y, gridDim.y, sm);
 }
 
-__global__ __launch_bounds__(64 * RW) void node_score_fwd_kernel(const float* __restrict__ X, const float* __restrict__ uvc,
-                                                                 float* __restrict__ s, long M, int D, uint64_t* rng_state,
-                                                                 uint64_t* rng_snaps, int rng_count) {
+__global__ __launch_bounds__(64 * RIDE_W) void node_score_fwd_kernel(const float* __restrict__ X, const float* __restrict__ uvc,
+                                                                     float* __restrict__ s, long M, int D, uint64_t* rng_state,
+                                                                     uint64_t* rng_snaps, int rng_count, const EarlyRows er,
+                                                                     const int own) {
+  extern __shared__ __attribute__((aligned(16))) float early_cs[];
+  if ((int)blockIdx.x >= own) {
+    early_row_block(er, (int)blockIdx.x - own, early_cs);
+    return;
+  }
+  if ((threadIdx.x >> 6) >= RW) return;
   if (rng_state && blockIdx.x == 0 && threadIdx.x < 64) {
     const uint64_t seed = rng_state[0], ctr = rng_state[1];
     for (int i = threadIdx.x; i < rng_count; i += 64) rng_snaps[2 * i] = seed, rng_snaps[2 * i + 1] = ctr + (uint64_t)i;
@@ -634,11 +649,22 @@
   return check_launch("colsum3/2");
 }
 
+static_assert(RIDE_W <= FW && RW <= RIDE_W, "a passenger row needs RIDE_W waves of its host's (padded) block");
+static EarlyRows early_or_none(const EarlyRows* early) {
+  EarlyRows er;
+  memset(&er, 0, sizeof er);
+  if (early && early->count > 0) er = *early;
+  return er;
+}
+static size_t early_lds(const EarlyRows& er) { return er.count > 0 ? sizeof(float) * RIDE_W * (size_t)er.D : 0; }
+
 int gat_fold_fwd(const float* flat, float* uvc, int D, int Dh, hipStream_t st, void* rng_state, void* rng_snaps,
-                 int rng_count) {
+                 int rng_count, const EarlyRows* early) {
   ProfScope ps("gat_fold_fwd", st);
-  hipLaunchKernelGGL(gat_fold_fwd_kernel, dim3(cdiv(D, FC)), dim3(64 * FW), 0, st, flat, uvc, D, Dh, (uint64_t*)rng_state,
-                     (uint64_t*)rng_snaps, rng_count);
+  const EarlyRows er = early_or_none(early);
+  const int own = (int)cdiv(D, FC);
+  hipLaunchKernelGGL(gat_fold_fwd_kernel, dim3(own + er.count), dim3(64 * FW), early_lds(er), st, flat, uvc, D, Dh,
+                     (uint64_t*)rng_state, (uint64_t*)rng_snaps, rng_count, er, own);
   return check_launch("gat_fold_fwd");
 }
 int gat_fold_bwd(const float* flat, const float* duvc, float* dflat, int D, int Dh, hipStream_t st, const float* part,
@@ -658,10 +684,13 @@
   return check_launch("gat_dlogit");
 }
 int node_score_fwd(const float* X, const float* uvc, float* s, long M, int D, hipStream_t st, void* rng_state, void* rng_snaps,
-                   int rng_count) {
+                   int rng_count, const EarlyRows* early) {
   ProfScope ps("node_score_fwd", st);
-  hipLaunchKernelGGL(node_score_fwd_kernel, dim3(cdiv(M, RW)), dim3(64 * RW), 0, st, X, uvc, s, M, D, (uint64_t*)rng_state,
-                     (uint64_t*)rng_snaps, rng_count);
+  const EarlyRows er = early_or_none(early);
+  const long own = cdiv(M, RW);
+  GC_REQUIRE(own + er.count <= 0x7fffffffL, "node_score_fwd: too many workgroups");
+  hipLaunchKernelGGL(node_score_fwd_kernel, dim3((unsigned)(own + er.count)), dim3(64 * (er.count > 0 ? RIDE_W : RW)), early_lds(er), st,
+                     X, uvc, s, M, D, (uint64_t*)rng_state, (uint64_t*)rng_snaps, rng_count, er, (int)own);
   return check_launch("node_score_fwd");
 }
 int node_score_bwd(const float* ds, const float* uvc, const float* dXin, float* dX, long M, int D, hipStream_t st) {
diff --git a/gcgcn_amd/csrc/rowops.hpp b/gcgcn_amd/csrc/rowops.hpp
--- a/gcgcn_amd/csrc/rowops.hpp
+++ b/gcgcn_amd/csrc/rowops.hpp
@@ -22,8 +22,9 @@
 int colsum3(const float* X0, const float* w0, float* o0, long R0, int C0, long ld0, const float* X1, const float* w1,
             float* o1, long R1, int C1, long ld1, const float* X2, const float* w2, float* o2, long R2, int C2, long ld2,
             float* scratch, hipStream_t st, bool stage2 = true, long* part_off = nullptr, int* ns_out = nullptr);
+struct EarlyRows;
 int gat_fold_fwd(const float* flat, float* uvc, int D, int Dh, hipStream_t st, void* rng_state = nullptr,
-                 void* rng_snaps = nullptr, int rng_count = 0);
+                 void* rng_snaps = nullptr, int rng_count = 0, const EarlyRows* early = nullptr);
 int gat_fold_bwd(const float* flat, const float* duvc, float* dflat, int D, int Dh, hipStream_t st,
                  const float* part = nullptr, const long* part_off = nullptr, int ns = 0);
 int gat_dlogit_slices(int D);
@@ -31,7 +32,7 @@
 int gat_dlogit(const float* P, const float* dA, const float* uvc, const float* dXin, float* dlogit, float* ds, float* dX,
                int B, int N, int D, int slices, Drop drop, hipStream_t st);
 int node_score_fwd(const float* X, const float* uvc, float* s, long M, int D, hipStream_t st, void* rng_state = nullptr,
-                   void* rng_snaps = nullptr, int rng_count = 0);
+                   void* rng_snaps = nullptr, int rng_count = 0, const EarlyRows* early = nullptr);
 int node_score_bwd(const float* ds, const float* uvc, const float* dXin, float* dX, long M, int D, hipStream_t st);
 int mask_rows(const float* x, float* y, long M, int D, int N, const int* n_valid, Drop drop, hipStream_t st,
               const float* wlin = nullptr, float* wsum = nullptr, int H = 0);
diff --git a/gcgcn_amd/functional.py b/gcgcn_amd/functional.py
--- a/gcgcn_amd/functional.py
+++ b/gcgcn_amd/functional.py
@@ -179,11 +179,19 @@
 class GatFn(torch.autograd.Function):
 
     @staticmethod
-    def forward(ctx, x, e, flat, n_valid, p, snap, pending, Dh, mask, uvc, uvc_valid):
+    def forward(ctx, x, e, flat, n_valid, p, snap, pending, Dh, mask, uvc, uvc_valid, early=None):
         B, N, D = x.shape
         uvc, uvc_valid, s, P, A, ebar, (st, sn, cnt) = _gat_fwd_buffers(x, snap, pending, uvc, uvc_valid)
-        call("gcgcn_gat_fwd", B, N, D, Dh, _p(x), _p(e), _p(n_valid), _p(flat), _p(snap), float(p), _p(uvc), _p(s),
-             _p(P), _p(A), _p(ebar), _p(st), _p(sn), cnt, _p(mask), 1 if uvc_valid else 0, _stream())
+        split = _early_split(early, B, N)
+        if split is None:
+            call("gcgcn_gat_fwd", B, N, D, Dh, _p(x), _p(e), _p(n_valid), _p(flat), _p(snap), float(p), _p(uvc), _p(s),
+                 _p(P), _p(A), _p(ebar), _p(st), _p(sn), cnt, _p(mask), 1 if uvc_valid else 0, _stream())
+        else:
+            e_next, ebar_next, (r_fold, r_score) = split
+            call("gcride_gat_fwd", B, N, D, Dh, _p(x), _p(e), _p(n_valid), _p(flat), _p(snap), float(p), _p(uvc), _p(s),
+                 _p(P), _p(A), _p(ebar), _p(st), _p(sn), cnt, _p(mask), 1 if uvc_valid else 0, _p(e_next), e_next.shape[3],
+                 _p(ebar_next), r_fold, r_score, _stream())
+            _park_early_rows(e_next, n_valid, ebar_next, r_fold + r_score)
         ctx.save_for_backward(x, e, flat, uvc, P)
         ctx.n_valid, ctx.p, ctx.snap, ctx.Dh, ctx.mask = n_valid, float(p), snap, Dh, mask
         return (P if A is None else A), ebar, x.view_as(x)
@@ -206,7 +214,7 @@
         call("gcgcn_gat_bwd", B, N, D, ctx.Dh, _p(x), _p(e), _p(ctx.n_valid), _p(flat), _p(ctx.snap), ctx.p, _p(uvc), _p(P),
              _p(dA), _p(dEbar), _p(dXin), _p(dX), _p(dE), _p(dflat), _p(dlogit), _p(ds), _p(dvpart), _p(duvc),
              _p(scratch), None if bp is None else bp.queue, _stream())
-        return dX, dE, dflat, None, None, None, None, None, None, None, None
+        return dX, dE, dflat, None, None, None, None, None, None, None, None, None
 
 
 class EdgeMeanFn(torch.autograd.Function):
@@ -357,9 +365,46 @@
     return bp
 
 
-def _ride(inp, n_valid, out, B, N, D):
-    r = _lib.EdgeRide(B, N, D, inp.data_ptr(), None if n_valid is None else n_valid.data_ptr(), out.data_ptr())
+def _ride(inp, n_valid, out, B, N, D, r0=0):
+    r = _lib.EdgeRide(B, N, D, r0, inp.data_ptr(), None if n_valid is None else n_valid.data_ptr(), out.data_ptr())
     return r, ctypes.cast(ctypes.pointer(r), ctypes.c_void_p)
+
+
+ride_early_split = None
+
+
+def _early_split(early, B, N):
+    if early is None:
+        return None
+    e_next, H, L = early
+    if (not isinstance(e_next, torch.Tensor) or not e_next.is_cuda or e_next.dim() != 4 or e_next.dtype != torch.float32
+            or not e_next.is_contiguous() or tuple(e_next.shape[:3]) != (B, N, N)):
+        return None
+    D = e_next.shape[3]
+    if ride_early_split is not None:
+        split = (int(ride_early_split[0]), int(ride_early_split[1]))
+    else:
+        out = (ctypes.c_int32 * 2)()
+        call("gcride_debug_plan", B, N, D, B * H, D // L, L, 1, 1 if e_next.data_ptr() % 16 else 0, ctypes.cast(out, ctypes.c_void_p))
+        split = (out[0], out[1])
+    if split[0] + split[1] <= 0:
+        return None
+    return e_next, torch.empty(B, N, D, device=e_next.device), split
+
+
+def _early_key(e_next: Tensor, n_valid):
+    return (e_next.data_ptr(), tuple(e_next.shape), e_next._version, None if n_valid is None else n_valid.data_ptr())
+
+
+def _park_early_rows(e_next: Tensor, n_valid, ebar_next: Tensor, rows: int):
+    _tls.early_rows = (_early_key(e_next, n_valid), ebar_next, rows)
+
+
+def _take_early_rows(e_next: Tensor, n_valid):
+    ent, _tls.early_rows = getattr(_tls, "early_rows", None), None
+    if ent is not None and ent[0] == _early_key(e_next, n_valid):
+        return ent[1], ent[2]
+    return None, 0
 
 
 head_sum_in_forward = True
@@ -381,8 +426,10 @@
     scratch = torch.empty(max(_lib.lib().gcgcn_gcn_scratch(B, N, D, H), 1), device=dev)
     ebar_next, ride, ride_p = None, None, None
     if e_next is not None:
-        ebar_next = torch.empty(e_next.shape[0], e_next.shape[1], e_next.shape[3], device=dev)
-        ride, ride_p = _ride(e_next, n_valid, ebar_next, *ebar_next.shape)
+        ebar_next, r0 = _take_early_rows(e_next, n_valid)
+        if ebar_next is None:
+            ebar_next = torch.empty(e_next.shape[0], e_next.shape[1], e_next.shape[3], device=dev)
+        ride, ride_p = _ride(e_next, n_valid, ebar_next, *ebar_next.shape, r0=r0)
     call("gcgcn_gcn_fwd", B, N, D, L, H, _p(x), _p(ebar), None if hook is not None else _p(adj), _p(n_valid), _p(flat), _p(snap),
          float(p), _p(out_snap), float(out_p), _p(out), _p(Pn), _p(Y), _p(HO), _p(rinv), _p(G), _p(wsum), _p(scratch), ride_p,
          None if hook is None else ctypes.cast(ctypes.pointer(hook), ctypes.c_void_p), _p(rowblk), _stream())
@@ -880,7 +927,8 @@
     return rng_snapshot(dev) if (training and p > 0.0) else None
 
 
-def gat_attention(x, e, flat, n_valid=None, p=0.1, training=False, hidden_dim=None, mask=None, uvc=None, uvc_valid=False):
+def gat_attention(x, e, flat, n_valid=None, p=0.1, training=False, hidden_dim=None, mask=None, uvc=None, uvc_valid=False,
+                  early=None):
     x, e = _chk(x, "node_feat", 3), _chk(e, "edge_feat", 4)
     B, N, D = x.shape
     if e.shape != (B, N, N, D):
@@ -892,7 +940,7 @@
             raise ValueError(f"mask: expected a GPU tensor of shape {(B, N, N)}, got {tuple(mask.shape)} on {mask.device}")
         mask = (mask != 0).to(torch.uint8).contiguous()
     return GatFn.apply(x, e, _chk(flat, "flat"), nv, p, snap, _take_pending_rng(x.device),
-                       D if hidden_dim is None else int(hidden_dim), mask, uvc, bool(uvc_valid))
+                       D if hidden_dim is None else int(hidden_dim), mask, uvc, bool(uvc_valid), early)
 
 
 def gat_attention_compact(x, ce: CompactEdges, flat, n_valid=None, p=0.1, training=False, hidden_dim=None, uvc=None, uvc_valid=False):
diff --git a/gcgcn_amd/modules.py b/gcgcn_amd/modules.py
--- a/gcgcn_amd/modules.py
+++ b/gcgcn_amd/modules.py
@@ -108,7 +108,7 @@
         return super()._load_from_state_dict(*args, **kwargs)
 
     def forward(self, node_feat: Tensor, edge_feat: Tensor, mask: Optional[Tensor] = None,
-                n_valid: Optional[Tensor] = None, return_input_alias: bool = False) -> Tensor:
+                n_valid: Optional[Tensor] = None, return_input_alias: bool = False, early_edge=None) -> Tensor:
         x, batched = _batched(node_feat, 2)
         compact = isinstance(edge_feat, F_.CompactEdges)
         if compact and self.apply_mask:
@@ -131,7 +131,7 @@
                                                    uvc=uvc, uvc_valid=valid)
         else:
             a, ebar, xa = F_.gat_attention(x, e, self.flat, n_valid, self.p, self.training, hidden_dim=self.hidden_dim,
-                                           mask=mk, uvc=uvc, uvc_valid=valid)
+                                           mask=mk, uvc=uvc, uvc_valid=valid, early=early_edge if batched else None)
         F_.park_edge_mean(edge_feat, n_valid, ebar)
         a = a if batched else a.squeeze(0)
         return (a, xa if batched else xa.squeeze(0)) if return_input_alias else a
@@ -461,8 +461,10 @@
                 mask = None
                 if self.get_weighted_adj_matrix.apply_mask and adj_matrix is not None:
                     mask = torch.eq(adj_matrix, 0)
-                a, xa = self.get_weighted_adj_matrix(x, e, mask, n_valid=n_valid, return_input_alias=True)
-                new = self.graphcnn[i](xa, e, a, n_valid=n_valid, ride_edge=ride(i), out_dropout=odrop, rowblk=rb)
+                nxt, conv = ride(i), self.graphcnn[i]
+                early = None if (nxt is None or isinstance(nxt, F_.CompactEdges)) else (nxt, conv.head_num, conv.layer_num)
+                a, xa = self.get_weighted_adj_matrix(x, e, mask, n_valid=n_valid, return_input_alias=True, early_edge=early)
+                new = conv(xa, e, a, n_valid=n_valid, ride_edge=nxt, out_dropout=odrop, rowblk=rb)
             else:
                 if self.fuse_maggc:
                     new = self.graphcnn[i].forward_with_attention(self.get_adj_matrix[i - 1], x, e, n_valid=n_valid,
diff --git a/include/gcgcn.h b/include/gcgcn.h
--- a/include/gcgcn.h
+++ b/include/gcgcn.h
@@ -54,6 +54,7 @@
 int64_t gcgcn_gcn_scratch(int B, int N, int D, int H);
 typedef struct gcgcn_edge_ride {
   int32_t B, N, D;
+  int32_t r0;
   const float* in;
   const int32_t* n_valid;
   float* out;
diff --git a/include/gcgcn_ride.h b/include/gcgcn_ride.h
--- /dev/null
+++ b/include/gcgcn_ride.h
@@ -0,0 +1,18 @@
+#ifndef GCGCN_RIDE_H
+#define GCGCN_RIDE_H
+#include <stdint.h>
+#ifdef __cplusplus
+extern "C" {
+#endif
+
+int gcride_debug_plan(int B, int N, int D, int pairs, int gh, int L, int present, int misalign, int32_t* out2);
+
+int gcride_gat_fwd(int B, int N, int D, int Dh, const float* X, const float* E, const int32_t* n_valid, const float* flat,
+                   const void* rng_snap, float p, float* uvc, float* s, float* P, float* A, float* Ebar, void* rng_state,
+                   void* rng_snaps, int rng_count, const uint8_t* mask, int uvc_valid, const float* E_next, int D_next,
+                   float* ebar_next, int r_fold, int r_score, void* stream);
+
+#ifdef __cplusplus
+}
+#endif
+#endif
```

New measurement: 66040 docs/s (median of 6 runs). Within noise of the previous version (+0.6%).
